# gattia/pyfocusr

Hardware: AMD Instinct MI355X
Metric: lowest-k eigenpairs/sec + KNN-correspondence wall-clock, 250k-vertex mesh pair k=5 (higher is better)
Workload: dtype f64

## Files before the change

include/pyfocusr_hip.h:

```cpp
#ifndef PYFOCUSR_HIP_H
#define PYFOCUSR_HIP_H

#include <stddef.h>
#include <stdint.h>

#ifdef __cplusplus
extern "C" {
#endif

#define PF_VERSION 1

#define PF_OK 0
#define PF_E_ARG (-1)
#define PF_E_HIP (-2)
#define PF_E_DEGENERATE (-3)
#define PF_E_STATE (-4)
#define PF_E_PERSIST_TIMEOUT (-5)
#define PF_E_INTERNAL (-6)

#define PF_OP_RW 0
#define PF_OP_SYM 1

typedef struct pf_ctx pf_ctx;
typedef struct pf_graph pf_graph;
typedef struct pf_mesh pf_mesh;

typedef struct pf_graph_info {
    int64_t n;
    int64_t n_faces;
    int64_t nnz_w;
    int64_t nnz_l;
    int32_t is_symmetric;
    int32_t n_isolated;
    int32_t n_components;
    int32_t max_degree;
    int64_t sell_entries;
    int64_t n_pad;
    int64_t n_oneway;
    double spectral_bound;
} pf_graph_info;

typedef struct pf_timing {
    double op_ms;
    int64_t op_launches;
    double op_bytes;
    double knn_ms;
    double build_ms;
    double persist_ms;
    int64_t persist_launches;
    int64_t persist_steps;
    double persist_bytes;
    double persist_lds_bytes;
} pf_timing;

int pf_version(void);
int pf_pool_poison(int on);
const char* pf_last_error(void);
int pf_device_count(void);
int pf_create(int device, pf_ctx** out);
void pf_destroy(pf_ctx* ctx);
int pf_sync(pf_ctx* ctx);
void* pf_stream(pf_ctx* ctx);
int pf_timing_enable(pf_ctx* ctx, int on);
int pf_timing_get(pf_ctx* ctx, pf_timing* out, int reset);

int pf_graph_build(pf_ctx* ctx, const double* pts, int64_t n, const int32_t* faces, int64_t n_faces,
                   int32_t verts_per_face, pf_graph** out);
int pf_mesh_upload(pf_ctx* ctx, const double* pts, int64_t n, const int32_t* faces, int64_t n_faces,
                   int32_t verts_per_face, pf_mesh** out);
void pf_mesh_free(pf_mesh* mesh);
int pf_graph_build_device(pf_mesh* mesh, pf_graph** out);
int pf_graph_build_device2(pf_mesh* mesh_a, pf_mesh* mesh_b, pf_graph** out_a, pf_graph** out_b);
int pf_graph_from_matrix(pf_ctx* ctx, int64_t n, const int32_t* rowptr, const int32_t* colidx, const double* values,
                         pf_graph** out);
int pf_graph_build_cotan(pf_mesh* mesh, int32_t mass_kind , pf_graph** out);
int pf_graph_cotan_info(pf_graph* g, double* hi, double* total_area);
int pf_graph_cotan_download(pf_graph* g, double* w, double* diag, double* mass);
int pf_cotan_apply(pf_graph* g, const double* x, int32_t ncols, double* out);
void pf_graph_free(pf_graph* g);
int pf_graph_get_info(pf_graph* g, pf_graph_info* out);
int pf_graph_rows_compacted(pf_graph* g);
int pf_graph_download(pf_graph* g, int32_t* rowptr, int32_t* colidx, double* w, double* l_offdiag,
                      double* deg, double* l_diag, int32_t* component_label);

int pf_ws_ensure(pf_graph* g, int32_t n_slots);
int pf_ws_upload(pf_graph* g, int32_t slot, const double* x);
int pf_ws_download(pf_graph* g, int32_t first, int32_t count, double* out);
int pf_ws_copy(pf_graph* g, int32_t src, int32_t dst, int32_t count);
int pf_start_vector(pf_graph* g, int32_t slot, uint64_t seed);
int pf_mask_isolated(pf_graph* g, int32_t slot);
int pf_lock_null_vectors(pf_graph* g, int32_t op, int32_t* n_locked);

int pf_spmv(pf_graph* g, int32_t op, int32_t src, int32_t dst);
int pf_spmv_multi(pf_graph* g, int32_t op, int32_t src_first, int32_t dst_first, int32_t count);
int pf_persist_enable(int on);
int pf_persist_two_step(int level);
int pf_persist_pair_halves(int on);
int pf_persist_clock(pf_ctx* ctx, double* kernel_ms, int64_t* launches, int reset);
typedef struct pf_persist_info {
    int32_t enabled;
    int32_t two_step;
    int32_t owner;
    int32_t timeouts;
    int64_t launches;
    int64_t launches_two_step;
    int32_t suspended_for;
    int32_t rearms;
    int32_t owner_switches;
    int32_t hold_ticks;
} pf_persist_info;
int pf_persist_state(pf_ctx* ctx , pf_persist_info* out);
int pf_graph_window_info(pf_graph* g, int32_t want_rings, int32_t* win_rows, int32_t* n_windows, int32_t* state,
                         int32_t* state2, int32_t* ghosts , int32_t* ghosts2 ,
                         int32_t* need );
int pf_persist_test_hook(int n_launches);
int pf_cheb(pf_graph* g, int32_t op, int32_t src, int32_t dst, int32_t degree, double c, double e, double rho);
int pf_cheb2(pf_graph* ga, int32_t op_a, int32_t src_a, int32_t dst_a, int32_t degree_a, double c_a, double e_a, double rho_a,
             pf_graph* gb, int32_t op_b, int32_t src_b, int32_t dst_b, int32_t degree_b, double c_b, double e_b, double rho_b);
int pf_dots(pf_graph* g, int32_t w, int32_t first, int32_t count, double* out);
int pf_orth(pf_graph* g, int32_t w, int32_t first, int32_t count, double* h, double* nrm);
int pf_orth_begin(pf_graph* g, int32_t w, int32_t first, int32_t count, int32_t normalize);
int pf_orth_end(pf_graph* g, double* h, double* nrm);
int pf_orth_begin2(pf_graph* ga, int32_t w_a, int32_t first_a, int32_t count_a, int32_t normalize_a, pf_graph* gb, int32_t w_b,
                   int32_t first_b, int32_t count_b, int32_t normalize_b);
int pf_orth_cheb2(pf_graph* ga, pf_graph* gb, const int32_t* orth, const int32_t* cheb_i, const double* cheb_d);
int pf_orth_redone(pf_graph* g);
int pf_orth_strict(pf_graph* g, int32_t on);
int pf_orth_device_passes(pf_graph* g, int32_t on);
int pf_orth_split(pf_graph* g, int32_t first2, int32_t split);
int pf_orth_one_launch(int32_t on);
int pf_scale(pf_graph* g, int32_t slot, double alpha);
int pf_combine(pf_graph* g, int32_t src_first, int32_t m, const double* Y, int32_t k, int32_t dst_first);
int pf_resnorm(pf_graph* g, int32_t ax, int32_t x, double lam, double* out);
int pf_gram(pf_graph* g, int32_t first_a, int32_t count_a, int32_t first_b, int32_t count_b, double* out);
int pf_resnorms(pf_graph* g, int32_t ax_first, int32_t x_first, const double* lam, int32_t count, double* out);
int pf_finalize_vectors(pf_graph* g, int32_t first, int32_t count, int32_t from_sym, int32_t minmax,
                        double* out);
int pf_finalize_vectors_begin(pf_graph* g, int32_t first, int32_t count, int32_t from_sym, int32_t minmax, double* out);
int pf_finalize_vectors_end(pf_graph* g);
int pf_final_remap_begin(pf_graph* g, const int32_t* col, const double* sign, int32_t count, double* out);
int pf_host_alloc(size_t bytes, void** out);
int pf_host_free(void* p);
int pf_host_detach(void* p);
int pf_final_rows(pf_graph* g, const int64_t* rows, int64_t n_rows, double* out);
int pf_point_rows(pf_graph* g, const int64_t* rows, int64_t n_rows, double* out);
int pf_spmv_host(pf_graph* g, int32_t op, const double* x, double* y);
int pf_mean_filter(pf_graph* g, const double* values, int32_t ncols, int32_t iterations, double* out);

int pf_knn1(pf_ctx* ctx, const double* ref, int64_t n_ref, const double* qry, int64_t n_qry, int32_t d,
            int64_t* idx_out, double* d2_out);
int pf_knn_mode(pf_ctx* ctx, int32_t mode);
int pf_knn_tree_stats(pf_ctx* ctx, int32_t enable_counting, int64_t* leaves_scanned, int64_t* supers_opened);
int pf_knn_count(pf_ctx* ctx, int32_t enable_counting, int64_t* pairs);
int pf_knn_wave_stats(pf_ctx* ctx, double* sum_us, double* max_us, int64_t* waves, int64_t* max_candidates, double* detail);
int pf_knn(pf_ctx* ctx, const double* ref, int64_t n_ref, const double* qry, int64_t n_qry, int32_t d, int32_t k,
           int64_t* idx_out, double* d2_out);
int pf_knn_topk(pf_ctx* ctx, const double* ref, int64_t n_ref, const double* qry, int64_t n_qry, int32_t d, int32_t k,
                int64_t* idx_out, double* d2_out);
int pf_knn1_graphs(pf_graph* ref_g, pf_graph* qry_g, int32_t d, const int32_t* col_ref, const double* scale_ref,
                   const int32_t* col_qry, const double* scale_qry, int64_t* idx_out, double* d2_out);
int pf_knn1_blocks(pf_ctx* ctx, const double* ref_block, int64_t n_ref, int32_t ref_stride, const double* qry_block,
                   int64_t n_qry, int32_t qry_stride, int32_t d, const int32_t* col_ref, const double* scale_ref,
                   const int32_t* col_qry, const double* scale_qry, int64_t* idx_out, double* d2_out);
int pf_eigsort_costs(pf_graph* g_target, pf_graph* g_source, const int64_t* rows_t, int64_t m_t, const int64_t* rows_s, int64_t m_s,
                     int32_t k, const int32_t* col_t, const double* sign_t, const int32_t* col_s, const double* sign_s, double* out,
                     int64_t* idx_out);
int pf_final_device(pf_graph* g, double** block, int64_t* n_rows, int32_t* n_cols);
int pf_knn_upload(pf_ctx* ctx, const double* ref, int64_t n_ref, const double* qry, int64_t n_qry, int32_t d);
int pf_knn_run(pf_ctx* ctx);
int pf_knn_download(pf_ctx* ctx, int64_t* idx_out, double* d2_out);

int pf_knn1_wide(pf_ctx* ctx, const double* ref, int64_t n_ref, const double* qry, int64_t n_qry, int32_t d,
                 int64_t* idx_out, double* d2_out );
int pf_knn1_wide_count(pf_ctx* ctx, int32_t enable_counting, int64_t* coordinate_pairs);
typedef struct pf_fmap pf_fmap;
int pf_fmap_create(pf_ctx* ctx, const double* phi_t, int64_t n_t, const double* phi_s, int64_t n_s, const double* mass_s,
                   int32_t K, pf_fmap** out);
void pf_fmap_free(pf_fmap* h);
int pf_fmap_set_p2p(pf_fmap* h, const int64_t* T);
int pf_fmap_get_p2p(pf_fmap* h, int64_t* T_out, double* d2_out);
int pf_fmap_project(pf_fmap* h, int32_t k_s, int32_t k_t, double* C_out);
int pf_fmap_convert(pf_fmap* h, const double* C, int32_t k_s, int32_t k_t);
int pf_fmap_zoomout(pf_fmap* h, int32_t k_start, int32_t k_end, int32_t step, int32_t n_iter_at_end, double* C_out);
int pf_fmap_set_samples(pf_fmap* h, const int64_t* S_t, int64_t q_t, const int64_t* S_s, int64_t q_s);
int pf_fmap_zoomout_sampled(pf_fmap* h, int32_t k_start, int32_t k_end, int32_t step, int32_t n_iter_at_end, double* C_out);

int pf_fps(pf_ctx* ctx, const double* points, int64_t n, int32_t d, int64_t m, int64_t start, int64_t* sel_out,
           int32_t* owner_out, double* dmin_out);

int pf_spectral_descriptors(pf_ctx* ctx, const double* phi, int64_t n, int32_t K, const double* G, int32_t T, double* out);
int pf_descriptor_coefficients(pf_ctx* ctx, const double* phi, const double* mass, int64_t n, int32_t K, const double* G,
                               int32_t T, int32_t k_out, double* A_out);

typedef struct pf_eigs_stats {
    int64_t matvecs;
    int32_t outer_steps;
    int32_t restarts;
    int32_t filter_resets;
    int32_t degree;
    int32_t n_null;
    double cut;
    double max_residual;
    int32_t second_passes;
    int32_t mode;
    int32_t local_steps;
    int32_t reserved;
} pf_eigs_stats;
int pf_eigs_smallest(pf_graph* g, int32_t n_wanted, int32_t minmax, double* vals, double* vecs, int32_t* n_out,
                     pf_eigs_stats* stats);
int pf_eigs_smallest_ex(pf_graph* g, int32_t n_wanted, int32_t minmax, int32_t async_download, double* vals, double* vecs,
                        double* residuals, int32_t* n_out, pf_eigs_stats* stats);
int pf_eigs_smallest2(pf_graph* ga, pf_graph* gb, int32_t n_wanted_a, int32_t n_wanted_b, int32_t minmax, int32_t async_download,
                      double* vals_a, double* vecs_a, double* res_a, int32_t* n_out_a, pf_eigs_stats* stats_a,
                      double* vals_b, double* vecs_b, double* res_b, int32_t* n_out_b, pf_eigs_stats* stats_b);

typedef struct pf_rows pf_rows;
int pf_op_step(pf_graph* g, int32_t op, int32_t x, int32_t prev, int32_t out, double alpha, double shift, double beta);
int pf_cheb_steps(pf_graph* g, int32_t op, int32_t prev, int32_t cur, int32_t k_first, int32_t n_steps, double c, double e,
                  double rho, int32_t* out_prev, int32_t* out_cur);
int pf_axpy(pf_graph* g, int32_t w, int32_t first, int32_t count, const double* coef);
int pf_rows_create(pf_graph* g, const int64_t* rows, int64_t n, pf_rows** out);
void pf_rows_free(pf_rows* r);
int pf_rows_gather(pf_rows* r, int32_t slot, double* out);
int pf_rows_scatter(pf_rows* r, int32_t slot, const double* in);
int pf_rows_gather_dev(pf_rows* r, int32_t slot, double* dst_device);
int pf_rows_scatter_dev(pf_rows* r, int32_t slot, const double* src_device);
int pf_rows_set_sources(pf_rows* r, const int64_t* offsets);
int pf_rows_gather2_dev(pf_rows* r, int32_t slot_a, int32_t slot_b, double* dst_device, int64_t stride);
int pf_rows_scatter2_dev(pf_rows* r, int32_t slot_a, int32_t slot_b, const double* src_device, int64_t stride);
int pf_rows_fill(pf_rows* r, int32_t slot, double value);

typedef struct pf_surface pf_surface;
int pf_surface_create(pf_ctx* ctx, const double* points, int64_t n, const int32_t* faces, int64_t n_faces,
                      int32_t verts_per_face, pf_surface** out);
void pf_surface_free(pf_surface* s);
int pf_surface_closest(pf_surface* s, const double* qry, int64_t n_qry, double* out_pts, int32_t* out_face,
                       double* out_d2);
int pf_surface_distance(pf_surface* s, const double* qry, int64_t n_qry, double* out_d2, int32_t* out_face,
                        double* stats);
int pf_surface_prepare_signed(pf_surface* s, const double* points, const int32_t* faces, int64_t* topology);
int pf_surface_signed_distance(pf_surface* s, const double* qry, int64_t n_qry, double* out_sd, int32_t* out_face,
                               int32_t* out_feature, int64_t* n_ambiguous);
int pf_surface_prepare_winding(pf_surface* s);
int pf_surface_winding(pf_surface* s, const double* qry, int64_t n_qry, double beta, double* out_w, double* out_bound);
int pf_surface_raycast(pf_surface* s, const double* origins, const double* dirs, int64_t n_rays, double t_min, double t_max,
                       int32_t facing, double* out_t, int32_t* out_face, double* out_uv, int32_t* out_count);
int pf_surface_vertex_normals(pf_surface* s, double* out);

typedef struct pf_surface_nd pf_surface_nd;
int pf_surface_nd_create(pf_ctx* ctx, const double* coords, int64_t n, int32_t d, const int32_t* faces, int64_t n_faces,
                         int32_t verts_per_face, pf_surface_nd** out);
void pf_surface_nd_free(pf_surface_nd* s);
int pf_surface_nd_closest(pf_surface_nd* s, const double* qry, int64_t n_qry, int32_t* out_face, int32_t* out_verts,
                          double* out_bary, double* out_d2, int32_t exhaustive);
int pf_surface_nd_last_search(pf_surface_nd* s, int64_t* chunks_opened, int64_t* packets, int64_t* n_chunks);

typedef struct pf_cpd pf_cpd;
int pf_cpd_create(pf_ctx* ctx, const double* X, int64_t N, const double* Y, int64_t M, int32_t d, pf_cpd** out);
void pf_cpd_free(pf_cpd* h);
int pf_cpd_estep(pf_cpd* h, const double* TY, double sigma2, double w, double* P1, double* Pt1, double* PX);
int pf_cpd_set_basis(pf_cpd* h, const double* Q, int32_t K);
int pf_cpd_weighted_gram(pf_cpd* h, double* H);
int pf_cpd_affine_sums(pf_cpd* h, double* shifts, double* sums);
int pf_cpd_apply_affine(pf_cpd* h, const double* B, const double* t);
int pf_cpd_deform_sums(pf_cpd* h, double* H, double* R);
int pf_cpd_apply_deform(pf_cpd* h, const double* C, double* sums);
int pf_cpd_download(pf_cpd* h, double* TY, double* P1, double* Pt1, double* PX);
int pf_cpd_gram(pf_ctx* ctx, const double* A, int64_t n_a, const double* B, int64_t n_b, int32_t d, double beta,
                const double* V, int32_t n_cols, double* out);

typedef struct pf_assign_stats {
    int32_t phases;
    int32_t dense_passes;
    int64_t rounds;
    int64_t bids;
    int64_t dense_bids;
    int64_t candidate_edges;
    int64_t launches;
    int64_t device_bytes;
    int32_t k;
    int32_t eps_floor_hit;
    double eps_initial, eps_final, eps_floor;
    double total_cost;
    double gap_bound;
    double lower_bound;
    double ms_candidates, ms_auction, ms_certificate;
} pf_assign_stats;
int pf_assign(pf_ctx* ctx, const double* rows, int64_t n_rows, const double* cols, int64_t n_cols, int32_t d,
              int64_t* col_of_row, double* u_out, double* v_out, pf_assign_stats* stats);

int pf_curvatures(pf_ctx* ctx, const double* pts, int64_t n, const int32_t* faces, int64_t n_faces, double* out_area,
                  double* out_gauss, double* out_mean, double* out_tensor6, double* out_kminmax, double* out_dirs,
                  double* out_normals, uint8_t* out_boundary, int64_t* topology, double* device_ms);

#define PF_TOPOLOGY_OUTWARD 1u
int pf_mesh_topology(pf_ctx* ctx, const double* pts, int64_t n, const int32_t* faces, int64_t n_faces, uint32_t flags,
                     int32_t* face_neighbours, int32_t* patch, uint8_t* flip, int32_t* boundary_loop, uint8_t* patch_orientable,
                     double* patch_volume, int64_t* report, double* device_ms);

#define PF_CLUSTER_UPDATE_ONLY 1u
int pf_mesh_cluster(pf_ctx* ctx, const double* pts, int64_t n, const int32_t* faces, int64_t n_faces, const double* mass,
                    const int64_t* seeds, int64_t m, int32_t n_iter, uint32_t flags, const double* centroids_in,
                    const int32_t* labels_in, int32_t* labels, double* centroids, int32_t* rep, int32_t* count, int32_t* changed,
                    int32_t* out_faces, int32_t* face_src, int32_t* votes, int64_t* report, double* device_ms);

int pf_map_distortion(pf_ctx* ctx, const double* src_pts, int64_t n_src, const int32_t* src_faces, int64_t n_faces,
                      const double* tgt_pts, int64_t n_tgt, const double* tgt_normals, const int32_t* map_vertices,
                      const double* map_weights, int32_t c, double* face_sigma, double* face_area_ratio, uint8_t* face_flags,
                      double* vertex_area, double* vertex_sigma, uint8_t* vertex_flags, int32_t* target_count,
                      double* target_premass, double* totals, int64_t* report, double* device_ms);

#ifdef __cplusplus
}
#endif
#endif
```

pyfocusr_amd/_hip.py:

```python
import atexit
import ctypes as C
import os
import threading
import weakref

import numpy as np

_HERE = os.path.dirname(os.path.abspath(__file__))
LIB_PATH = os.environ.get("PYFOCUSR_HIP_LIB", os.path.join(_HERE, "csrc", "libpyfocusr_hip.so"))

PF_OP_RW = 0
PF_OP_SYM = 1

_f64p = C.POINTER(C.c_double)
_i32p = C.POINTER(C.c_int32)
_i64p = C.POINTER(C.c_int64)


class HipUnavailable(RuntimeError):
    pass


class PfError(RuntimeError):
    def __init__(self, code, msg):
        RuntimeError.__init__(self, "libpyfocusr_hip error %d: %s" % (code, msg))
        self.code = code


class _Struct(C.Structure):

    def as_dict(self):
        return {name: getattr(self, name) for name, _ in self._fields_}


class GraphInfo(_Struct):
    _fields_ = [("n", C.c_int64), ("n_faces", C.c_int64), ("nnz_w", C.c_int64), ("nnz_l", C.c_int64),
                ("is_symmetric", C.c_int32), ("n_isolated", C.c_int32), ("n_components", C.c_int32),
                ("max_degree", C.c_int32), ("sell_entries", C.c_int64), ("n_pad", C.c_int64), ("n_oneway", C.c_int64),
                ("spectral_bound", C.c_double)]


class EigsStats(_Struct):
    _fields_ = [("matvecs", C.c_int64), ("outer_steps", C.c_int32), ("restarts", C.c_int32), ("filter_resets", C.c_int32),
                ("degree", C.c_int32), ("n_null", C.c_int32), ("cut", C.c_double), ("max_residual", C.c_double),
                ("second_passes", C.c_int32), ("mode", C.c_int32), ("local_steps", C.c_int32), ("reserved", C.c_int32)]


class Timing(_Struct):
    _fields_ = [("op_ms", C.c_double), ("op_launches", C.c_int64), ("op_bytes", C.c_double), ("knn_ms", C.c_double),
                ("build_ms", C.c_double), ("persist_ms", C.c_double), ("persist_launches", C.c_int64),
                ("persist_steps", C.c_int64), ("persist_bytes", C.c_double), ("persist_lds_bytes", C.c_double)]


class AssignStats(_Struct):
    _fields_ = [("phases", C.c_int32), ("dense_passes", C.c_int32), ("rounds", C.c_int64), ("bids", C.c_int64),
                ("dense_bids", C.c_int64), ("candidate_edges", C.c_int64), ("launches", C.c_int64),
                ("device_bytes", C.c_int64), ("k", C.c_int32), ("eps_floor_hit", C.c_int32), ("eps_initial", C.c_double),
                ("eps_final", C.c_double), ("eps_floor", C.c_double), ("total_cost", C.c_double),
                ("gap_bound", C.c_double), ("lower_bound", C.c_double), ("ms_candidates", C.c_double),
                ("ms_auction", C.c_double), ("ms_certificate", C.c_double)]


SIGNATURES = {
    "pf_version": (C.c_int, []),
    "pf_pool_poison": (C.c_int, [C.c_int]),
    "pf_last_error": (C.c_char_p, []),
    "pf_device_count": (C.c_int, []),
    "pf_create": (C.c_int, [C.c_int, C.POINTER(C.c_void_p)]),
    "pf_destroy": (None, [C.c_void_p]),
    "pf_sync": (C.c_int, [C.c_void_p]),
    "pf_stream": (C.c_void_p, [C.c_void_p]),
    "pf_timing_enable": (C.c_int, [C.c_void_p, C.c_int]),
    "pf_timing_get": (C.c_int, [C.c_void_p, C.POINTER(Timing), C.c_int]),
    "pf_graph_build": (C.c_int, [C.c_void_p, _f64p, C.c_int64, _i32p, C.c_int64, C.c_int32, C.POINTER(C.c_void_p)]),
    "pf_mesh_upload": (C.c_int, [C.c_void_p, _f64p, C.c_int64, _i32p, C.c_int64, C.c_int32, C.POINTER(C.c_void_p)]),
    "pf_mesh_free": (None, [C.c_void_p]),
    "pf_graph_build_device": (C.c_int, [C.c_void_p, C.POINTER(C.c_void_p)]),
    "pf_graph_build_device2": (C.c_int, [C.c_void_p, C.c_void_p, C.POINTER(C.c_void_p), C.POINTER(C.c_void_p)]),
    "pf_graph_from_matrix": (C.c_int, [C.c_void_p, C.c_int64, _i32p, _i32p, _f64p, C.POINTER(C.c_void_p)]),
    "pf_graph_build_cotan": (C.c_int, [C.c_void_p, C.c_int32, C.POINTER(C.c_void_p)]),
    "pf_graph_cotan_info": (C.c_int, [C.c_void_p, C.POINTER(C.c_double), C.POINTER(C.c_double)]),
    "pf_graph_cotan_download": (C.c_int, [C.c_void_p, _f64p, _f64p, _f64p]),
    "pf_cotan_apply": (C.c_int, [C.c_void_p, _f64p, C.c_int32, _f64p]),
    "pf_graph_free": (None, [C.c_void_p]),
    "pf_graph_get_info": (C.c_int, [C.c_void_p, C.POINTER(GraphInfo)]),
    "pf_graph_rows_compacted": (C.c_int, [C.c_void_p]),
    "pf_graph_download": (C.c_int, [C.c_void_p, _i32p, _i32p, _f64p, _f64p, _f64p, _f64p, _i32p]),
    "pf_ws_ensure": (C.c_int, [C.c_void_p, C.c_int32]),
    "pf_ws_upload": (C.c_int, [C.c_void_p, C.c_int32, _f64p]),
    "pf_ws_download": (C.c_int, [C.c_void_p, C.c_int32, C.c_int32, _f64p]),
    "pf_ws_copy": (C.c_int, [C.c_void_p, C.c_int32, C.c_int32, C.c_int32]),
    "pf_start_vector": (C.c_int, [C.c_void_p, C.c_int32, C.c_uint64]),
    "pf_mask_isolated": (C.c_int, [C.c_void_p, C.c_int32]),
    "pf_lock_null_vectors": (C.c_int, [C.c_void_p, C.c_int32, _i32p]),
    "pf_spmv": (C.c_int, [C.c_void_p, C.c_int32, C.c_int32, C.c_int32]),
    "pf_spmv_multi": (C.c_int, [C.c_void_p, C.c_int32, C.c_int32, C.c_int32, C.c_int32]),
    "pf_knn_mode": (C.c_int, [C.c_void_p, C.c_int32]),
    "pf_knn_tree_stats": (C.c_int, [C.c_void_p, C.c_int32, C.POINTER(C.c_int64), C.POINTER(C.c_int64)]),
    "pf_persist_enable": (C.c_int, [C.c_int]),
    "pf_persist_two_step": (C.c_int, [C.c_int]),
    "pf_persist_pair_halves": (C.c_int, [C.c_int]),
    "pf_persist_clock": (C.c_int, [C.c_void_p, C.POINTER(C.c_double), C.POINTER(C.c_int64), C.c_int]),
    "pf_persist_state": (C.c_int, [C.c_void_p, C.c_void_p]),
    "pf_graph_window_info": (C.c_int, [C.c_void_p, C.c_int32] + [C.POINTER(C.c_int32)] * 4 + [_i32p, _i32p, _i32p]),
    "pf_persist_test_hook": (C.c_int, [C.c_int]),
    "pf_cheb": (C.c_int, [C.c_void_p, C.c_int32, C.c_int32, C.c_int32, C.c_int32, C.c_double, C.c_double, C.c_double]),
    "pf_cheb2": (C.c_int, [C.c_void_p, C.c_int32, C.c_int32, C.c_int32, C.c_int32, C.c_double, C.c_double, C.c_double,
                           C.c_void_p, C.c_int32, C.c_int32, C.c_int32, C.c_int32, C.c_double, C.c_double, C.c_double]),
    "pf_dots": (C.c_int, [C.c_void_p, C.c_int32, C.c_int32, C.c_int32, _f64p]),
    "pf_orth": (C.c_int, [C.c_void_p, C.c_int32, C.c_int32, C.c_int32, _f64p, _f64p]),
    "pf_orth_begin": (C.c_int, [C.c_void_p, C.c_int32, C.c_int32, C.c_int32, C.c_int32]),
    "pf_orth_end": (C.c_int, [C.c_void_p, _f64p, _f64p]),
    "pf_orth_split": (C.c_int, [C.c_void_p, C.c_int32, C.c_int32]),
    "pf_orth_one_launch": (C.c_int, [C.c_int32]),
    "pf_orth_begin2": (C.c_int, [C.c_void_p, C.c_int32, C.c_int32, C.c_int32, C.c_int32, C.c_void_p, C.c_int32, C.c_int32, C.c_int32,
                                 C.c_int32]),
    "pf_orth_cheb2": (C.c_int, [C.c_void_p, C.c_void_p, _i32p, _i32p, _f64p]),
    "pf_eigsort_costs": (C.c_int, [C.c_void_p, C.c_void_p, _i64p, C.c_int64, _i64p, C.c_int64, C.c_int32, _i32p, _f64p, _i32p, _f64p, _f64p,
                                   _i64p]),
    "pf_orth_redone": (C.c_int, [C.c_void_p]),
    "pf_orth_strict": (C.c_int, [C.c_void_p, C.c_int32]),
    "pf_scale": (C.c_int, [C.c_void_p, C.c_int32, C.c_double]),
    "pf_combine": (C.c_int, [C.c_void_p, C.c_int32, C.c_int32, _f64p, C.c_int32, C.c_int32]),
    "pf_resnorm": (C.c_int, [C.c_void_p, C.c_int32, C.c_int32, C.c_double, _f64p]),
    "pf_gram": (C.c_int, [C.c_void_p, C.c_int32, C.c_int32, C.c_int32, C.c_int32, _f64p]),
    "pf_resnorms": (C.c_int, [C.c_void_p, C.c_int32, C.c_int32, _f64p, C.c_int32, _f64p]),
    "pf_finalize_vectors": (C.c_int, [C.c_void_p, C.c_int32, C.c_int32, C.c_int32, C.c_int32, _f64p]),
    "pf_finalize_vectors_begin": (C.c_int, [C.c_void_p, C.c_int32, C.c_int32, C.c_int32, C.c_int32, _f64p]),
    "pf_finalize_vectors_end": (C.c_int, [C.c_void_p]),
    "pf_final_remap_begin": (C.c_int, [C.c_void_p, _i32p, _f64p, C.c_int32, _f64p]),
    "pf_host_alloc": (C.c_int, [C.c_size_t, C.POINTER(C.c_void_p)]),
    "pf_host_free": (C.c_int, [C.c_void_p]),
    "pf_final_rows": (C.c_int, [C.c_void_p, _i64p, C.c_int64, _f64p]),
    "pf_point_rows": (C.c_int, [C.c_void_p, _i64p, C.c_int64, _f64p]),
    "pf_spmv_host": (C.c_int, [C.c_void_p, C.c_int32, _f64p, _f64p]),
    "pf_mean_filter": (C.c_int, [C.c_void_p, _f64p, C.c_int32, C.c_int32, _f64p]),
    "pf_knn1": (C.c_int, [C.c_void_p, _f64p, C.c_int64, _f64p, C.c_int64, C.c_int32, _i64p, _f64p]),
    "pf_knn": (C.c_int, [C.c_void_p, _f64p, C.c_int64, _f64p, C.c_int64, C.c_int32, C.c_int32, _i64p, _f64p]),
    "pf_knn_topk": (C.c_int, [C.c_void_p, _f64p, C.c_int64, _f64p, C.c_int64, C.c_int32, C.c_int32, _i64p, _f64p]),
    "pf_knn1_graphs": (C.c_int, [C.c_void_p, C.c_void_p, C.c_int32, _i32p, _f64p, _i32p, _f64p, _i64p, _f64p]),
    "pf_knn1_blocks": (C.c_int, [C.c_void_p, C.c_void_p, C.c_int64, C.c_int32, C.c_void_p, C.c_int64, C.c_int32, C.c_int32,
                                 _i32p, _f64p, _i32p, _f64p, _i64p, _f64p]),
    "pf_final_device": (C.c_int, [C.c_void_p, C.POINTER(C.c_void_p), _i64p, _i32p]),
    "pf_knn_upload": (C.c_int, [C.c_void_p, _f64p, C.c_int64, _f64p, C.c_int64, C.c_int32]),
    "pf_knn_run": (C.c_int, [C.c_void_p]),
    "pf_knn_download": (C.c_int, [C.c_void_p, _i64p, _f64p]),
    "pf_eigs_smallest": (C.c_int, [C.c_void_p, C.c_int32, C.c_int32, _f64p, _f64p, C.POINTER(C.c_int32), C.POINTER(EigsStats)]),
    "pf_knn_count": (C.c_int, [C.c_void_p, C.c_int32, C.POINTER(C.c_int64)]),
    "pf_knn_wave_stats": (C.c_int, [C.c_void_p, C.POINTER(C.c_double), C.POINTER(C.c_double), C.POINTER(C.c_int64), C.POINTER(C.c_int64),
                                    _f64p]),
    "pf_host_detach": (C.c_int, [C.c_void_p]),
    "pf_orth_device_passes": (C.c_int, [C.c_void_p, C.c_int32]),
    "pf_eigs_smallest_ex": (C.c_int, [C.c_void_p, C.c_int32, C.c_int32, C.c_int32, _f64p, _f64p, _f64p, C.POINTER(C.c_int32),
                                      C.POINTER(EigsStats)]),
    "pf_eigs_smallest2": (C.c_int, [C.c_void_p, C.c_void_p, C.c_int32, C.c_int32, C.c_int32, C.c_int32,
                                    _f64p, _f64p, _f64p, C.POINTER(C.c_int32), C.POINTER(EigsStats),
                                    _f64p, _f64p, _f64p, C.POINTER(C.c_int32), C.POINTER(EigsStats)]),
    "pf_op_step": (C.c_int, [C.c_void_p, C.c_int32, C.c_int32, C.c_int32, C.c_int32, C.c_double, C.c_double, C.c_double]),
    "pf_cheb_steps": (C.c_int, [C.c_void_p, C.c_int32, C.c_int32, C.c_int32, C.c_int32, C.c_int32, C.c_double, C.c_double,
                                C.c_double, C.POINTER(C.c_int32), C.POINTER(C.c_int32)]),
    "pf_axpy": (C.c_int, [C.c_void_p, C.c_int32, C.c_int32, C.c_int32, _f64p]),
    "pf_rows_create": (C.c_int, [C.c_void_p, _i64p, C.c_int64, C.POINTER(C.c_void_p)]),
    "pf_rows_free": (None, [C.c_void_p]),
    "pf_rows_gather": (C.c_int, [C.c_void_p, C.c_int32, _f64p]),
    "pf_rows_scatter": (C.c_int, [C.c_void_p, C.c_int32, _f64p]),
    "pf_rows_gather_dev": (C.c_int, [C.c_void_p, C.c_int32, C.c_void_p]),
    "pf_rows_scatter_dev": (C.c_int, [C.c_void_p, C.c_int32, C.c_void_p]),
    "pf_rows_set_sources": (C.c_int, [C.c_void_p, _i64p]),
    "pf_rows_gather2_dev": (C.c_int, [C.c_void_p, C.c_int32, C.c_int32, C.c_void_p, C.c_int64]),
    "pf_rows_scatter2_dev": (C.c_int, [C.c_void_p, C.c_int32, C.c_int32, C.c_void_p, C.c_int64]),
    "pf_rows_fill": (C.c_int, [C.c_void_p, C.c_int32, C.c_double]),
    "pf_surface_create": (C.c_int, [C.c_void_p, _f64p, C.c_int64, _i32p, C.c_int64, C.c_int32, C.POINTER(C.c_void_p)]),
    "pf_surface_free": (None, [C.c_void_p]),
    "pf_surface_closest": (C.c_int, [C.c_void_p, _f64p, C.c_int64, _f64p, _i32p, _f64p]),
    "pf_surface_distance": (C.c_int, [C.c_void_p, _f64p, C.c_int64, _f64p, _i32p, _f64p]),
    "pf_surface_prepare_signed": (C.c_int, [C.c_void_p, _f64p, _i32p, _i64p]),
    "pf_surface_signed_distance": (C.c_int, [C.c_void_p, _f64p, C.c_int64, _f64p, _i32p, _i32p, _i64p]),
    "pf_surface_prepare_winding": (C.c_int, [C.c_void_p]),
    "pf_surface_winding": (C.c_int, [C.c_void_p, _f64p, C.c_int64, C.c_double, _f64p, _f64p]),
    "pf_surface_raycast": (C.c_int, [C.c_void_p, _f64p, _f64p, C.c_int64, C.c_double, C.c_double, C.c_int32, _f64p, _i32p, _f64p,
                                     _i32p]),
    "pf_surface_vertex_normals": (C.c_int, [C.c_void_p, _f64p]),
    "pf_knn1_wide": (C.c_int, [C.c_void_p, _f64p, C.c_int64, _f64p, C.c_int64, C.c_int32, _i64p, _f64p]),
    "pf_knn1_wide_count": (C.c_int, [C.c_void_p, C.c_int32, _i64p]),
    "pf_fmap_create": (C.c_int, [C.c_void_p, _f64p, C.c_int64, _f64p, C.c_int64, _f64p, C.c_int32, C.POINTER(C.c_void_p)]),
    "pf_fmap_free": (None, [C.c_void_p]),
    "pf_fmap_set_p2p": (C.c_int, [C.c_void_p, _i64p]),
    "pf_fmap_get_p2p": (C.c_int, [C.c_void_p, _i64p, _f64p]),
    "pf_fmap_project": (C.c_int, [C.c_void_p, C.c_int32, C.c_int32, _f64p]),
    "pf_fmap_convert": (C.c_int, [C.c_void_p, _f64p, C.c_int32, C.c_int32]),
    "pf_fmap_zoomout": (C.c_int, [C.c_void_p, C.c_int32, C.c_int32, C.c_int32, C.c_int32, _f64p]),
    "pf_fmap_set_samples": (C.c_int, [C.c_void_p, _i64p, C.c_int64, _i64p, C.c_int64]),
    "pf_fmap_zoomout_sampled": (C.c_int, [C.c_void_p, C.c_int32, C.c_int32, C.c_int32, C.c_int32, _f64p]),
    "pf_fps": (C.c_int, [C.c_void_p, _f64p, C.c_int64, C.c_int32, C.c_int64, C.c_int64, _i64p, _i32p, _f64p]),
    "pf_spectral_descriptors": (C.c_int, [C.c_void_p, _f64p, C.c_int64, C.c_int32, _f64p, C.c_int32, _f64p]),
    "pf_descriptor_coefficients": (C.c_int, [C.c_void_p, _f64p, _f64p, C.c_int64, C.c_int32, _f64p, C.c_int32, C.c_int32, _f64p]),
    "pf_surface_nd_create": (C.c_int, [C.c_void_p, _f64p, C.c_int64, C.c_int32, _i32p, C.c_int64, C.c_int32,
                                       C.POINTER(C.c_void_p)]),
    "pf_surface_nd_free": (None, [C.c_void_p]),
    "pf_surface_nd_closest": (C.c_int, [C.c_void_p, _f64p, C.c_int64, _i32p, _i32p, _f64p, _f64p, C.c_int32]),
    "pf_surface_nd_last_search": (C.c_int, [C.c_void_p, _i64p, _i64p, _i64p]),
    "pf_cpd_create": (C.c_int, [C.c_void_p, _f64p, C.c_int64, _f64p, C.c_int64, C.c_int32, C.POINTER(C.c_void_p)]),
    "pf_cpd_free": (None, [C.c_void_p]),
    "pf_cpd_estep": (C.c_int, [C.c_void_p, _f64p, C.c_double, C.c_double, _f64p, _f64p, _f64p]),
    "pf_cpd_set_basis": (C.c_int, [C.c_void_p, _f64p, C.c_int32]),
    "pf_cpd_weighted_gram": (C.c_int, [C.c_void_p, _f64p]),
    "pf_cpd_affine_sums": (C.c_int, [C.c_void_p, _f64p, _f64p]),
    "pf_cpd_apply_affine": (C.c_int, [C.c_void_p, _f64p, _f64p]),
    "pf_cpd_deform_sums": (C.c_int, [C.c_void_p, _f64p, _f64p]),
    "pf_cpd_apply_deform": (C.c_int, [C.c_void_p, _f64p, _f64p]),
    "pf_cpd_download": (C.c_int, [C.c_void_p, _f64p, _f64p, _f64p, _f64p]),
    "pf_cpd_gram": (C.c_int, [C.c_void_p, _f64p, C.c_int64, _f64p, C.c_int64, C.c_int32, C.c_double, _f64p, C.c_int32, _f64p]),
    "pf_assign": (C.c_int, [C.c_void_p, _f64p, C.c_int64, _f64p, C.c_int64, C.c_int32, _i64p, _f64p, _f64p,
                            C.POINTER(AssignStats)]),
    "pf_curvatures": (C.c_int, [C.c_void_p, _f64p, C.c_int64, _i32p, C.c_int64, _f64p, _f64p, _f64p, _f64p, _f64p, _f64p, _f64p,
                                C.POINTER(C.c_uint8), _i64p, _f64p]),
    "pf_mesh_topology": (C.c_int, [C.c_void_p, _f64p, C.c_int64, _i32p, C.c_int64, C.c_uint32, _i32p, _i32p, C.POINTER(C.c_uint8),
                                   _i32p, C.POINTER(C.c_uint8), _f64p, _i64p, _f64p]),
    "pf_mesh_cluster": (C.c_int, [C.c_void_p, _f64p, C.c_int64, _i32p, C.c_int64, _f64p, _i64p, C.c_int64, C.c_int32, C.c_uint32,
                                  _f64p, _i32p, _i32p, _f64p, _i32p, _i32p, _i32p, _i32p, _i32p, _i32p, _i64p, _f64p]),
    "pf_map_distortion": (C.c_int, [C.c_void_p, _f64p, C.c_int64, _i32p, C.c_int64, _f64p, C.c_int64, _f64p, _i32p, _f64p, C.c_int32,
                                    _f64p, _f64p, C.POINTER(C.c_uint8), _f64p, _f64p, C.POINTER(C.c_uint8), _i32p, _f64p, _f64p,
                                    _i64p, _f64p]),
}

_lib = None
_lib_lock = threading.Lock()
_live_graphs = weakref.WeakSet()
_live_contexts = weakref.WeakSet()


@atexit.register
def _shutdown():
    for g in list(_live_graphs):
        g.close()
    for c in list(_live_contexts):
        c.close()


def load_library():
    global _lib
    with _lib_lock:
        if _lib is not None:
            return _lib
        if not os.path.exists(LIB_PATH):
            raise HipUnavailable(
                "%s not found: build it with `python -c 'import __graft_entry__ as g; g.build()'` "
                "(hipcc --offload-arch=gfx950); there is no CPU fallback" % LIB_PATH)
        lib = C.CDLL(LIB_PATH)
        for name, (res, args) in SIGNATURES.items():
            fn = getattr(lib, name)
            fn.restype = res
            fn.argtypes = args
        _lib = lib
        return lib


PF_E_DEGENERATE = -3
PF_E_STATE = -4
PF_E_PERSIST_TIMEOUT = -5
PF_E_INTERNAL = -6
PF_TOPOLOGY_OUTWARD = 1
PF_CLUSTER_UPDATE_ONLY = 1


class _PinnedBlock(object):
    __slots__ = ("ptr", "nbytes")

    def __init__(self, ptr, nbytes):
        self.ptr, self.nbytes = ptr, nbytes

    def __del__(self):
        try:
            _pinned_release(self.ptr, self.nbytes)
        except Exception:
            pass


_pinned_free = {}
_pinned_cached = [0]
_pinned_lock = threading.RLock()
_PINNED_CACHE_BYTES = 1 << 30


def _pinned_release(ptr, nbytes):
    if _pinned_free is None or _lib is None:
        return
    _lib.pf_host_detach(C.c_void_p(ptr))
    evicted = []
    with _pinned_lock:
        if nbytes <= _PINNED_CACHE_BYTES:
            while _pinned_cached[0] + nbytes > _PINNED_CACHE_BYTES:
                others = [sz for sz, ptrs in _pinned_free.items() if ptrs and sz != nbytes]
                if not others:
                    break
                sz = max(others)
                evicted.append(_pinned_free[sz].pop())
                _pinned_cached[0] -= sz
        keep = _pinned_cached[0] + nbytes <= _PINNED_CACHE_BYTES
        if keep:
            _pinned_free.setdefault(nbytes, []).append(ptr)
            _pinned_cached[0] += nbytes
    for other in evicted:
        _lib.pf_host_free(C.c_void_p(other))
    if not keep:
        _lib.pf_host_free(C.c_void_p(ptr))


def pinned_trim():
    with _pinned_lock:
        blocks = [p for ptrs in _pinned_free.values() for p in ptrs]
        _pinned_free.clear()
        _pinned_cached[0] = 0
    for ptr in blocks:
        _lib.pf_host_free(C.c_void_p(ptr))


def pinned_empty(shape, dtype=np.float64):
    lib = load_library()
    dtype = np.dtype(dtype)
    count = int(np.prod(shape)) if len(shape) else 1
    nbytes = max(count * dtype.itemsize, 1)
    nbytes = (nbytes + 4095) & ~4095
    ptr = None
    with _pinned_lock:
        free = _pinned_free.get(nbytes)
        if free:
            ptr = free.pop()
            _pinned_cached[0] -= nbytes
    if ptr is None:
        p = C.c_void_p()
        _check(lib.pf_host_alloc(C.c_size_t(nbytes), C.byref(p)))
        ptr = int(p.value)
    buf = (C.c_char * nbytes).from_address(ptr)
    buf._pf_block = _PinnedBlock(ptr, nbytes)
    return np.frombuffer(buf, dtype=dtype, count=count).reshape(shape)


def persist_enable(on=True):
    _check(load_library().pf_persist_enable(int(bool(on))))


def pool_poison(on=True):
    on = int(on)
    if on not in (0, 1, 2):
        raise ValueError("pool_poison: 0 (off), 1 (0xFF bytes) or 2 (zero bytes), got %r" % (on,))
    _check(load_library().pf_pool_poison(on))


def orth_one_launch(on=True):
    _check(load_library().pf_orth_one_launch(int(bool(on))))


def persist_two_step(level=1):
    _check(load_library().pf_persist_two_step(int(level)))


def persist_pair_halves(on=True):
    _check(load_library().pf_persist_pair_halves(int(bool(on))))


def persist_clock(ctx, reset=False):
    ms, n = C.c_double(0.0), C.c_int64(0)
    _check(load_library().pf_persist_clock(ctx._h, C.byref(ms), C.byref(n), int(bool(reset))))
    return ms.value, n.value


class _PersistInfo(_Struct):
    _fields_ = [("enabled", C.c_int32), ("two_step", C.c_int32), ("owner", C.c_int32), ("timeouts", C.c_int32),
                ("launches", C.c_int64), ("launches_two_step", C.c_int64), ("suspended_for", C.c_int32), ("rearms", C.c_int32),
                ("owner_switches", C.c_int32), ("hold_ticks", C.c_int32)]


def persist_state(ctx=None):
    info = _PersistInfo()
    _check(load_library().pf_persist_state(None if ctx is None else ctx._h, C.byref(info)))
    return info.as_dict()


def persist_test_hook(n_launches=1):
    _check(load_library().pf_persist_test_hook(int(n_launches)))


def _check(code):
    if code != 0:
        raise PfError(code, load_library().pf_last_error().decode("utf-8", "replace"))


_POINTER_OF = {np.dtype(t): C.POINTER(c) for t, c in ((np.float64, C.c_double), (np.int32, C.c_int32), (np.int64, C.c_int64),
                                                        (np.uint8, C.c_uint8), (np.uint64, C.c_uint64))}


def _ptr(a):
    if a is None:
        return None
    try:
        ptype = _POINTER_OF[a.dtype]
    except KeyError:
        raise TypeError("no pointer type for dtype %s: the library takes float64, int32, int64, uint8 and uint64" % a.dtype)
    if not a.flags.c_contiguous:
        raise ValueError("the library needs a C-contiguous array, not a strided view")
    return a.ctypes.data_as(ptype)


def _f64(a):
    if a is not None and a.dtype != np.float64:
        raise TypeError("a float64 array is needed, not %s" % a.dtype)
    return _ptr(a)


def _c_f64(a, shape=None):
    a = np.ascontiguousarray(a, dtype=np.float64)
    if shape is not None and a.shape != shape:
        raise ValueError("expected shape %r, got %r" % (shape, a.shape))
    return a


def _c_i32(a):
    return np.ascontiguousarray(a, dtype=np.int32)


def _c_i64(a):
    return np.ascontiguousarray(a, dtype=np.int64)


_EQUAL_D = "%s must be (n, d) arrays with equal d"


def _same_d(a, b, message=_EQUAL_D % "ref and qry"):
    a, b = _c_f64(a), _c_f64(b)
    if a.ndim != 2 or b.ndim != 2 or a.shape[1] != b.shape[1]:
        raise ValueError(message)
    return a, b


def _queries(a, noun="queries", message=None):
    a = _c_f64(a)
    if a.ndim != 2 or a.shape[1] != 3 or a.shape[0] == 0:
        raise ValueError(message or "%s must be a non-empty (n, 3) array" % noun)
    return a


def _rays(origins, directions):
    message = "origins and directions must be non-empty (n, 3) arrays of the same length"
    o, d = _queries(origins, message=message), _c_f64(directions)
    if d.shape != o.shape:
        raise ValueError(message)
    return o, d


def _upload_arrays(points, faces, empty_ok=True):
    pts, f = _c_f64(points).reshape(-1, 3), _c_i32(faces)
    if f.ndim != 2 or not (empty_ok or f.shape[0]):
        raise ValueError("faces must be %s" % ("(F, verts_per_face)" if empty_ok else "a non-empty (F, verts_per_face) array"))
    return pts, f, f.shape[1] if f.shape[0] else 3


def degenerate_extent_message(target_points, source_points):
    found = []
    for name, pts in (("target", target_points), ("source", source_points)):
        pts = np.asarray(pts, dtype=np.float64).reshape(-1, 3)
        with np.errstate(invalid="ignore"):
            flat = np.isnan(pts).any(axis=0) | ~(np.max(pts, axis=0) > np.min(pts, axis=0))
        if flat.any():
            found.append("the %s sample (%d points) has no extent along %s" % (name, len(pts), ", ".join("xyz"[a] for a in np.where(flat)[0])))
    return ("eigsort: degenerate extent - %s: the min-max normalisation of the sampled points divides by zero (a planar "
            "mesh, or a sample of one point), so no point has a nearest neighbour"
            % ("; ".join(found) if found else "the sampled points do not compare"))


KNN_TOPK_MAX_K = 64
KNN_TOPK_MAX_D = 128


def check_knn_topk(ref, qry, k):
    ref_shape, qry_shape = np.shape(ref), np.shape(qry)
    if len(ref_shape) != 2 or len(qry_shape) != 2 or ref_shape[1] != qry_shape[1]:
        raise ValueError(_EQUAL_D % "ref and qry")
    if not 1 <= ref_shape[1] <= KNN_TOPK_MAX_D:
        raise ValueError("d = %d out of range (1 .. %d)" % (ref_shape[1], KNN_TOPK_MAX_D))
    k = int(k)
    if not 1 <= k <= min(KNN_TOPK_MAX_K, ref_shape[0]):
        raise ValueError("k = %d out of range (1 .. min(%d, n_ref = %d))" % (k, KNN_TOPK_MAX_K, ref_shape[0]))
    return k


class Context(object):

    def __init__(self, device=0):
        lib = load_library()
        if lib.pf_device_count() <= 0:
            raise HipUnavailable("no HIP device visible: the pyfocusr_amd hot path needs an MI355X (no CPU fallback)")
        h = C.c_void_p()
        _check(lib.pf_create(int(device), C.byref(h)))
        self._lib = lib
        self._h = h
        self.device = int(device)
        self._children = weakref.WeakSet()
        _live_contexts.add(self)

    def close(self):
        if getattr(self, "_h", None):
            for child in list(self._children):
                child.close()
            self._lib.pf_destroy(self._h)
            self._h = None

    def __del__(self):
        try:
            self.close()
        except Exception:
            pass

    def sync(self):
        _check(self._lib.pf_sync(self._h))

    @property
    def stream_ptr(self):
        return int(self._lib.pf_stream(self._h) or 0)

    def timing_enable(self, on=True):
        _check(self._lib.pf_timing_enable(self._h, int(on)))

    def timing(self, reset=False):
        t = Timing()
        _check(self._lib.pf_timing_get(self._h, C.byref(t), int(bool(reset))))
        return t.as_dict()

    def knn_mode(self, mode):
        _check(self._lib.pf_knn_mode(self._h, int(mode)))

    def knn_count(self, enable_counting=False):
        pairs = C.c_int64()
        _check(self._lib.pf_knn_count(self._h, int(bool(enable_counting)), C.byref(pairs)))
        return int(pairs.value)

    def knn_tree_stats(self, enable_counting=False):
        a, b = C.c_int64(), C.c_int64()
        _check(self._lib.pf_knn_tree_stats(self._h, int(bool(enable_counting)), C.byref(a), C.byref(b)))
        return int(a.value), int(b.value)

    def knn1(self, ref, qry, return_d2=False):
        ref, qry = _same_d(ref, qry)
        idx = np.empty(qry.shape[0], dtype=np.int64)
        d2 = np.empty(qry.shape[0], dtype=np.float64) if return_d2 else None
        _check(self._lib.pf_knn1(self._h, _f64(ref), ref.shape[0], _f64(qry), qry.shape[0], ref.shape[1],
                                 _ptr(idx), _f64(d2)))
        return (idx, d2) if return_d2 else idx

    def knn1_wide(self, ref, qry, return_d2=False):
        ref, qry = _same_d(ref, qry)
        idx = np.empty(qry.shape[0], dtype=np.int64)
        d2 = np.empty(qry.shape[0], dtype=np.float64) if return_d2 else None
        _check(self._lib.pf_knn1_wide(self._h, _f64(ref), ref.shape[0], _f64(qry), qry.shape[0], ref.shape[1],
                                      _ptr(idx), _f64(d2)))
        return (idx, d2) if return_d2 else idx

    def knn1_wide_count(self, enable_counting=False):
        pairs = C.c_int64()
        _check(self._lib.pf_knn1_wide_count(self._h, int(bool(enable_counting)), C.byref(pairs)))
        return int(pairs.value)

    def farthest_point_sampling(self, points, m, start=-1, return_owner=False, return_d2=False):
        pts = _c_f64(points)
        if pts.ndim != 2:
            raise ValueError("points must be an (n, d) array")
        n, m = pts.shape[0], int(m)
        sel = np.empty(max(m, 0), dtype=np.int64)
        owner = np.empty(n, dtype=np.int32) if return_owner else None
        d2 = np.empty(n, dtype=np.float64) if return_d2 else None
        _check(self._lib.pf_fps(self._h, _f64(pts), n, pts.shape[1], m, int(start), _ptr(sel), _ptr(owner), _f64(d2)))
        out = (sel,) + ((owner,) if return_owner else ()) + ((d2,) if return_d2 else ())
        return out if len(out) > 1 else sel

    def spectral_descriptors(self, phi, G):
        phi, G = _c_f64(phi), _c_f64(G)
        if phi.ndim != 2 or G.ndim != 2 or G.shape[0] != phi.shape[1]:
            raise ValueError("phi must be (n, K) and G (K, T)")
        out = np.empty((phi.shape[0], G.shape[1]), dtype=np.float64)
        _check(self._lib.pf_spectral_descriptors(self._h, _f64(phi), phi.shape[0], phi.shape[1], _f64(G), G.shape[1], _f64(out)))
        return out

    def descriptor_coefficients(self, phi, mass, G, k_out):
        phi, G = _c_f64(phi), _c_f64(G)
        if phi.ndim != 2 or G.ndim != 2 or G.shape[0] != phi.shape[1]:
            raise ValueError("phi must be (n, K) and G (K, T)")
        mass = _c_f64(mass, (phi.shape[0],))
        out = np.empty((max(int(k_out), 0), G.shape[1]), dtype=np.float64)
        _check(self._lib.pf_descriptor_coefficients(self._h, _f64(phi), _f64(mass), phi.shape[0], phi.shape[1], _f64(G), G.shape[1],
                                                    int(k_out), _f64(out)))
        return out

    def curvatures(self, points, faces):
        pts = _c_f64(points)
        f = _c_i32(faces)
        if pts.ndim != 2 or pts.shape[1] != 3 or f.ndim != 2 or f.shape[1] != 3:
            raise ValueError("points must be (n, 3) and faces (m, 3)")
        n = pts.shape[0]
        out = {"area": np.empty(n), "gaussian": np.empty(n), "mean": np.empty(n), "tensor": np.empty((n, 6)), "k": np.empty((n, 4)),
               "dirs": np.empty((n, 6)), "normals": np.empty((n, 3))}
        boundary = np.empty(n, dtype=np.uint8)
        topology = np.zeros(5, dtype=np.int64)
        ms = C.c_double(0.0)
        _check(self._lib.pf_curvatures(self._h, _f64(pts), n, _ptr(f), f.shape[0], _f64(out["area"]),
                                       _f64(out["gaussian"]), _f64(out["mean"]), _f64(out["tensor"]), _f64(out["k"]),
                                       _f64(out["dirs"]), _f64(out["normals"]), _ptr(boundary), _ptr(topology), C.byref(ms)))
        out.update(boundary=boundary.astype(bool), topology=topology, device_ms=ms.value)
        return out

    def mesh_topology(self, n_points, faces, points=None, outward=True):
        f = _c_i32(faces)
        if f.ndim != 2 or f.shape[1] != 3:
            raise ValueError("faces must be (m, 3)")
        n, m = int(n_points), f.shape[0]
        pts = None
        if points is not None:
            pts = _c_f64(points)
            if pts.shape != (n, 3):
                raise ValueError("points must be (n_points, 3)")
        nbr, loop = np.empty((m, 3), dtype=np.int32), np.empty((m, 3), dtype=np.int32)
        patch, flip = np.empty(m, dtype=np.int32), np.empty(m, dtype=np.uint8)
        orientable, volume = np.empty(m, dtype=np.uint8), np.empty(m)
        report = np.zeros(8, dtype=np.int64)
        ms = C.c_double(0.0)
        _check(self._lib.pf_mesh_topology(self._h, _f64(pts), n, _ptr(f), m, PF_TOPOLOGY_OUTWARD if outward else 0, _ptr(nbr),
                                          _ptr(patch), _ptr(flip), _ptr(loop), _ptr(orientable), _f64(volume), _ptr(report),
                                          C.byref(ms)))
        P = int(report[4])
        return {"face_neighbours": nbr, "patch": patch, "flip": flip.astype(bool), "boundary_loop": loop,
                "patch_orientable": orientable[:P].astype(bool), "patch_volume": volume[:P].copy(), "report": report,
                "device_ms": ms.value}

    def cluster_mesh(self, points, faces, mass, seeds=None, n_iter=20, centroids=None, labels=None, update_only=False):
        pts = _c_f64(points)
        if pts.ndim != 2 or pts.shape[1] != 3:
            raise ValueError("points must be (n, 3)")
        n = pts.shape[0]
        f = np.zeros((0, 3), dtype=np.int32) if faces is None else _c_i32(faces)
        if f.ndim != 2 or f.shape[1] != 3:
            raise ValueError("faces must be (f, 3)")
        mass = _c_f64(mass, (n,))
        if (seeds is None) == (centroids is None):
            raise ValueError("give either seeds or centroids")
        sel = cen = lab = None
        if seeds is not None:
            sel = _c_i64(seeds)
            if sel.ndim != 1:
                raise ValueError("seeds must be a vector of vertex indices")
            m = sel.shape[0]
        else:
            cen = _c_f64(centroids)
            if cen.ndim != 2 or cen.shape[1] != 3:
                raise ValueError("centroids must be (m, 3)")
            m = cen.shape[0]
        if labels is not None:
            lab = _c_i32(labels)
            if lab.shape != (n,):
                raise ValueError("labels must be (n,)")
        n_iter, k = int(n_iter), f.shape[0]
        out_labels, out_c = np.empty(n, dtype=np.int32), np.empty((m, 3))
        rep, count = np.empty(m, dtype=np.int32), np.empty(m, dtype=np.int32)
        changed = np.zeros(max(n_iter, 0), dtype=np.int32)
        out_f, src, votes = np.empty((k, 3), dtype=np.int32), np.empty(k, dtype=np.int32), np.empty((k, 2), dtype=np.int32)
        report = np.zeros(8, dtype=np.int64)
        ms = C.c_double(0.0)
        _check(self._lib.pf_mesh_cluster(
            self._h, _f64(pts), n, _ptr(f if k else None), k, _f64(mass), _ptr(sel), m, n_iter,
            PF_CLUSTER_UPDATE_ONLY if update_only else 0, _f64(cen), _ptr(lab), _ptr(out_labels), _f64(out_c), _ptr(rep),
            _ptr(count), _ptr(changed), _ptr(out_f), _ptr(src), _ptr(votes), _ptr(report), C.byref(ms)))
        run, kept = (0 if update_only else int(report[0])), int(report[1])
        return {"labels": out_labels, "centroids": out_c, "rep": rep, "count": count, "changed": changed[:run].copy(),
                "n_iter_run": int(report[0]), "faces": out_f[:kept].copy(), "face_src": src[:kept].copy(),
                "votes": votes[:kept].copy(), "n_candidate_faces": int(report[2]), "report": report, "device_ms": ms.value}

    def map_distortion(self, src_points, src_faces, tgt_points, map_vertices, map_weights=None, tgt_normals=None):
        pts, tgt = _c_f64(src_points), _c_f64(tgt_points)
        f = _c_i32(src_faces)
        if pts.ndim != 2 or pts.shape[1] != 3 or tgt.ndim != 2 or tgt.shape[1] != 3 or f.ndim != 2 or f.shape[1] != 3:
            raise ValueError("points must be (n, 3) and faces (m, 3)")
        n, m, k = pts.shape[0], f.shape[0], tgt.shape[0]
        mv = _c_i32(map_vertices)
        if mv.ndim == 1:
            mv = mv.reshape(-1, 1)
        if mv.ndim != 2 or mv.shape[0] != n or mv.shape[1] not in (1, 3):
            raise ValueError("map_vertices must be (n,), (n, 1) or (n, 3)")
        c = mv.shape[1]
        mw = None
        if c == 3:
            if map_weights is None:
                raise ValueError("a map of 3 corners needs map_weights (n, 3)")
            mw = _c_f64(map_weights, (n, 3))
        nrm = None if tgt_normals is None else _c_f64(tgt_normals, (k, 3))
        out = {"face_sigma": np.empty((m, 2)), "face_area_ratio": np.empty(m), "face_flags": np.empty(m, dtype=np.uint8),
               "vertex_area": np.empty(n), "vertex_sigma": np.empty((n, 2)), "vertex_flags": np.empty(n, dtype=np.uint8),
               "target_count": np.empty(k, dtype=np.int32), "target_premass": np.empty(k), "totals": np.zeros(8),
               "report": np.zeros(8, dtype=np.int64)}
        ms = C.c_double(0.0)
        _check(self._lib.pf_map_distortion(
            self._h, _f64(pts), n, _ptr(f), m, _f64(tgt), k, _f64(nrm), _ptr(mv), _f64(mw), c, _f64(out["face_sigma"]),
            _f64(out["face_area_ratio"]), _ptr(out["face_flags"]), _f64(out["vertex_area"]), _f64(out["vertex_sigma"]),
            _ptr(out["vertex_flags"]), _ptr(out["target_count"]), _f64(out["target_premass"]), _f64(out["totals"]),
            _ptr(out["report"]), C.byref(ms)))
        out["device_ms"] = ms.value
        return out

    def assign(self, rows, cols, return_duals=False):
        rows, cols = _same_d(rows, cols, _EQUAL_D % "rows and cols")
        if not (np.isfinite(rows).all() and np.isfinite(cols).all()):
            raise ValueError("coordinates must be finite")
        n_r, n_c = rows.shape[0], cols.shape[0]
        col = np.empty(n_r, dtype=np.int64)
        u = np.empty(n_r) if return_duals else None
        v = np.empty(n_c) if return_duals else None
        stats = AssignStats()
        _check(self._lib.pf_assign(self._h, _f64(rows), n_r, _f64(cols), n_c, rows.shape[1], _ptr(col), _f64(u), _f64(v),
                                   C.byref(stats)))
        return (col, stats, u, v) if return_duals else (col, stats)

    def knn(self, ref, qry, k):
        ref, qry = _same_d(ref, qry)
        idx = np.empty((qry.shape[0], int(k)), dtype=np.int64)
        d2 = np.empty((qry.shape[0], int(k)), dtype=np.float64)
        _check(self._lib.pf_knn(self._h, _f64(ref), ref.shape[0], _f64(qry), qry.shape[0], ref.shape[1], int(k),
                                _ptr(idx), _f64(d2)))
        return idx, d2

    def knn_topk(self, ref, qry, k, return_d2=True):
        k = check_knn_topk(ref, qry, k)
        ref, qry = _c_f64(ref), _c_f64(qry)
        idx = np.empty((qry.shape[0], k), dtype=np.int64)
        d2 = np.empty((qry.shape[0], k), dtype=np.float64) if return_d2 else None
        _check(self._lib.pf_knn_topk(self._h, _f64(ref), ref.shape[0], _f64(qry), qry.shape[0], ref.shape[1], k,
                                     _ptr(idx), _f64(d2)))
        return (idx, d2) if return_d2 else idx

    def knn1_graphs(self, dev_ref, dev_qry, col_ref, scale_ref, col_qry, scale_qry, return_d2=False):
        col_ref, col_qry = _c_i32(col_ref), _c_i32(col_qry)
        scale_ref, scale_qry = _c_f64(scale_ref), _c_f64(scale_qry)
        d = len(col_ref)
        if not (len(col_qry) == len(scale_ref) == len(scale_qry) == d):
            raise ValueError("col / scale arrays must share one length d")
        idx = np.empty(dev_qry.n, dtype=np.int64)
        d2 = np.empty(dev_qry.n, dtype=np.float64) if return_d2 else None
        _check(self._lib.pf_knn1_graphs(dev_ref._h, dev_qry._h, d, _ptr(col_ref), _f64(scale_ref), _ptr(col_qry), _f64(scale_qry),
                                        _ptr(idx), _f64(d2)))
        return (idx, d2) if return_d2 else idx

    def eigsort_costs(self, dev_t, dev_s, rows_t, rows_s, k, col_t, sign_t, col_s, sign_s):
        rows_t, rows_s, col_t, col_s = _c_i64(rows_t), _c_i64(rows_s), _c_i32(col_t), _c_i32(col_s)
        sign_t, sign_s = _c_f64(sign_t), _c_f64(sign_s)
        if min(len(col_t), len(col_s), len(sign_t), len(sign_s)) < k:
            raise ValueError("eigsort_costs: k columns / signs per graph are needed")
        out = np.empty((4, int(k), int(k)), dtype=np.float64)
        idx = np.empty(len(rows_t), dtype=np.int64)
        _check(self._lib.pf_eigsort_costs(dev_t._h, dev_s._h, _ptr(rows_t), len(rows_t), _ptr(rows_s), len(rows_s), int(k),
                                          _ptr(col_t), _f64(sign_t), _ptr(col_s), _f64(sign_s), _f64(out), _ptr(idx)))
        if len(idx) and (idx.min() < 0 or idx.max() >= len(rows_s)):
            raise ValueError(degenerate_extent_message(dev_t.point_rows(rows_t), dev_s.point_rows(rows_s)))
        return out, idx

    def knn1_blocks(self, ref_ptr, n_ref, ref_stride, qry_ptr, n_qry, qry_stride, col_ref, scale_ref, col_qry, scale_qry,
                    return_d2=False):
        col_ref, col_qry = _c_i32(col_ref), _c_i32(col_qry)
        scale_ref, scale_qry = _c_f64(scale_ref), _c_f64(scale_qry)
        d = len(col_ref)
        if not (len(col_qry) == len(scale_ref) == len(scale_qry) == d):
            raise ValueError("col / scale arrays must share one length d")
        idx = np.empty(int(n_qry), dtype=np.int64)
        d2 = np.empty(int(n_qry), dtype=np.float64) if return_d2 else None
        _check(self._lib.pf_knn1_blocks(self._h, C.c_void_p(int(ref_ptr)), int(n_ref), int(ref_stride), C.c_void_p(int(qry_ptr)),
                                        int(n_qry), int(qry_stride), d, _ptr(col_ref), _f64(scale_ref), _ptr(col_qry),
                                        _f64(scale_qry), _ptr(idx), _f64(d2)))
        return (idx, d2) if return_d2 else idx

    def knn_upload(self, ref, qry):
        ref, qry = _c_f64(ref), _c_f64(qry)
        _check(self._lib.pf_knn_upload(self._h, _f64(ref), ref.shape[0], _f64(qry), qry.shape[0], ref.shape[1]))
        self._knn_nq = qry.shape[0]

    def knn_run(self):
        _check(self._lib.pf_knn_run(self._h))

    def knn_download(self):
        idx = np.empty(self._knn_nq, dtype=np.int64)
        d2 = np.empty(self._knn_nq, dtype=np.float64)
        _check(self._lib.pf_knn_download(self._h, _ptr(idx), _f64(d2)))
        return idx, d2


_default_ctx = {}


def default_context(device=None):
    if device is None:
        device = int(os.environ.get("PYFOCUSR_DEVICE", os.environ.get("LOCAL_RANK", "0")))
        n = load_library().pf_device_count()
        if n > 0:
            device %= n
    if device not in _default_ctx:
        _default_ctx[device] = Context(device)
    return _default_ctx[device]


class _Handle(object):

    _free = None
    _h = None

    def __init__(self, ctx=None):
        self.ctx = ctx if ctx is not None else default_context()
        self._lib = self.ctx._lib

    def _adopt(self, h):
        self._h = h
        _live_graphs.add(self)
        self.ctx._children.add(self)

    def _create(self, name, *args):
        h = C.c_void_p()
        _check(getattr(self._lib, name)(*(args + (C.byref(h),))))
        self._adopt(h)

    def close(self):
        h, self._h = self._h, None
        if h:
            getattr(self._lib, self._free)(h)

    def __enter__(self):
        return self

    def __exit__(self, *exc):
        self.close()
        return False

    def __del__(self):
        try:
            self.close()
        except Exception:
            pass


class DeviceMesh(_Handle):

    _free = "pf_mesh_free"

    def __init__(self, points, faces, ctx=None):
        _Handle.__init__(self, ctx)
        pts, f, v = _upload_arrays(points, faces)
        self._create("pf_mesh_upload", self.ctx._h, _f64(pts), pts.shape[0], _ptr(f), f.shape[0], v)
        self.n, self.n_faces = pts.shape[0], f.shape[0]


def _fan_triangles(faces):
    v = faces.shape[1]
    return np.stack([faces[:, [0, j + 1, j + 2]] for j in range(v - 2)], axis=1).reshape(-1, 3)


class DeviceSurface(_Handle):

    _free = "pf_surface_free"

    def __init__(self, points, faces, ctx=None):
        _Handle.__init__(self, ctx)
        pts, f, v = _upload_arrays(points, faces, empty_ok=False)
        self._create("pf_surface_create", self.ctx._h, _f64(pts), pts.shape[0], _ptr(f), f.shape[0], v)
        self.n, self.n_faces = pts.shape[0], f.shape[0]
        self.points, self.faces = pts, f
        self._topology = None
        self._winding_ready = False

    def _prepare_signed(self):
        if self._topology is None:
            t = np.zeros(4, dtype=np.int64)
            _check(self._lib.pf_surface_prepare_signed(self._h, _f64(self.points), _ptr(self.faces), _ptr(t)))
            self._topology = t
        return self._topology

    def topology(self):
        t = self._prepare_signed()
        tri = _fan_triangles(self.faces)
        a, b, c = self.points[tri[:, 0]], self.points[tri[:, 1]], self.points[tri[:, 2]]
        volume = float(np.sum(np.einsum("ij,ij->i", a, np.cross(b, c)))) / 6.0
        return {"n_edges": int(t[0]), "n_boundary_edges": int(t[1]), "n_nonmanifold_edges": int(t[2]),
                "n_inconsistent_edges": int(t[3]), "closed": bool(t[1] == 0), "volume": volume}

    def signed_distance(self, queries):
        q = _queries(queries)
        self._prepare_signed()
        sd = np.empty(len(q), dtype=np.float64)
        face = np.empty(len(q), dtype=np.int32)
        feature = np.empty(len(q), dtype=np.int32)
        amb = C.c_int64(0)
        _check(self._lib.pf_surface_signed_distance(self._h, _f64(q), len(q), _f64(sd), _ptr(face), _ptr(feature), C.byref(amb)))
        return sd, face, feature, int(amb.value)

    def winding_number(self, queries, beta=0.0):
        q = _queries(queries)
        if not self._winding_ready:
            _check(self._lib.pf_surface_prepare_winding(self._h))
            self._winding_ready = True
        w = np.empty(len(q), dtype=np.float64)
        bound = np.empty(len(q), dtype=np.float64)
        _check(self._lib.pf_surface_winding(self._h, _f64(q), len(q), float(beta), _f64(w), _f64(bound)))
        return w, bound

    def raycast(self, origins, directions, t_min=0.0, t_max=np.inf, facing=0, count=False):
        o, d = _rays(origins, directions)
        t = np.empty(len(o), dtype=np.float64)
        face = np.empty(len(o), dtype=np.int32)
        uv = np.empty((len(o), 2), dtype=np.float64)
        n_hit = np.empty(len(o), dtype=np.int32) if count else None
        _check(self._lib.pf_surface_raycast(self._h, _f64(o), _f64(d), len(o), float(t_min), float(t_max), int(facing), _f64(t),
                                            _ptr(face), _f64(uv), _ptr(n_hit)))
        return (t, face, uv, n_hit) if count else (t, face, uv)

    def vertex_normals(self):
        self._prepare_signed()
        out = np.empty((self.n, 3), dtype=np.float64)
        _check(self._lib.pf_surface_vertex_normals(self._h, _f64(out)))
        return out

    def closest(self, queries):
        q = _c_f64(queries).reshape(-1, 3)
        pts = np.empty_like(q)
        face = np.empty(len(q), dtype=np.int32)
        d2 = np.empty(len(q), dtype=np.float64)
        _check(self._lib.pf_surface_closest(self._h, _f64(q), len(q), _f64(pts), _ptr(face), _f64(d2)))
        return pts, face, d2

    def distance(self, queries, per_point=True):
        q = _queries(queries)
        d2 = np.empty(len(q), dtype=np.float64) if per_point else None
        face = np.empty(len(q), dtype=np.int32) if per_point else None
        st = np.empty(6, dtype=np.float64)
        _check(self._lib.pf_surface_distance(self._h, _f64(q), len(q), _f64(d2), _ptr(face), _f64(st)))
        stats = {"n_finite": int(st[0]), "n_nan": int(st[1]), "sum_d": float(st[2]), "sum_d2": float(st[3]),
                 "max_d": float(st[4]), "argmax": int(st[5])}
        return d2, face, stats


class DeviceSurfaceND(_Handle):

    MAX_DIM = 16
    _free = "pf_surface_nd_free"

    def __init__(self, coords, faces, ctx=None):
        x = _c_f64(coords)
        f = _c_i32(faces)
        if x.ndim != 2 or x.shape[0] == 0 or not 1 <= x.shape[1] <= self.MAX_DIM:
            raise ValueError("coords must be a non-empty (n, d) array with 1 <= d <= %d" % self.MAX_DIM)
        if f.ndim != 2 or f.shape[0] == 0 or f.shape[1] < 3:
            raise ValueError("faces must be a non-empty (F, verts_per_face >= 3) array")
        _Handle.__init__(self, ctx)
        self._create("pf_surface_nd_create", self.ctx._h, _f64(x), x.shape[0], x.shape[1], _ptr(f), f.shape[0], f.shape[1])
        self.n, self.d, self.n_faces = x.shape[0], x.shape[1], f.shape[0]

    def closest(self, queries, exhaustive=False):
        q = _c_f64(queries)
        if q.ndim != 2 or q.shape[0] == 0 or q.shape[1] != self.d:
            raise ValueError("queries must be a non-empty (n, %d) array" % self.d)
        face = np.empty(len(q), dtype=np.int32)
        verts = np.empty((len(q), 3), dtype=np.int32)
        bary = np.empty((len(q), 3), dtype=np.float64)
        d2 = np.empty(len(q), dtype=np.float64)
        _check(self._lib.pf_surface_nd_closest(self._h, _f64(q), len(q), _ptr(face), _ptr(verts),
                                               _f64(bary), _f64(d2), 1 if exhaustive else 0))
        return face, verts, bary, d2

    def last_search(self):
        v = [C.c_int64(0) for _ in range(3)]
        _check(self._lib.pf_surface_nd_last_search(self._h, *[C.byref(x) for x in v]))
        return {"chunks_opened": int(v[0].value), "packets": int(v[1].value), "n_chunks": int(v[2].value)}


class DeviceFunctionalMap(_Handle):

    MAX_K = 128
    _free = "pf_fmap_free"

    def __init__(self, phi_t, phi_s, mass_s, ctx=None):
        pt, ps, m = _c_f64(phi_t), _c_f64(phi_s), _c_f64(mass_s)
        if pt.ndim != 2 or ps.ndim != 2 or pt.shape[1] != ps.shape[1] or pt.shape[0] == 0 or ps.shape[0] == 0:
            raise ValueError("phi_t and phi_s must be non-empty (n, K) arrays with equal K")
        if not 1 <= pt.shape[1] <= self.MAX_K:
            raise ValueError("1 <= K <= %d basis functions, got %d" % (self.MAX_K, pt.shape[1]))
        if m.shape != (ps.shape[0],):
            raise ValueError("mass_s must have one entry per source vertex")
        _Handle.__init__(self, ctx)
        self._create("pf_fmap_create", self.ctx._h, _f64(pt), pt.shape[0], _f64(ps), ps.shape[0], _f64(m), pt.shape[1])
        self.n_t, self.n_s, self.K = pt.shape[0], ps.shape[0], pt.shape[1]

    def set_p2p(self, T):
        T = _c_i64(T)
        if T.shape != (self.n_s,):
            raise ValueError("T must have one target index per source vertex")
        _check(self._lib.pf_fmap_set_p2p(self._h, _ptr(T)))

    def get_p2p(self, return_d2=False):
        T = np.empty(self.n_s, dtype=np.int64)
        d2 = np.empty(self.n_s) if return_d2 else None
        _check(self._lib.pf_fmap_get_p2p(self._h, _ptr(T), _f64(d2)))
        return (T, d2) if return_d2 else T

    def project(self, k_s, k_t):
        Cm = np.empty((int(k_s), int(k_t)))
        _check(self._lib.pf_fmap_project(self._h, int(k_s), int(k_t), _f64(Cm)))
        return Cm

    def convert(self, k_s, k_t, Cm=None):
        if Cm is not None:
            Cm = _c_f64(Cm, (int(k_s), int(k_t)))
        _check(self._lib.pf_fmap_convert(self._h, _f64(Cm), int(k_s), int(k_t)))

    def zoomout(self, k_start, k_end, step=1, n_iter_at_end=0):
        Cm = np.empty((int(k_end), int(k_end)))
        _check(self._lib.pf_fmap_zoomout(self._h, int(k_start), int(k_end), int(step), int(n_iter_at_end), _f64(Cm)))
        return Cm

    def set_samples(self, S_t, S_s):
        S_t, S_s = _c_i64(S_t), _c_i64(S_s)
        if S_t.ndim != 1 or S_s.ndim != 1:
            raise ValueError("S_t and S_s must be vectors of indices")
        _check(self._lib.pf_fmap_set_samples(self._h, _ptr(S_t), S_t.shape[0], _ptr(S_s), S_s.shape[0]))

    def zoomout_sampled(self, k_start, k_end, step=1, n_iter_at_end=0):
        if not 1 <= int(k_end) <= self.K:
            raise ValueError("k_end must lie in 1 .. K = %d" % self.K)
        Cm = np.empty((int(k_end), int(k_end)))
        _check(self._lib.pf_fmap_zoomout_sampled(self._h, int(k_start), int(k_end), int(step), int(n_iter_at_end), _f64(Cm)))
        return Cm


class DeviceCpd(_Handle):

    _free = "pf_cpd_free"

    def __init__(self, X, Y, ctx=None):
        _Handle.__init__(self, ctx)
        X, Y = _same_d(X, Y, "X (N,d) and Y (M,d) must share d")
        self.N, self.M, self.D = X.shape[0], Y.shape[0], X.shape[1]
        self._create("pf_cpd_create", self.ctx._h, _f64(X), self.N, _f64(Y), self.M, self.D)
        self._P1, self._Pt1, self._PX = np.empty(self.M), np.empty(self.N), np.empty((self.M, self.D))
        self._H = np.empty((0, 0))

    def estep(self, TY, sigma2, w=0.0):
        TY = _c_f64(TY)
        if TY.shape != (self.M, self.D):
            raise ValueError("TY must be (%d, %d)" % (self.M, self.D))
        _check(self._lib.pf_cpd_estep(self._h, _f64(TY), float(sigma2), float(w), _f64(self._P1), _f64(self._Pt1),
                                      _f64(self._PX)))
        return self._P1, self._Pt1, self._PX

    def estep_resident(self, sigma2, w=0.0):
        _check(self._lib.pf_cpd_estep(self._h, None, float(sigma2), float(w), None, None, None))

    def affine_sums(self):
        D = self.D
        shifts, sums = np.empty(32), np.empty(2 * D * D + 3 * D + 3)
        _check(self._lib.pf_cpd_affine_sums(self._h, _f64(shifts), _f64(sums)))
        o = 1 + 2 * D + 2 * D * D
        return dict(cx=shifts[:D], cy=shifts[16:16 + D], Np=sums[0], sPX=sums[1:1 + D], sP1Y=sums[1 + D:1 + 2 * D],
                    PXY=sums[1 + 2 * D:1 + 2 * D + D * D].reshape(D, D), YPY=sums[1 + 2 * D + D * D:o].reshape(D, D),
                    sPt1=sums[o], sPt1XX=sums[o + 1], sPt1X=sums[o + 2:o + 2 + D])

    def apply_affine(self, B, t):
        B, t = _c_f64(B), _c_f64(t)
        _check(self._lib.pf_cpd_apply_affine(self._h, _f64(B), _f64(t)))

    def deform_sums(self):
        K = self._H.shape[0]
        R = np.empty((K, self.D))
        _check(self._lib.pf_cpd_deform_sums(self._h, _f64(self._H), _f64(R)))
        return self._H, R

    def apply_deform(self, Cmat):
        Cmat = _c_f64(Cmat)
        sums = np.empty(5)
        _check(self._lib.pf_cpd_apply_deform(self._h, _f64(Cmat), _f64(sums)))
        return sums

    def download(self):
        TY = np.empty((self.M, self.D))
        _check(self._lib.pf_cpd_download(self._h, _f64(TY), _f64(self._P1), _f64(self._Pt1), _f64(self._PX)))
        return TY, self._P1, self._Pt1, self._PX

    def set_basis(self, Q):
        Q = _c_f64(Q)
        if Q.ndim != 2 or Q.shape[0] != self.M:
            raise ValueError("Q must be (%d, K)" % self.M)
        _check(self._lib.pf_cpd_set_basis(self._h, _f64(Q), Q.shape[1]))
        self._H = np.empty((Q.shape[1], Q.shape[1]))

    def weighted_gram(self):
        _check(self._lib.pf_cpd_weighted_gram(self._h, _f64(self._H)))
        return self._H


def gaussian_gram_product(A, B, beta, V, ctx=None):
    ctx = ctx if ctx is not None else default_context()
    A, B, V = _c_f64(A), _c_f64(B), _c_f64(V)
    if A.ndim != 2 or B.ndim != 2 or A.shape[1] != B.shape[1] or V.ndim != 2 or V.shape[0] != B.shape[0]:
        raise ValueError("shapes: A (a,d), B (b,d), V (b,c)")
    out = np.empty((A.shape[0], V.shape[1]))
    _check(ctx._lib.pf_cpd_gram(ctx._h, _f64(A), A.shape[0], _f64(B), B.shape[0], A.shape[1], float(beta), _f64(V),
                                V.shape[1], _f64(out)))
    return out


class _Rows(_Handle):

    _free = "pf_rows_free"

    def __init__(self, graph, idx):
        _Handle.__init__(self, graph.ctx)
        idx = _c_i64(idx)
        self._create("pf_rows_create", graph._h, _ptr(idx), len(idx))
        self.n = len(idx)


class DeviceLaplacian(_Handle):

    _free = "pf_graph_free"
    _rows = ()
    cotangent = False

    def __init__(self, points=None, faces=None, ctx=None, device_mesh=None, matrix=None, _handle=None, cotangent=False):
        if cotangent:
            if matrix is not None or _handle is not None:
                raise ValueError("cotangent=True needs a mesh (points and faces, or device_mesh)")
            mesh = device_mesh if device_mesh is not None else DeviceMesh(points, faces, ctx=ctx)
            _Handle.__init__(self, mesh.ctx)
            try:
                self._create("pf_graph_build_cotan", mesh._h, 0)
            finally:
                if device_mesh is None:
                    mesh.close()
        elif _handle is not None:
            _Handle.__init__(self, _handle[0])
            self._adopt(_handle[1])
        elif matrix is not None:
            _Handle.__init__(self, ctx)
            rp, ci, va = _c_i32(matrix[0]), _c_i32(matrix[1]), _c_f64(matrix[2])
            self._create("pf_graph_from_matrix", self.ctx._h, len(rp) - 1, _ptr(rp), _ptr(ci), _f64(va))
        elif device_mesh is not None:
            _Handle.__init__(self, device_mesh.ctx)
            self._create("pf_graph_build_device", device_mesh._h)
        else:
            _Handle.__init__(self, ctx)
            pts, f, v = _upload_arrays(points, faces)
            self._create("pf_graph_build", self.ctx._h, _f64(pts), pts.shape[0], _ptr(f), f.shape[0], v)
        h = self._h
        info = GraphInfo()
        _check(self._lib.pf_graph_get_info(h, C.byref(info)))
        self.info = info
        fields = info.as_dict()
        for name in ("n", "nnz_w", "nnz_l", "n_isolated", "n_components", "max_degree", "n_oneway"):
            setattr(self, name, fields[name])
        self.symmetric = bool(info.is_symmetric)
        self.rows_compacted = bool(self._lib.pf_graph_rows_compacted(h))
        self.spectral_bound = info.spectral_bound if 0.0 < info.spectral_bound <= 2.0 else 2.0
        self.op = PF_OP_SYM if self.symmetric else PF_OP_RW
        self.has_points = matrix is None
        self._rows = []
        if cotangent:
            self.cotangent = True
            hi, area = C.c_double(), C.c_double()
            _check(self._lib.pf_graph_cotan_info(h, C.byref(hi), C.byref(area)))
            self.hi, self.total_area = float(hi.value), float(area.value)
            self.spectral_bound = self.hi
            self.mass = self.cotan_download(w=False, diag=False)["mass"]

    @classmethod
    def build_pair(cls, mesh_a, mesh_b):
        if mesh_a.ctx is not mesh_b.ctx:
            raise ValueError("build_pair: the two meshes must belong to one context")
        ha, hb = C.c_void_p(), C.c_void_p()
        _check(mesh_a.ctx._lib.pf_graph_build_device2(mesh_a._h, mesh_b._h, C.byref(ha), C.byref(hb)))
        return cls(_handle=(mesh_a.ctx, ha)), cls(_handle=(mesh_b.ctx, hb))

    def close(self):
        for rows in self._rows:
            rows.close()
        _Handle.close(self)
        self._final_out = None

    def download(self, labels=False):
        n, nnz = self.n, self.nnz_w
        out = dict(rowptr=np.empty(n + 1, np.int32), colidx=np.empty(nnz, np.int32), w=np.empty(nnz),
                   l_offdiag=np.empty(nnz), deg=np.empty(n), l_diag=np.empty(n))
        lab = np.empty(n, np.int32) if labels else None
        _check(self._lib.pf_graph_download(self._h, _ptr(out["rowptr"]), _ptr(out["colidx"]), _f64(out["w"]), _f64(out["l_offdiag"]),
                                           _f64(out["deg"]), _f64(out["l_diag"]), _ptr(lab)))
        if labels:
            out["labels"] = lab
        return out

    def cotan_download(self, w=True, diag=True, mass=True):
        out = {}
        if w:
            out["w"] = np.empty(self.nnz_w)
        if diag:
            out["diag"] = np.empty(self.n)
        if mass:
            out["mass"] = np.empty(self.n)
        _check(self._lib.pf_graph_cotan_download(self._h, *[_f64(out.get(k)) for k in ("w", "diag", "mass")]))
        return out

    def cotan_apply(self, x):
        v = _c_f64(x)
        v2 = v.reshape(self.n, -1)
        out = np.empty_like(v2)
        _check(self._lib.pf_cotan_apply(self._h, _f64(v2), v2.shape[1], _f64(out)))
        return out[:, 0] if v.ndim == 1 else out

    def ws_ensure(self, n_slots):
        _check(self._lib.pf_ws_ensure(self._h, int(n_slots)))

    def upload(self, slot, x):
        x = _c_f64(x, (self.n,))
        _check(self._lib.pf_ws_upload(self._h, int(slot), _f64(x)))

    def download_slots(self, first, count):
        out = np.empty((int(count), self.n), dtype=np.float64)
        _check(self._lib.pf_ws_download(self._h, int(first), int(count), _f64(out)))
        return out.T

    def copy(self, src, dst, count):
        _check(self._lib.pf_ws_copy(self._h, int(src), int(dst), int(count)))

    def mask_isolated(self, slot):
        _check(self._lib.pf_mask_isolated(self._h, int(slot)))

    def start_vector(self, slot, seed):
        _check(self._lib.pf_start_vector(self._h, int(slot), int(seed)))

    def lock_null_vectors(self):
        k = C.c_int32()
        _check(self._lib.pf_lock_null_vectors(self._h, self.op, C.byref(k)))
        return int(k.value)

    def spmv(self, src, dst):
        _check(self._lib.pf_spmv(self._h, self.op, int(src), int(dst)))

    def spmv_multi(self, src_first, dst_first, count):
        _check(self._lib.pf_spmv_multi(self._h, self.op, int(src_first), int(dst_first), int(count)))

    def cheb(self, src, dst, degree, c, e, rho=1.0):
        _check(self._lib.pf_cheb(self._h, self.op, int(src), int(dst), int(degree), float(c), float(e), float(rho)))

    def window_info(self, rings=False):
        n_max = int(self.info.n_pad) // 1024 + 1
        scalars = [C.c_int32() for _ in range(4)]
        ghosts, ghosts2, need = (np.full(n_max, -1, np.int32) for _ in range(3))
        _check(self._lib.pf_graph_window_info(self._h, int(bool(rings)), *[C.byref(s) for s in scalars],
                                              _ptr(ghosts), _ptr(ghosts2), _ptr(need)))
        win_rows, nw, state, state2 = (int(s.value) for s in scalars)
        return dict(win_rows=win_rows, n_windows=nw, state=state, state2=state2,
                    ghosts=ghosts[:nw].copy() if state == 1 else None, need=need[:nw].copy() if state == 1 else None,
                    ghosts2=ghosts2[:nw].copy() if state2 == 1 else None)

    def cheb2(self, req_self, other, req_other):
        a, b = req_self, req_other
        _check(self._lib.pf_cheb2(self._h, self.op, int(a[0]), int(a[1]), int(a[2]), float(a[3]), float(a[4]), float(a[5]),
                                  other._h, other.op, int(b[0]), int(b[1]), int(b[2]), float(b[3]), float(b[4]), float(b[5])))

    def dots(self, w, first, count):
        out = np.empty(int(count), dtype=np.float64)
        _check(self._lib.pf_dots(self._h, int(w), int(first), int(count), _f64(out)))
        return out

    def orth(self, w, first, count):
        h = np.empty(max(int(count), 1), dtype=np.float64)
        nrm = C.c_double()
        _check(self._lib.pf_orth(self._h, int(w), int(first), int(count), _f64(h), C.byref(nrm)))
        return h[: int(count)], float(nrm.value)

    def orth_begin(self, w, first, count, normalize=True):
        _check(self._lib.pf_orth_begin(self._h, int(w), int(first), int(count), int(bool(normalize))))
        self._orth_count = int(count)

    def orth_begin2(self, req, other, req_other):
        _check(self._lib.pf_orth_begin2(self._h, int(req[0]), int(req[1]), int(req[2]), int(bool(req[3])), other._h, int(req_other[0]),
                                        int(req_other[1]), int(req_other[2]), int(bool(req_other[3]))))
        self._orth_count, other._orth_count = int(req[2]), int(req_other[2])

    def orth_cheb2(self, orth, req, other, orth_other, req_other):
        o = (C.c_int32 * 8)(int(orth[0]), int(orth[1]), int(orth[2]), int(bool(orth[3])), int(orth_other[0]), int(orth_other[1]),
                            int(orth_other[2]), int(bool(orth_other[3])))
        ci = (C.c_int32 * 8)(self.op, int(req[0]), int(req[1]), int(req[2]), other.op, int(req_other[0]), int(req_other[1]),
                             int(req_other[2]))
        cd = (C.c_double * 6)(float(req[3]), float(req[4]), float(req[5]), float(req_other[3]), float(req_other[4]), float(req_other[5]))
        _check(self._lib.pf_orth_cheb2(self._h, other._h, o, ci, cd))
        self._orth_count, other._orth_count = int(orth[2]), int(orth_other[2])

    def orth_split(self, first2, split):
        _check(self._lib.pf_orth_split(self._h, int(first2), int(split)))

    def orth_strict(self, on):
        _check(self._lib.pf_orth_strict(self._h, 2 if on == 2 and on is not True else int(bool(on))))

    def orth_device_passes(self, on):
        _check(self._lib.pf_orth_device_passes(self._h, int(bool(on))))

    def orth_end(self):
        h = np.empty(max(self._orth_count, 1), dtype=np.float64)
        nrm = C.c_double()
        _check(self._lib.pf_orth_end(self._h, _f64(h), C.byref(nrm)))
        r = self._lib.pf_orth_redone(self._h)
        self.orth_redone = r == 1
        self.orth_twice = r == 2
        return h[: self._orth_count], float(nrm.value)

    def orth_abandon(self):
        try:
            self.orth_end()
        except PfError:
            pass

    def scale(self, slot, alpha):
        _check(self._lib.pf_scale(self._h, int(slot), float(alpha)))

    def combine(self, src_first, m, Y, dst_first):
        Y = _c_f64(Y)
        if Y.ndim != 2 or Y.shape[0] != m:
            raise ValueError("Y must be (m, k)")
        _check(self._lib.pf_combine(self._h, int(src_first), int(m), _f64(Y), Y.shape[1], int(dst_first)))

    def resnorm(self, ax, x, lam):
        out = C.c_double()
        _check(self._lib.pf_resnorm(self._h, int(ax), int(x), float(lam), C.byref(out)))
        return float(out.value)

    def gram(self, first_a, count_a, first_b, count_b):
        out = np.empty((int(count_a), int(count_b)), dtype=np.float64)
        _check(self._lib.pf_gram(self._h, int(first_a), int(count_a), int(first_b), int(count_b), _f64(out)))
        return out

    def resnorms(self, ax_first, x_first, lams):
        lams = _c_f64(lams)
        out = np.empty(len(lams), dtype=np.float64)
        _check(self._lib.pf_resnorms(self._h, int(ax_first), int(x_first), _f64(lams), len(lams), _f64(out)))
        return out

    def finalize_vectors(self, first, count, minmax, wait=True):
        out = pinned_empty((self.n, int(count)))
        _check(self._lib.pf_finalize_vectors_begin(self._h, int(first), int(count), int(self.op == PF_OP_SYM), int(bool(minmax)),
                                                   _f64(out)))
        self._final_count = int(count)
        self._final_pending = True
        self._final_out = out
        if wait:
            self.finalize_wait()
        return out

    def final_remap(self, cols, signs, out):
        cols = _c_i32(cols)
        signs = np.ascontiguousarray(signs, dtype=np.float64)
        assert out.flags.c_contiguous and out.shape == (self.n, len(cols))
        _check(self._lib.pf_final_remap_begin(self._h, _ptr(cols), _f64(signs), len(cols), _f64(out)))
        self._final_pending = True
        self._final_out = out

    def finalize_wait(self):
        if getattr(self, "_final_pending", False) and self._h:
            self._final_pending = False
            try:
                _check(self._lib.pf_finalize_vectors_end(self._h))
            finally:
                self._final_out = None

    def final_rows(self, rows):
        rows = _c_i64(rows)
        out = np.empty((len(rows), self._final_count), dtype=np.float64)
        _check(self._lib.pf_final_rows(self._h, _ptr(rows), len(rows), _f64(out)))
        return out

    def final_device(self):
        ptr, n_rows, n_cols = C.c_void_p(), C.c_int64(), C.c_int32()
        _check(self._lib.pf_final_device(self._h, C.byref(ptr), C.byref(n_rows), C.byref(n_cols)))
        return int(ptr.value), int(n_rows.value), int(n_cols.value)

    def point_rows(self, rows):
        rows = _c_i64(rows)
        out = np.empty((len(rows), 3), dtype=np.float64)
        _check(self._lib.pf_point_rows(self._h, _ptr(rows), len(rows), _f64(out)))
        return out

    def spmv_host(self, x, op=None):
        x = _c_f64(x, (self.n,))
        y = np.empty(self.n, dtype=np.float64)
        _check(self._lib.pf_spmv_host(self._h, self.op if op is None else int(op), _f64(x), _f64(y)))
        return y

    def eigs_smallest(self, n_wanted, minmax=False, wait=True):
        m = int(n_wanted)
        vals, vecs, resid, n_out, st = np.empty(m), pinned_empty((self.n, m)), np.zeros(m), C.c_int32(), EigsStats()
        _check(self._lib.pf_eigs_smallest_ex(self._h, m, int(bool(minmax)), 0 if wait else 1, _f64(vals), _f64(vecs), _f64(resid),
                                             C.byref(n_out), C.byref(st)))
        return self._eigs_result(vals, vecs, resid, n_out.value, st, wait)

    def _eigs_result(self, vals, vecs, resid, m, st, wait):
        self._final_count = m
        self._final_pending = (not wait) and m > 0
        self._final_out = vecs if self._final_pending else None
        if m != vecs.shape[1]:
            if self._final_pending:
                self.finalize_wait()
            vecs = np.ascontiguousarray(vecs.reshape(-1)[: self.n * m].reshape(self.n, m))
        stats = st.as_dict()
        stats["residuals"] = resid[:m].copy()
        return vals[:m].copy(), vecs, stats

    def eigs_smallest2(self, other, n_wanted, n_wanted_other, minmax=False, wait=True):
        outs = []
        for dev, m in ((self, int(n_wanted)), (other, int(n_wanted_other))):
            outs.append((np.empty(m), pinned_empty((dev.n, m)), np.zeros(m), C.c_int32(), EigsStats()))
        (va, xa, ra, na, sa), (vb, xb, rb, nb, sb) = outs
        _check(self._lib.pf_eigs_smallest2(self._h, other._h, int(n_wanted), int(n_wanted_other), int(bool(minmax)), 0 if wait else 1,
                                           _f64(va), _f64(xa), _f64(ra), C.byref(na), C.byref(sa),
                                           _f64(vb), _f64(xb), _f64(rb), C.byref(nb), C.byref(sb)))
        return tuple(dev._eigs_result(vals, vecs, resid, n_out.value, st, wait) for dev, (vals, vecs, resid, n_out, st) in zip((self, other), outs))

    def op_step(self, x, prev, out, alpha, c, beta, op=None):
        _check(self._lib.pf_op_step(self._h, self.op if op is None else int(op), int(x), -1 if prev is None else int(prev),
                                    int(out), float(alpha), float(c), float(beta)))

    def cheb_steps(self, prev, cur, k_first, n_steps, c, e, rho=1.0, op=None):
        op_, oc = C.c_int32(), C.c_int32()
        _check(self._lib.pf_cheb_steps(self._h, self.op if op is None else int(op), int(prev), int(cur), int(k_first),
                                       int(n_steps), float(c), float(e), float(rho), C.byref(op_), C.byref(oc)))
        return op_.value, oc.value

    def axpy(self, w, first, count, coef):
        coef = _c_f64(coef)
        _check(self._lib.pf_axpy(self._h, int(w), int(first), int(count), _f64(coef)))

    def rows_create(self, idx):
        rows = _Rows(self, idx)
        self._rows.append(rows)
        return rows

    def rows_gather(self, slot, rows):
        out = np.empty(rows.n)
        _check(self._lib.pf_rows_gather(rows._h, int(slot), _f64(out)))
        return out

    def rows_scatter(self, slot, rows, values):
        values = _c_f64(values, (rows.n,))
        _check(self._lib.pf_rows_scatter(rows._h, int(slot), _f64(values)))

    def rows_gather_dev(self, slot, rows, device_ptr):
        _check(self._lib.pf_rows_gather_dev(rows._h, int(slot), C.c_void_p(int(device_ptr))))

    def rows_scatter_dev(self, slot, rows, device_ptr):
        _check(self._lib.pf_rows_scatter_dev(rows._h, int(slot), C.c_void_p(int(device_ptr))))

    def rows_set_sources(self, rows, offsets):
        offsets = _c_i64(offsets)
        if len(offsets) != rows.n:
            raise ValueError("one offset per row")
        _check(self._lib.pf_rows_set_sources(rows._h, _ptr(offsets)))

    def rows_gather2_dev(self, slot_a, slot_b, rows, device_ptr, stride):
        _check(self._lib.pf_rows_gather2_dev(rows._h, int(slot_a), -1 if slot_b is None else int(slot_b),
                                             C.c_void_p(int(device_ptr)), int(stride)))

    def rows_scatter2_dev(self, slot_a, slot_b, rows, device_ptr, stride):
        _check(self._lib.pf_rows_scatter2_dev(rows._h, int(slot_a), -1 if slot_b is None else int(slot_b),
                                              C.c_void_p(int(device_ptr)), int(stride)))

    def sync(self):
        self.ctx.sync()

    def rows_fill(self, slot, rows, value):
        _check(self._lib.pf_rows_fill(rows._h, int(slot), float(value)))

    def mean_filter(self, values, iterations):
        v = _c_f64(values)
        one_d = v.ndim == 1
        v2 = v.reshape(self.n, -1)
        out = np.empty_like(v2)
        _check(self._lib.pf_mean_filter(self._h, _f64(v2), v2.shape[1], int(iterations), _f64(out)))
        return out[:, 0] if one_d else out
```

pyfocusr_amd/csrc/pf_eigsort.hip:

```cpp
#include <float.h>
#include <string.h>

#include <vector>

#include "pf_internal.h"

extern "C" int pf_knn1_blocks(pf_ctx* c, const double* ref_block, int64_t n_ref, int32_t ref_stride, const double* qry_block, int64_t n_qry,
                              int32_t qry_stride, int32_t d, const int32_t* col_ref, const double* scale_ref, const int32_t* col_qry,
                              const double* scale_qry, int64_t* idx_out, double* d2_out);

namespace {

constexpr int ES_SORT_THREADS = 1024;
constexpr int ES_MAX_SAMPLES = 16384;
constexpr int ES_RED_THREADS = 256;

__global__ __launch_bounds__(PF_BLOCK) void k_es_gather(const double* __restrict__ fin, int32_t fc, const double* __restrict__ pts,
                                                        const int64_t* __restrict__ rows, int64_t m, int32_t k,
                                                        const int32_t* __restrict__ col, const double* __restrict__ sign,
                                                        double* __restrict__ vals, double* __restrict__ raw) {
    const int64_t e = (int64_t)blockIdx.x * PF_BLOCK + threadIdx.x;
    if (e >= m * (k + 3)) return;
    const int64_t c = e / m, r = e - c * m;
    if (c < k) vals[c * m + r] = fin[rows[r] * fc + col[c]] * sign[c];
    else raw[r * 3 + (c - k)] = pts[rows[r] * 3 + (c - k)];
}

__global__ __launch_bounds__(ES_RED_THREADS) void k_es_minmax(const double* __restrict__ raw, int64_t m, double* __restrict__ lohi) {
    __shared__ double slo[ES_RED_THREADS], shi[ES_RED_THREADS];
    const int c = blockIdx.x;
    double lo = INFINITY, hi = -INFINITY;
    for (int64_t r = threadIdx.x; r < m; r += ES_RED_THREADS) {
        const double v = raw[r * 3 + c];
        lo = v < lo ? v : lo;
        hi = v > hi ? v : hi;
    }
    slo[threadIdx.x] = lo;
    shi[threadIdx.x] = hi;
    __syncthreads();
    for (int s = ES_RED_THREADS / 2; s > 0; s >>= 1) {
        if (threadIdx.x < s) {
            slo[threadIdx.x] = slo[threadIdx.x + s] < slo[threadIdx.x] ? slo[threadIdx.x + s] : slo[threadIdx.x];
            shi[threadIdx.x] = shi[threadIdx.x + s] > shi[threadIdx.x] ? shi[threadIdx.x + s] : shi[threadIdx.x];
        }
        __syncthreads();
    }
    if (threadIdx.x == 0) {
        lohi[c] = slo[0];
        lohi[3 + c] = shi[0];
    }
}

__global__ __launch_bounds__(PF_BLOCK) void k_es_normalize(const double* __restrict__ raw, const double* __restrict__ lohi, int64_t m,
                                                           double* __restrict__ out) {
    const int64_t e = (int64_t)blockIdx.x * PF_BLOCK + threadIdx.x;
    if (e >= m * 3) return;
    const int c = (int)(e % 3);
    out[e] = (raw[e] - lohi[c]) / (lohi[3 + c] - lohi[c]);
}

__global__ __launch_bounds__(ES_SORT_THREADS) void k_es_sort_log(const double* __restrict__ vals_t, const double* __restrict__ vals_s,
                                                                 int64_t mt, int64_t ms, int32_t k, double* __restrict__ lt,
                                                                 double* __restrict__ ls, double* __restrict__ lsf) {
    extern __shared__ double buf[];
    const int b = blockIdx.x;
    const int64_t m = b < k ? mt : ms;
    int n_pow2 = 2;
    while (n_pow2 < m) n_pow2 <<= 1;
    const double* src = b < k ? vals_t + (int64_t)b * m : vals_s + (int64_t)(b - k) * m;
    for (int i = threadIdx.x; i < n_pow2; i += ES_SORT_THREADS) buf[i] = i < m ? src[i] : INFINITY;
    __syncthreads();
    for (int size = 2; size <= n_pow2; size <<= 1) {
        for (int stride = size >> 1; stride > 0; stride >>= 1) {
            for (int t = threadIdx.x; t < n_pow2 / 2; t += ES_SORT_THREADS) {
                const int pos = 2 * t - (t & (stride - 1));
                const double a = buf[pos], c = buf[pos + stride];
                const bool up = (pos & size) == 0;
                if ((a > c) == up) {
                    buf[pos] = c;
                    buf[pos + stride] = a;
                }
            }
            __syncthreads();
        }
    }
    const double eps = DBL_EPSILON;
    if (b < k) {
        for (int64_t i = threadIdx.x; i < m; i += ES_SORT_THREADS) lt[(int64_t)b * m + i] = log(buf[i] + 0.5 + eps);
    } else {
        const int64_t o = (int64_t)(b - k) * m;
        for (int64_t i = threadIdx.x; i < m; i += ES_SORT_THREADS) {
            ls[o + i] = log(buf[i] + 0.5 + eps);
            lsf[o + i] = log(-buf[m - 1 - i] + 0.5 + eps);
        }
    }
}

__device__ __forceinline__ double es_block_sum(double v, double* sh) {
    sh[threadIdx.x] = v;
    __syncthreads();
    for (int s = ES_RED_THREADS / 2; s > 0; s >>= 1) {
        if (threadIdx.x < s) sh[threadIdx.x] += sh[threadIdx.x + s];
        __syncthreads();
    }
    const double r = sh[0];
    __syncthreads();
    return r;
}

__global__ __launch_bounds__(ES_RED_THREADS) void k_es_w1(const double* __restrict__ lt, const double* __restrict__ ls,
                                                          const double* __restrict__ lsf, int64_t mt, int64_t ms, int32_t k,
                                                          double* __restrict__ out) {
    __shared__ double sh[ES_RED_THREADS];
    const int i = blockIdx.x / k, j = blockIdx.x - i * k;
    const double unit = 1.0 / ((double)mt * (double)ms);
    double acc = 0.0, accf = 0.0;
    for (int64_t a = threadIdx.x; a < mt; a += ES_RED_THREADS) {
        const double t = lt[(int64_t)i * mt + a];
        const int64_t lo = a * ms, hi = lo + ms;
        for (int64_t b = lo / mt; b < ms && b * mt < hi; ++b) {
            const int64_t from = b * mt > lo ? b * mt : lo, to = (b + 1) * mt < hi ? (b + 1) * mt : hi;
            const double len = (double)(to - from) * unit;
            acc += len * fabs(t - ls[(int64_t)j * ms + b]);
            accf += len * fabs(t - lsf[(int64_t)j * ms + b]);
        }
    }
    acc = es_block_sum(acc, sh);
    accf = es_block_sum(accf, sh);
    if (threadIdx.x == 0) {
        out[i * k + j] = acc;
        out[k * k + i * k + j] = accf;
    }
}

__global__ __launch_bounds__(ES_RED_THREADS) void k_es_spatial(const double* __restrict__ vals_t, const double* __restrict__ vals_s,
                                                               const int64_t* __restrict__ idx, int64_t m, int64_t ms, int32_t k,
                                                               double* __restrict__ out) {
    __shared__ double sh[ES_RED_THREADS];
    const int i = blockIdx.x / k, j = blockIdx.x - i * k;
    double a = 0.0, f = 0.0;
    for (int64_t r = threadIdx.x; r < m; r += ES_RED_THREADS) {
        const int64_t nn = idx[r];
        const double t = vals_t[(int64_t)i * m + r], s = (nn >= 0 && nn < ms) ? vals_s[(int64_t)j * ms + nn] : NAN;
        const double d0 = s - t, d1 = -s - t;
        a += d0 * d0;
        f += d1 * d1;
    }
    a = es_block_sum(a, sh);
    f = es_block_sum(f, sh);
    if (threadIdx.x == 0) {
        out[2 * k * k + i * k + j] = sqrt(a) / (double)m;
        out[3 * k * k + i * k + j] = sqrt(f) / (double)m;
    }
}

}

extern "C" int pf_eigsort_costs(pf_graph* gt, pf_graph* gs, const int64_t* rows_t, int64_t mt, const int64_t* rows_s, int64_t ms, int32_t k,
                                const int32_t* col_t, const double* sign_t, const int32_t* col_s, const double* sign_s, double* out,
                                int64_t* idx_out) {
    PF_CHECK(gt && gs && rows_t && rows_s && col_t && sign_t && col_s && sign_s && out && idx_out, PF_E_ARG,
             "pf_eigsort_costs: NULL argument");
    PF_CHECK(gt->ctx == gs->ctx, PF_E_ARG, "pf_eigsort_costs: the two graphs must share one ctx");
    PF_CHECK(mt >= 1 && mt <= ES_MAX_SAMPLES && ms >= 1 && ms <= ES_MAX_SAMPLES && k >= 1 && k <= 16, PF_E_ARG,
             "pf_eigsort_costs: %lld / %lld samples (1..%d), k = %d (1..16)", (long long)mt, (long long)ms, ES_MAX_SAMPLES, k);
    PF_CHECK(gt->final_vecs && gs->final_vecs, PF_E_STATE, "pf_eigsort_costs: no pf_finalize_vectors result is resident");
    PF_CHECK(gt->pts && gs->pts, PF_E_STATE, "pf_eigsort_costs: the graphs were not built from meshes");
    for (int32_t c = 0; c < k; ++c)
        PF_CHECK(col_t[c] >= 0 && col_t[c] < gt->final_count && col_s[c] >= 0 && col_s[c] < gs->final_count, PF_E_ARG,
                 "pf_eigsort_costs: column out of range");
    for (int64_t r = 0; r < mt; ++r) PF_CHECK(rows_t[r] >= 0 && rows_t[r] < gt->n, PF_E_ARG, "pf_eigsort_costs: sample row out of range");
    for (int64_t r = 0; r < ms; ++r) PF_CHECK(rows_s[r] >= 0 && rows_s[r] < gs->n, PF_E_ARG, "pf_eigsort_costs: sample row out of range");
    pf_ctx* c = gt->ctx;
    PF_HIP(hipSetDevice(c->device));
    hipStream_t st = c->stream;
    int32_t n_pow2 = 2;
    while (n_pow2 < (mt > ms ? mt : ms)) n_pow2 <<= 1;
    const size_t sort_lds = sizeof(double) * (size_t)n_pow2;
    if (sort_lds > 64 * 1024)
        PF_HIP(hipFuncSetAttribute(reinterpret_cast<const void*>(k_es_sort_log), hipFuncAttributeMaxDynamicSharedMemorySize,
                                   (int)(sizeof(double) * ES_MAX_SAMPLES)));

    const size_t head = sizeof(int64_t) * (size_t)(mt + ms);
    const size_t small = ((sizeof(int32_t) * 2 * k + 7) & ~(size_t)7) + sizeof(double) * 2 * k;
    std::vector<unsigned char> host(head + small);
    memcpy(host.data(), rows_t, sizeof(int64_t) * (size_t)mt);
    memcpy(host.data() + sizeof(int64_t) * (size_t)mt, rows_s, sizeof(int64_t) * (size_t)ms);
    int32_t* hcol = reinterpret_cast<int32_t*>(host.data() + head);
    double* hsign = reinterpret_cast<double*>(host.data() + head + ((sizeof(int32_t) * 2 * k + 7) & ~(size_t)7));
    for (int32_t i = 0; i < k; ++i) {
        hcol[i] = col_t[i];
        hcol[k + i] = col_s[i];
        hsign[i] = sign_t[i];
        hsign[k + i] = sign_s[i];
    }
    const size_t kt = (size_t)k * (size_t)mt, ks = (size_t)k * (size_t)ms;
    const size_t doubles = 2 * kt + 3 * ks + 6 * (size_t)(mt + ms) + 12 + 4 * (size_t)k * k;
    unsigned char* d = nullptr;
    const size_t up_bytes = (host.size() + 7) & ~(size_t)7, out_bytes = sizeof(double) * 4 * (size_t)k * k;
    unsigned char* pin = nullptr;
    PF_TRY(pf_pinned_scratch(c, up_bytes + out_bytes, reinterpret_cast<void**>(&pin)));
    memcpy(pin, host.data(), host.size());
    PF_HIP(pf_malloc(st, (void**)&d, up_bytes + sizeof(double) * doubles));
    int rc = PF_OK;
    do {
        auto fail = [&](hipError_t e) {
            if (e == hipSuccess) return false;
            pf_set_error("pf_eigsort_costs: %s", hipGetErrorString(e));
            rc = PF_E_HIP;
            return true;
        };
        if ((rc = pf_copy_by_kernel(st, pin, d, up_bytes)) != PF_OK) break;
        const int64_t* d_rows_t = reinterpret_cast<const int64_t*>(d);
        const int64_t* d_rows_s = d_rows_t + mt;
        const int32_t* d_col = reinterpret_cast<const int32_t*>(d + head);
        const double* d_sign = reinterpret_cast<const double*>(d + head + ((sizeof(int32_t) * 2 * k + 7) & ~(size_t)7));
        double* base = reinterpret_cast<double*>(d + up_bytes);
        double* vals_t = base;
        double* vals_s = vals_t + kt;
        double* raw_t = vals_s + ks;
        double* raw_s = raw_t + 3 * mt;
        double* norm_t = raw_s + 3 * ms;
        double* norm_s = norm_t + 3 * mt;
        double* lohi = norm_s + 3 * ms;
        double* lt = lohi + 12;
        double* ls = lt + kt;
        double* lsf = ls + ks;
        double* d_out = lsf + ks;
        k_es_gather<<<pf_blocks(mt * (k + 3)), PF_BLOCK, 0, st>>>(gt->final_vecs, gt->final_count, gt->pts, d_rows_t, mt, k, d_col, d_sign,
                                                                  vals_t, raw_t);
        k_es_gather<<<pf_blocks(ms * (k + 3)), PF_BLOCK, 0, st>>>(gs->final_vecs, gs->final_count, gs->pts, d_rows_s, ms, k, d_col + k,
                                                                  d_sign + k, vals_s, raw_s);
        k_es_minmax<<<3, ES_RED_THREADS, 0, st>>>(raw_t, mt, lohi);
        k_es_minmax<<<3, ES_RED_THREADS, 0, st>>>(raw_s, ms, lohi + 6);
        k_es_normalize<<<pf_blocks(3 * mt), PF_BLOCK, 0, st>>>(raw_t, lohi, mt, norm_t);
        k_es_normalize<<<pf_blocks(3 * ms), PF_BLOCK, 0, st>>>(raw_s, lohi + 6, ms, norm_s);
        k_es_sort_log<<<(unsigned)(2 * k), ES_SORT_THREADS, sort_lds, st>>>(vals_t, vals_s, mt, ms, k, lt, ls, lsf);
        k_es_w1<<<(unsigned)(k * k), ES_RED_THREADS, 0, st>>>(lt, ls, lsf, mt, ms, k, d_out);
        if (fail(hipGetLastError())) break;
        const int32_t cols3[3] = {0, 1, 2};
        const double ones3[3] = {1.0, 1.0, 1.0};
        rc = pf_knn1_blocks(c, norm_s, ms, 3, norm_t, mt, 3, 3, cols3, ones3, cols3, ones3, idx_out, nullptr);
        if (rc != PF_OK) break;
        k_es_spatial<<<(unsigned)(k * k), ES_RED_THREADS, 0, st>>>(vals_t, vals_s, c->knn_idx.p, mt, ms, k, d_out);
        if (fail(hipGetLastError())) break;
        if ((rc = pf_copy_by_kernel(st, d_out, pin + up_bytes, out_bytes)) != PF_OK) break;
        if (fail(hipStreamSynchronize(st))) break;
        memcpy(out, pin + up_bytes, out_bytes);
    } while (0);
    if (rc != PF_OK) (void)hipStreamSynchronize(st);
    pf_free(st, d);
    return rc;
}
```

pyfocusr_amd/csrc/pf_internal.h:

```cpp
#pragma once
#include <hip/hip_runtime.h>
#include <stdint.h>
#include <atomic>
#include <map>
#include <mutex>
#include <type_traits>
#include <unordered_map>
#include <vector>

#include "../../include/pyfocusr_hip.h"
#include "pf_scratch.h"

void pf_set_error(const char* fmt, ...);

#define PF_HIP(call)                                                                          \
    do {                                                                                      \
        hipError_t e_ = (call);                                                               \
        if (e_ != hipSuccess) {                                                               \
            pf_set_error("%s:%d %s: %s", __FILE__, __LINE__, #call, hipGetErrorString(e_));   \
            (void)hipGetLastError();  \
            return PF_E_HIP;                                                                  \
        }                                                                                     \
    } while (0)

#define PF_CHECK(cond, code, ...)        \
    do {                                 \
        if (!(cond)) {                   \
            pf_set_error(__VA_ARGS__);   \
            return (code);               \
        }                                \
    } while (0)

#define PF_TRY(call)            \
    do {                        \
        int r_ = (call);        \
        if (r_ != PF_OK) return r_; \
    } while (0)

template <int LO, int HI, class F>
int pf_dispatch_d(int d, F&& f, const char* msg) {
    if constexpr (LO > HI) {
        pf_set_error(msg, d);
        return PF_E_ARG;
    } else {
        if (d == LO) return f(std::integral_constant<int, LO>{});
        return pf_dispatch_d<LO + 1, HI>(d, f, msg);
    }
}

constexpr int PF_WAVE = 64;
constexpr int PF_BLOCK = 256;
constexpr int PF_DOT_CHUNK = 4096;
constexpr int PF_MAX_ROOTS = 4096;
constexpr int PF_WIN_THREADS = 1024;
constexpr int PF_WIN_GHOSTS = 1024;
constexpr int PF_WIN_MAX = 1024;
constexpr int PF_WIN_G1 = 512;
constexpr int PF_WIN_GW = 16;
constexpr int PF_STAGE_SLOTS = 8;
constexpr size_t PF_STAGE_BYTES = 32768;
constexpr int PF_WS_TMPS = 4;

inline unsigned pf_blocks(int64_t n) { return (unsigned)((n + PF_BLOCK - 1) / PF_BLOCK); }

inline int pf_index_bits(int64_t count) {
    int b = 1;
    while (b < 62 && ((int64_t)1 << b) < count) ++b;
    return b;
}

inline int pf_check_faces(const char* fn, const int32_t* faces, int64_t n_faces, int32_t vpf, int64_t n, bool distinct) {
    for (int64_t i = 0; !distinct && i < n_faces * vpf; ++i)
        PF_CHECK(faces[i] >= 0 && faces[i] < n, PF_E_ARG, "%s: face %lld references vertex %d of %lld", fn, (long long)(i / vpf),
                 faces[i], (long long)n);
    for (int64_t t = 0; distinct && t < n_faces; ++t) {
        const int32_t* f = faces + 3 * t;
        for (int j = 0; j < 3; ++j)
            PF_CHECK(f[j] >= 0 && f[j] < n, PF_E_ARG, "%s: face %lld references vertex %d of %lld", fn, (long long)t, f[j], (long long)n);
        PF_CHECK(f[0] != f[1] && f[1] != f[2] && f[0] != f[2], PF_E_DEGENERATE, "%s: face %lld repeats a vertex", fn, (long long)t);
    }
    return PF_OK;
}

inline int pf_hip_failed(const char* fn, hipError_t e) {
    (void)hipGetLastError();
    pf_set_error("%s: %s", fn, hipGetErrorString(e));
    return PF_E_HIP;
}

struct pf_knn_tree {
    DevBuf<double> pts;
    DevBuf<int32_t> orig;
    DevBuf<double> leaf_lo;
    DevBuf<double> sup_lo;
    DevBuf<int32_t> qry_order;
    void* grid = nullptr;
    unsigned long long* counters = nullptr;
    bool count_visits = false;
};

struct pf_ctx {
    int device = 0;
    hipStream_t stream = nullptr;
    void* stage_ring = nullptr;
    hipEvent_t stage_ev[8] = {nullptr, nullptr, nullptr, nullptr, nullptr, nullptr, nullptr, nullptr};
    int stage_next = 0;
    hipStream_t copy_stream = nullptr;
    hipEvent_t ev0 = nullptr, ev1 = nullptr;
    bool timing = false;
    int timing_stride = 1;
    int64_t timing_count = 0;
    uint32_t* persist_sync = nullptr;
    int32_t* persist_abort = nullptr;
    void* persist_cal = nullptr;
    double op_ms = 0.0;
    int64_t op_launches = 0;
    double op_bytes = 0.0;
    double persist_ms = 0.0, persist_bytes = 0.0, persist_lds_bytes = 0.0;
    int64_t persist_launches = 0, persist_steps = 0;
    double knn_ms = 0.0;
    double build_ms = 0.0;
    bool build_pending = false;
    DevBuf<double> knn_ref;
    DevBuf<double> knn_qry;
    DevBuf<double> knn_ref_s;
    DevBuf<double> knn_ref_soa;
    int64_t knn_ref_ld = 0;
    DevBuf<double> knn_qry_s;
    DevBuf<unsigned> knn_ref_key;
    DevBuf<unsigned> knn_qry_key;
    DevBuf<int32_t> knn_cell_start;
    int knn_res = 0;
    void* knn_grid = nullptr;
    DevBuf<int32_t> knn_ref_orig;
    DevBuf<int32_t> knn_qry_orig;
    unsigned long long* knn_ext = nullptr;
    int64_t knn_nref = 0, knn_nqry = 0;
    int32_t knn_d = 0;
    int32_t knn_k = 1;
    DevBuf<int64_t> knn_idx;
    DevBuf<double> knn_d2;
    bool knn_ready = false, knn_done = false;
    pf_knn_tree knn_tree;
    bool knn_count_on = false;
    DevBuf<unsigned long long> knn_visited;
    int64_t knn_visited_waves = 0;
    unsigned long long* wide_count = nullptr;
    bool wide_count_on = false;
    int32_t knn_mode = 0;
    struct TimedSpan {
        hipEvent_t e0, e1;
        int64_t launches;
        double bytes;
        int64_t persist_steps;
        double lds_bytes;
    };
    std::vector<TimedSpan> spans_pending;
    std::vector<std::pair<hipEvent_t, hipEvent_t>> spans_free;
    HostPools pools;
    void* pinned_scratch = nullptr;
    size_t pinned_scratch_bytes = 0;
    std::multimap<size_t, void*> free_blocks;
    std::unordered_map<void*, size_t> live_blocks;
    std::mutex alloc_mutex;
    hipStream_t stream_b = nullptr;
    hipEvent_t poison_ev = nullptr;
    hipEvent_t join_ev = nullptr, fork_ev = nullptr;
    std::vector<pf_graph*> deferred;
    std::mutex deferred_mutex;
    int64_t alloc_misses = 0;
    void* pinned_scratch_b = nullptr;
    size_t pinned_scratch_b_bytes = 0;
    void* pinned_scratch_knn = nullptr;
    size_t pinned_scratch_knn_bytes = 0;
};

inline uint64_t pf_next_uid() {
    static std::atomic<uint64_t> next{1};
    return next.fetch_add(1);
}

struct pf_graph {
    hipStream_t side_stream = nullptr;
    uint64_t uid = pf_next_uid();
    pf_ctx* ctx = nullptr;
    int64_t n = 0, n_pad = 0, n_faces = 0;
    int32_t vpf = 0;
    int32_t* rowptr = nullptr;
    int32_t* col = nullptr;
    double* w = nullptr;
    int64_t nnz_w = 0;
    double* deg = nullptr;
    double* g = nullptr;
    double* sg = nullptr;
    int32_t* label = nullptr;
    int32_t* morder = nullptr;
    int32_t* mrank = nullptr;
    int32_t* perm_m = nullptr;
    int32_t* iperm_m = nullptr;
    int32_t* perm = nullptr;
    int32_t* iperm = nullptr;
    unsigned long long* order_bbox = nullptr;
    double* smooth = nullptr;
    DevBuf<double> stage;
    int64_t n_slices = 0, sell_entries = 0;
    int64_t* slice_ptr = nullptr;
    int32_t* scol = nullptr;
    double* sval_rw = nullptr;
    double* sval_sym = nullptr;
    double* diag = nullptr;
    int32_t* mf_col = nullptr;
    double* mf_val = nullptr;
    int32_t win_rows = 1024;
    std::vector<int64_t> h_slice_ptr;
    int32_t px_state = -1;
    HostLanding px_land;
    int32_t* px_slot = nullptr;
    int32_t* px_gh_cnt = nullptr;
    int32_t* px_gh_row = nullptr;
    int32_t* px_need = nullptr;
    std::vector<int32_t> h_px_gh_cnt;
    int64_t px_gh_total = 0;
    double* persist_ring = nullptr;
    int32_t persist_phase = 0;
    uint64_t persist_epoch = 0;
    int32_t px2_state = -1;
    int32_t* px_gh_cnt2 = nullptr;
    int32_t* px_need2 = nullptr;
    uint8_t* px_g1_w = nullptr;
    int32_t* px_g1_pos = nullptr;
    uint16_t* px_g1_slot = nullptr;
    int32_t* px_g1_gw = nullptr;
    std::vector<int32_t> h_px_gh_cnt2, h_px_g1_gw;
    int64_t px_gh2_total = 0, px_g1_entries = 0;
    int32_t single_applications = 0;
    uint64_t lds_need_partner = 0;
    int64_t lds_need_value = -2, lds_need2_value = -2;
    double* persist_ring2 = nullptr;
    int32_t persist_phase2 = 0;
    uint64_t persist_epoch2 = 0;
    int32_t is_symmetric = 0, n_isolated = 0, n_components = 0, max_degree = 0, n_oneway = 0;
    bool rows_compacted = false;
    int32_t unit_g = 0;
    std::vector<int32_t> roots;
    double* ws = nullptr;
    int32_t n_slots = 0;
    double* partials = nullptr;
    int32_t partial_cap = 0;
    double* coef = nullptr;
    int32_t coef_cap = 0;
    int64_t n_chunks = 0;
    HostLanding orth_land;
    int32_t orth_pending = -1;
    HostLanding small_land;
    int32_t small_pending = 0;
    bool small_root = false;
    hipEvent_t orth_wait = nullptr;
    int32_t orth_w = 0, orth_first = 0, orth_normalize = 0;
    int32_t orth_redone = 0;
    double orth_serial = 0.0;
    unsigned long long* orth_counter = nullptr;
    unsigned long long orth_arrivals = 0;
    uint64_t orth_epoch = 0;
    int32_t orth_split = -1, orth_first2 = 0;
    int32_t orth_split_now = -1, orth_first2_now = 0;
    double orth_ticket = 0.0;
    double orth_thresh = 0.09;
    int32_t orth_device_passes = 0;
    int32_t orth_twice = 0;
    double* final_vecs = nullptr;
    int32_t final_count = 0;
    int32_t final_pending = 0;
    double* final_params = nullptr;
    HostLanding final_land;
    hipEvent_t final_done = nullptr;
    const double* dl_src = nullptr;
    double* dl_dst = nullptr;
    size_t dl_bytes = 0;
    int32_t final_check = 0;
    double* final_tmp = nullptr;
    double* pts = nullptr;
    bool deg_block = false;
    double spectral_bound = 2.0;
    int32_t is_cotan = 0;
    double* cot_w = nullptr;
    double* cot_diag = nullptr;
    double* cot_mass = nullptr;
    double* cot_sqrtm = nullptr;
    double cot_hi = 0.0;
    double cot_area = 0.0;
};

struct pf_mesh {
    pf_ctx* ctx = nullptr;
    double* pts = nullptr;
    int32_t* faces = nullptr;
    int64_t n = 0, n_faces = 0;
    int32_t vpf = 0;
};

int pf_timing_collect(pf_ctx* c);
int pf_pinned_scratch(pf_ctx* c, size_t bytes, void** out, int which = 0);
int pf_copy_by_kernel(hipStream_t st, const void* src, void* dst, size_t bytes);
int pf_downloads_release(pf_ctx* c);
int pf_download_cancel(pf_graph* g);
hipStream_t pf_stream_b(pf_ctx* c);
hipError_t pf_create_side_stream(hipStream_t* s, bool low = false);

constexpr int PF_ND_MAX = 16;
struct TriHierarchy {
    double* tri = nullptr;
    int32_t* tri_orig = nullptr;
    double* box = nullptr;
    double* sbox = nullptr;
    int64_t n_tri = 0, n_chunks = 0, n_super = 0;
    int32_t d = 0;
};
struct KeyBox {
    double lo[3], ext[3];
    int32_t nk;
};
KeyBox pf_key_box(const double* pts, int64_t n, int32_t d, bool finite_only);
const int32_t* pf_surface_morton_order(Scratch& sc, const double* d_pts, int32_t d, const int32_t* d_faces, int32_t vpf, int64_t n,
                                       const KeyBox& bb);
void pf_tri_hierarchy_build(Scratch& sc, TriHierarchy& h, const double* d_pts, int32_t d, const int32_t* d_faces, int64_t n_faces,
                            int32_t vpf, const KeyBox& bb);
void pf_tri_hierarchy_free(hipStream_t st, TriHierarchy& h);

__host__ __device__ static inline int64_t pf_sell_index(int64_t base, int32_t width, int32_t j, int lane) {
    const int32_t pairs = width >> 1;
    return j < 2 * pairs ? base + (int64_t)(j >> 1) * (2 * PF_WAVE) + 2 * lane + (j & 1)
                         : base + (int64_t)pairs * (2 * PF_WAVE) + lane;
}

static inline double* pf_slot(pf_graph* g, int32_t s) { return g->ws + (int64_t)s * g->n_pad; }
static inline double* pf_tmp(pf_graph* g, int which) { return g->ws + (int64_t)(g->n_slots + which) * g->n_pad; }

int pf_graph_finish_general(pf_graph* g, const double* d_pts);

void pf_sort_pairs(Scratch& sc, const unsigned* k_in, unsigned* k_out, const int32_t* v_in, int32_t* v_out, int64_t n, int end_bit);
void pf_sort_pairs(Scratch& sc, const unsigned long long* k_in, unsigned long long* k_out, const int32_t* v_in, int32_t* v_out,
                   int64_t n, int end_bit);
inline void pf_sort_pairs(Scratch& sc, const unsigned long long* k_in, unsigned long long* k_out, const unsigned* v_in, unsigned* v_out,
                          int64_t n, int end_bit) {
    pf_sort_pairs(sc, k_in, k_out, (const int32_t*)v_in, (int32_t*)v_out, n, end_bit);
}

int pf_exclusive_scan_i32(hipStream_t st, const int32_t* in, int32_t* out, int64_t n);
int pf_exclusive_scan_i64(hipStream_t st, const int64_t* in, int64_t* out, int64_t n);

int pf_check_slots(pf_graph* g, int32_t first, int32_t count, const char* who);
const double* pf_op_values(pf_graph* g, int32_t op);
int64_t pf_op_bytes(const pf_graph* g);
int pf_launch_op(pf_graph* g, const double* vals, const double* x, const double* prev, double* out, double alpha, double shift,
                 double beta);
struct OpTimer {
    pf_ctx* c;
    int64_t launches;
    double bytes;
    bool on;
    int64_t persist_steps = 0;
    double lds_bytes = 0.0;
    hipEvent_t e0 = nullptr, e1 = nullptr;
    OpTimer(pf_ctx* ctx, int64_t n, double b);
    int finish();
};

constexpr size_t PF_PARTIAL_BYTES = 48;
int pf_reduce_ensure(pf_graph* g, int32_t count);
int pf_dots_device(pf_graph* g, int32_t w, int32_t first, int32_t count, double* d_out, double* d_acc, int accumulate);
int pf_dot_partials(pf_graph* g, int32_t w, int32_t first, int32_t count, double* partial);
int pf_scale_rsqrt(pf_graph* g, double* x, const double* nrm2);

int pf_multi_axpy(pf_graph* g, int32_t w, int32_t first, int32_t count, const double* d_h);

int pf_compute_order(pf_graph* g, const double* d_pts, int32_t* d_overflow = nullptr);
int pf_morton_order(pf_graph* g, const double* d_pts, int32_t* d_overflow);

static inline int32_t pf_window_rows(int64_t n_pad) { return n_pad <= 262144 ? 1024 : (n_pad <= 524288 ? 2048 : 4096); }

int pf_knn1_device(pf_ctx* c, const double* ref_block, int64_t n_ref, int32_t ref_stride, const double* qry_block, int64_t n_qry,
                   int32_t qry_stride, int32_t d);

int pf_knn_extent(hipStream_t st, const double* pts, int64_t n, int32_t d, unsigned long long* ext);

constexpr int PF_KNN_TREE_MIN_D = 7;
int pf_knn_tree_run(pf_ctx* c);

int pf_gram_begin(pf_graph* g, int32_t first_a, int32_t count_a, int32_t first_b, int32_t count_b, int32_t append);
int pf_resnorms_begin(pf_graph* g, int32_t ax_first, int32_t x_first, const double* lam, int32_t count);
int pf_small_end(pf_graph* g, double* out);
int pf_combine2(pf_graph* g, int32_t src_first, int32_t m, const double* Y, int32_t k, int32_t dst_first, int32_t src_first2,
                int32_t dst_first2);

struct pf_persist_args {
    pf_graph* g;
    const double* vals;
    const double* src;
    double* dst;
    int32_t degree;
    double c, e, rho;
};
int pf_persist_cheb(const pf_persist_args* a, const pf_persist_args* b , int* done, double* lds_bytes ,
                    bool first_try = true );
int pf_persist_ring_prefill(pf_graph* g, hipStream_t st);
int pf_persist_check(pf_ctx* ctx);
int pf_persist_set(int on);
void pf_persist_release(pf_ctx* ctx);
int pf_window_slots_prepare(pf_graph* g);
int pf_window_slots_begin(pf_graph* g);
bool pf_persist_enabled();
bool pf_persist_trusted();
uint64_t pf_persist_abort_epoch();
int pf_persist_sync_ensure(pf_ctx* ctx);
int pf_window_rings_prepare(pf_graph* g);
void pf_window_slots_free(pf_graph* g);
```

pyfocusr_amd/csrc/pf_knn.hip:

```cpp
#include <hipcub/hipcub.hpp>

#include <string.h>

#include <algorithm>

#include "pf_internal.h"
#include "pf_wave.h"

namespace {

constexpr int KNN_LDS_DOUBLES = 4096;

struct KnnGrid {
    int a0, a1;
    int r0, r1;
    double lo0, lo1;
    double s0, s1;
};

__device__ __forceinline__ int cell_of(double x, double lo, double scale, int r) {
    const double t = (x - lo) * scale;
    return t > 0.0 ? (t >= (double)r ? r - 1 : (int)t) : 0;
}

__global__ __launch_bounds__(PF_BLOCK) void k_extent(const double* __restrict__ pts, int64_t n, int d, unsigned long long* ext ) {
    __shared__ unsigned long long part[PF_BLOCK / PF_WAVE][32];
    const int wave = threadIdx.x / PF_WAVE;
    for (int a = 0; a < d; ++a) {
        unsigned long long lo = ~0ull, hi = 0ull;
        for (int64_t i = (int64_t)blockIdx.x * PF_BLOCK + threadIdx.x; i < n; i += (int64_t)gridDim.x * PF_BLOCK) {
            const unsigned long long e = enc_f64(pts[i * d + a]);
            lo = e < lo ? e : lo;
            hi = e > hi ? e : hi;
        }
        for (int off = PF_WAVE / 2; off > 0; off >>= 1) {
            const unsigned long long l2 = __shfl_xor(lo, off, PF_WAVE), h2 = __shfl_xor(hi, off, PF_WAVE);
            lo = l2 < lo ? l2 : lo;
            hi = h2 > hi ? h2 : hi;
        }
        if ((threadIdx.x & (PF_WAVE - 1)) == 0) {
            part[wave][a] = lo;
            part[wave][16 + a] = hi;
        }
    }
    __syncthreads();
    if ((int)threadIdx.x < 2 * d) {
        const bool is_hi = (int)threadIdx.x >= d;
        const int a = is_hi ? (int)threadIdx.x - d + 16 : (int)threadIdx.x;
        unsigned long long v = part[0][a];
        for (int w = 1; w < PF_BLOCK / PF_WAVE; ++w) {
            const unsigned long long o = part[w][a];
            v = is_hi ? (o > v ? o : v) : (o < v ? o : v);
        }
        if (is_hi)
            atomicMax(&ext[a], v);
        else
            atomicMin(&ext[a], v);
    }
}

__global__ void k_make_grid(const unsigned long long* __restrict__ ext, int d, int res, KnnGrid* g) {
    if (threadIdx.x | blockIdx.x) return;
    int b0 = 0, b1 = 0;
    double w0 = -1.0, w1 = -1.0;
    for (int a = 0; a < d; ++a) {
        const double e = dec_f64(ext[16 + a]) - dec_f64(ext[a]);
        if (e > w0) {
            w1 = w0;
            b1 = b0;
            w0 = e;
            b0 = a;
        } else if (e > w1) {
            w1 = e;
            b1 = a;
        }
    }
    if (d == 1) {
        b1 = b0;
        w1 = 0.0;
    }
    g->a0 = b0;
    g->a1 = b1;
    g->r0 = res;
    g->r1 = d == 1 ? 1 : res;
    g->lo0 = dec_f64(ext[b0]);
    g->lo1 = dec_f64(ext[b1]);
    g->s0 = (w0 > 0.0 && isfinite(w0)) ? (double)res / w0 : 0.0;
    g->s1 = (d > 1 && w1 > 0.0 && isfinite(w1)) ? (double)res / w1 : 0.0;
}

__device__ __forceinline__ unsigned spread16(unsigned v) {
    v &= 0xffffu;
    v = (v | (v << 8)) & 0x00ff00ffu;
    v = (v | (v << 4)) & 0x0f0f0f0fu;
    v = (v | (v << 2)) & 0x33333333u;
    v = (v | (v << 1)) & 0x55555555u;
    return v;
}

__global__ __launch_bounds__(PF_BLOCK) void k_cell_keys(const double* __restrict__ pts, int64_t n, int d,
                                                        const KnnGrid* __restrict__ gp, int morton, unsigned* __restrict__ keys,
                                                        int32_t* __restrict__ vals, int32_t* __restrict__ hist) {
    const int64_t i = (int64_t)blockIdx.x * PF_BLOCK + threadIdx.x;
    if (i >= n) return;
    const KnnGrid g = *gp;
    const int cx = cell_of(pts[i * d + g.a0], g.lo0, g.s0, g.r0);
    const int cy = cell_of(pts[i * d + g.a1], g.lo1, g.s1, g.r1);
    const unsigned key = morton ? (spread16((unsigned)cx) | (spread16((unsigned)cy) << 1)) : (unsigned)(cy * g.r0 + cx);
    keys[i] = key;
    if (hist) atomicAdd(&hist[key], 1);
    else vals[i] = (int32_t)i;
}

__global__ __launch_bounds__(PF_BLOCK) void k_gather_rows(const double* __restrict__ pts, const int32_t* __restrict__ order,
                                                          int64_t n, int d, double* __restrict__ out) {
    const int64_t i = (int64_t)blockIdx.x * PF_BLOCK + threadIdx.x;
    if (i >= n) return;
    const int64_t src = order[i];
    for (int c = 0; c < d; ++c) out[i * d + c] = pts[src * d + c];
}

__global__ __launch_bounds__(PF_BLOCK) void k_cell_start(const unsigned* __restrict__ keys, int64_t n, int64_t n_cells,
                                                         int32_t* __restrict__ cell_start) {
    const int64_t c = (int64_t)blockIdx.x * PF_BLOCK + threadIdx.x;
    if (c > n_cells) return;
    int64_t lo = 0, hi = n;
    while (lo < hi) {
        const int64_t mid = (lo + hi) >> 1;
        if ((int64_t)keys[mid] < c) lo = mid + 1; else hi = mid;
    }
    cell_start[c] = (int32_t)lo;
}

template <int D>
__device__ __forceinline__ double dist2(const double (&q)[D], const double* __restrict__ r) {
    double s = 0.0;
#pragma unroll
    for (int c = 0; c < D; ++c) {
        const double df = q[c] - r[c];
        const double sq = df * df;
        s = (c == 0) ? sq : s + sq;
    }
    return s;
}

template <int D, int P>
__device__ __forceinline__ double dist2_head(const double (&q)[D], const double* __restrict__ r) {
    double s = 0.0;
#pragma unroll
    for (int c = 0; c < P; ++c) {
        const double df = q[c] - r[c];
        const double sq = df * df;
        s = (c == 0) ? sq : s + sq;
    }
    return s;
}
template <int D, int P>
__device__ __forceinline__ double dist2_tail(const double (&q)[D], const double* __restrict__ r, double s) {
#pragma unroll
    for (int c = P; c < D; ++c) {
        const double df = q[c] - r[c];
        s = s + df * df;
    }
    return s;
}

template <int K>
__device__ __forceinline__ void topk_insert(double (&best)[K], int32_t (&bidx)[K], double s, int32_t o) {
    if (!(s < best[K - 1] || (s == best[K - 1] && o < bidx[K - 1]))) return;
    best[K - 1] = s;
    bidx[K - 1] = o;
#pragma unroll
    for (int j = K - 1; j > 0; --j) {
        const bool sw = best[j] < best[j - 1] || (best[j] == best[j - 1] && bidx[j] < bidx[j - 1]);
        const double ts = best[j - 1];
        const int32_t to = bidx[j - 1];
        best[j - 1] = sw ? best[j] : ts;
        bidx[j - 1] = sw ? bidx[j] : to;
        best[j] = sw ? ts : best[j];
        bidx[j] = sw ? to : bidx[j];
    }
}

template <int D, int K, int BS, int LANE_CELLS>
__global__ __launch_bounds__(BS) void k_knn_grid(const double* __restrict__ ref_s ,
                                                       const int32_t* __restrict__ ref_orig,
                                                       const int32_t* __restrict__ cell_start, int64_t n_ref,
                                                       const double* __restrict__ qry_s, const int32_t* __restrict__ qry_orig,
                                                       int64_t n_qry, const KnnGrid* __restrict__ gp,
                                                       int64_t* __restrict__ idx_out, double* __restrict__ d2_out) {
    constexpr int KNN_TILE = (BS >= 256 ? KNN_LDS_DOUBLES : KNN_LDS_DOUBLES / 4) / (D <= 8 ? 8 : 16);
    __shared__ double tile[KNN_TILE * D];
    __shared__ int32_t tile_idx[KNN_TILE];
    __shared__ int box[BS / PF_WAVE][4];
    const KnnGrid g = *gp;
    const int64_t qi = (int64_t)blockIdx.x * BS + threadIdx.x;
    const bool mine = qi < n_qry;
    const int64_t qq = mine ? qi : n_qry - 1;
    double q[D];
#pragma unroll
    for (int c = 0; c < D; ++c) q[c] = qry_s[qq * D + c];
    const double qx = qry_s[qq * D + g.a0], qy = qry_s[qq * D + g.a1];
    const int cx = cell_of(qx, g.lo0, g.s0, g.r0), cy = cell_of(qy, g.lo1, g.s1, g.r1);

    double bestk[K];
    int32_t bidx[K];
#pragma unroll
    for (int j = 0; j < K; ++j) {
        bestk[j] = INFINITY;
        bidx[j] = 0x7fffffff;
    }
    int rx0 = 0, rx1 = -1, ry0 = 0, ry1 = -1;
    for (int ring = 1; ring <= 4 && bestk[K - 1] == INFINITY; ++ring) {
#pragma unroll
        for (int j = 0; j < K; ++j) {
            bestk[j] = INFINITY;
            bidx[j] = 0x7fffffff;
        }
        const int y0 = cy - ring > 0 ? cy - ring : 0, y1 = cy + ring < g.r1 - 1 ? cy + ring : g.r1 - 1;
        const int x0 = cx - ring > 0 ? cx - ring : 0, x1 = cx + ring < g.r0 - 1 ? cx + ring : g.r0 - 1;
        rx0 = x0, rx1 = x1, ry0 = y0, ry1 = y1;
        for (int y = y0; y <= y1; ++y) {
            const int32_t b = cell_start[y * g.r0 + x0], e = cell_start[y * g.r0 + x1 + 1];
            for (int32_t r = b; r < e; ++r) {
                topk_insert<K>(bestk, bidx, dist2<D>(q, ref_s + (int64_t)r * D), ref_orig[r]);
            }
        }
    }
    auto block_rectangle = [&](int& bx0, int& bx1, int& by0, int& by1) {
        const double best = bestk[K - 1];
        const double rad = sqrt(best) * (1.0 + 1e-9) + 1e-300;
        double xl = qx - rad, xh = qx + rad, yl = qy - rad, yh = qy + rad;
        xl -= fabs(xl) * 1e-15;
        xh += fabs(xh) * 1e-15;
        yl -= fabs(yl) * 1e-15;
        yh += fabs(yh) * 1e-15;
        bx0 = cell_of(xl, g.lo0, g.s0, g.r0), bx1 = cell_of(xh, g.lo0, g.s0, g.r0);
        by0 = cell_of(yl, g.lo1, g.s1, g.r1), by1 = cell_of(yh, g.lo1, g.s1, g.r1);
        if (!(best < INFINITY)) {
            bx0 = 0;
            by0 = 0;
            bx1 = g.r0 - 1;
            by1 = g.r1 - 1;
        }
#pragma unroll
        for (int off = PF_WAVE / 2; off > 0; off >>= 1) {
            bx0 = min(bx0, __shfl_xor(bx0, off, PF_WAVE));
            by0 = min(by0, __shfl_xor(by0, off, PF_WAVE));
            bx1 = max(bx1, __shfl_xor(bx1, off, PF_WAVE));
            by1 = max(by1, __shfl_xor(by1, off, PF_WAVE));
        }
        __syncthreads();
        if ((threadIdx.x & (PF_WAVE - 1)) == 0) {
            int* b = box[threadIdx.x / PF_WAVE];
            b[0] = bx0;
            b[1] = bx1;
            b[2] = by0;
            b[3] = by1;
        }
        __syncthreads();
#pragma unroll
        for (int w = 0; w < BS / PF_WAVE; ++w) {
            bx0 = min(bx0, box[w][0]);
            bx1 = max(bx1, box[w][1]);
            by0 = min(by0, box[w][2]);
            by1 = max(by1, box[w][3]);
        }
    };
    {
        const double best = bestk[K - 1];
        const double rad = sqrt(best) * (1.0 + 1e-9) + 1e-300;
        double xl = qx - rad, xh = qx + rad, yl = qy - rad, yh = qy + rad;
        xl -= fabs(xl) * 1e-15;
        xh += fabs(xh) * 1e-15;
        yl -= fabs(yl) * 1e-15;
        yh += fabs(yh) * 1e-15;
        int lx0 = cell_of(xl, g.lo0, g.s0, g.r0), lx1 = cell_of(xh, g.lo0, g.s0, g.r0);
        int ly0 = cell_of(yl, g.lo1, g.s1, g.r1), ly1 = cell_of(yh, g.lo1, g.s1, g.r1);
        const bool bounded = best < INFINITY;
        const int cells = bounded ? (lx1 - lx0 + 1) * (ly1 - ly0 + 1) : 0x7fffffff;
        if (!__syncthreads_or(cells > LANE_CELLS)) {
            if (!(lx0 >= rx0 && lx1 <= rx1 && ly0 >= ry0 && ly1 <= ry1)) {
                for (int y = ly0; y <= ly1; ++y) {
                    const int32_t b = cell_start[y * g.r0 + lx0], e = cell_start[y * g.r0 + lx1 + 1];
                    for (int32_t r = b; r < e; ++r) {
                        const double s = dist2<D>(q, ref_s + (int64_t)r * D);
                        if (s <= bestk[K - 1]) {
                            const int32_t o = ref_orig[r];
                            bool seen = false;
#pragma unroll
                            for (int j = 0; j < K; ++j) seen |= (bidx[j] == o);
                            if (!seen) topk_insert<K>(bestk, bidx, s, o);
                        }
                    }
                }
            }
            if (mine) {
                const int64_t dst = qry_orig[qi];
#pragma unroll
                for (int j = 0; j < K; ++j) {
                    idx_out[dst * K + j] = bidx[j];
                    d2_out[dst * K + j] = bestk[j];
                }
            }
            return;
        }
    }
    int bx0, bx1, by0, by1;
    block_rectangle(bx0, bx1, by0, by1);

    const int mid = (by0 + by1) / 2;
    const int half = max(mid - by0, by1 - mid);
    int since_refresh = 0;
    for (int t = 0; t <= 2 * half; ++t) {
        const int y = (t & 1) ? mid + (t + 1) / 2 : mid - t / 2;
        if (y < by0 || y > by1) continue;
        const int32_t run_b = cell_start[y * g.r0 + bx0], run_e = cell_start[y * g.r0 + bx1 + 1];
        for (int32_t t0 = run_b; t0 < run_e; t0 += KNN_TILE) {
            const int cnt = (run_e - t0) < KNN_TILE ? (run_e - t0) : KNN_TILE;
            __syncthreads();
            for (int k = threadIdx.x; k < cnt * D; k += BS) tile[k] = ref_s[(int64_t)t0 * D + k];
            for (int k = threadIdx.x; k < cnt; k += BS) tile_idx[k] = ref_orig[t0 + k];
            __syncthreads();
            for (int r = 0; r < cnt; ++r) {
                double s;
                if constexpr (D >= 6) {
                    constexpr int P = D / 2;
                    s = dist2_head<D, P>(q, tile + r * D);
                    if (!__any(s <= bestk[K - 1])) continue;
                    s = dist2_tail<D, P>(q, tile + r * D, s);
                } else {
                    s = dist2<D>(q, tile + r * D);
                }
                if (s <= bestk[K - 1]) {
                    const int32_t o = tile_idx[r];
                    bool seen = false;
#pragma unroll
                    for (int j = 0; j < K; ++j) seen |= (bidx[j] == o);
                    if (!seen) topk_insert<K>(bestk, bidx, s, o);
                }
            }
        }
        since_refresh += run_e - run_b;
        if (since_refresh >= 4 * KNN_TILE && by1 - by0 >= 8) {
            since_refresh = 0;
            int nx0, nx1, ny0, ny1;
            block_rectangle(nx0, nx1, ny0, ny1);
            bx0 = max(bx0, nx0);
            bx1 = min(bx1, nx1);
            by0 = max(by0, ny0);
            by1 = min(by1, ny1);
        }
    }
    if (mine) {
        const int64_t dst = qry_orig[qi];
#pragma unroll
        for (int j = 0; j < K; ++j) {
            idx_out[dst * K + j] = bidx[j];
            d2_out[dst * K + j] = bestk[j];
        }
    }
}

constexpr int knn_group(int d) { return d <= 4 ? 8 : (d <= 8 ? 4 : 2); }

template <int D, bool COUNT = false>
__global__ __launch_bounds__(PF_BLOCK) void k_knn_coop(const double* __restrict__ soa, int64_t ld, const int32_t* __restrict__ ref_orig,
                                                       const int32_t* __restrict__ cell_start, const double* __restrict__ qry_s,
                                                       const int32_t* __restrict__ qry_orig, int64_t n_qry,
                                                       const KnnGrid* __restrict__ gp, int64_t* __restrict__ idx_out,
                                                       double* __restrict__ d2_out, unsigned long long* __restrict__ visited = nullptr) {
    constexpr int G = knn_group(D);
    unsigned long long seen = 0;
    const unsigned long long t_begin = COUNT ? __builtin_amdgcn_s_memrealtime() : 0ull;
    unsigned long long n_chunks = 0, n_scans = 0, t_scan = 0, t_bounds = 0, n_pass = 0;
    const KnnGrid g = *gp;
    const int lane = threadIdx.x & (PF_WAVE - 1);
    const int64_t group = (int64_t)blockIdx.x * (PF_BLOCK / PF_WAVE) + __builtin_amdgcn_readfirstlane((int)(threadIdx.x / PF_WAVE));
    const int64_t q0 = group * G;
    if (q0 >= n_qry) return;
    const int nq = n_qry - q0 < G ? (int)(n_qry - q0) : G;
    double q[G][D];
    double qx[G], qy[G];
    double best[G];
    int32_t bidx[G];
    int ux0 = 0x7fffffff, ux1 = -1, uy0 = 0x7fffffff, uy1 = -1;
#pragma unroll
    for (int i = 0; i < G; ++i) {
        const int64_t qi = q0 + (i < nq ? i : nq - 1);
#pragma unroll
        for (int c = 0; c < D; ++c) q[i][c] = qry_s[qi * D + c];
        qx[i] = qry_s[qi * D + g.a0];
        qy[i] = qry_s[qi * D + g.a1];
        const int cx = cell_of(qx[i], g.lo0, g.s0, g.r0), cy = cell_of(qy[i], g.lo1, g.s1, g.r1);
        ux0 = min(ux0, cx), ux1 = max(ux1, cx);
        uy0 = min(uy0, cy), uy1 = max(uy1, cy);
        best[i] = INFINITY;
        bidx[i] = 0x7fffffff;
    }
    auto scan_rows = [&](int row_of, int x0, int x1) {
        int32_t b_l = 0, e_l = 0;
        if (row_of >= 0) {
            b_l = cell_start[row_of * g.r0 + x0];
            e_l = cell_start[row_of * g.r0 + x1 + 1];
        }
        int32_t inc = (e_l - b_l + PF_WAVE - 1) >> 6;
#pragma unroll
        for (int off = 1; off < PF_WAVE; off <<= 1) {
            const int32_t up = __shfl_up(inc, off, PF_WAVE);
            if (lane >= off) inc += up;
        }
        const int32_t total = __builtin_amdgcn_readlane(inc, PF_WAVE - 1);
        if constexpr (COUNT) n_chunks += (unsigned long long)total, n_scans += 1ull;
        for (int32_t j = 0; j < total; ++j) {
            const int row = (int)__popcll(__ballot(inc <= j));
            const int32_t first = row > 0 ? __builtin_amdgcn_readlane(inc, row - 1) : 0;
            const int32_t r = __builtin_amdgcn_readlane(b_l, row) + (j - first) * PF_WAVE + lane;
            if constexpr (COUNT) seen += (unsigned long long)__popcll(__ballot(r < __builtin_amdgcn_readlane(e_l, row)));
            if (r < __builtin_amdgcn_readlane(e_l, row)) {
                double x[D];
#pragma unroll
                for (int c = 0; c < D; ++c) x[c] = soa[(int64_t)c * ld + r];
                const int32_t o = ref_orig[r];
                if constexpr (COUNT) {
                    bool pass = false;
#pragma unroll
                    for (int i = 0; i < G; ++i) {
                        double s3 = 0.0;
#pragma unroll
                        for (int c = 0; c < D; ++c)
                            if (c != g.a0 && c != g.a1) s3 += (q[i][c] - x[c]) * (q[i][c] - x[c]);
                        pass = pass || s3 <= best[i];
                    }
                    n_pass += (unsigned long long)__popcll(__ballot(pass));
                }
#pragma unroll
                for (int i = 0; i < G; ++i) {
                    double s = 0.0;
                    constexpr int P = D >= 6 ? D / 2 : D;
#pragma unroll
                    for (int c = 0; c < P; ++c) {
                        const double df = q[i][c] - x[c];
                        const double sq = df * df;
                        s = (c == 0) ? sq : s + sq;
                    }
                    if constexpr (P < D) {
                        if (!__any(s <= best[i])) continue;
#pragma unroll
                        for (int c = P; c < D; ++c) {
                            const double df = q[i][c] - x[c];
                            s = s + df * df;
                        }
                    }
                    if (s < best[i] || (s == best[i] && o < bidx[i])) {
                        best[i] = s;
                        bidx[i] = o;
                    }
                }
            }
        }
    };
    auto bounds = [&](int& bx0, int& bx1, int& by0, int& by1) -> bool {
        bool all = true;
        bx0 = 0x7fffffff, bx1 = -1, by0 = 0x7fffffff, by1 = -1;
#pragma unroll
        for (int i = 0; i < G; ++i) {
            wave_argmin(best[i], bidx[i]);
            all = all && best[i] < INFINITY;
            const double rad = sqrt(best[i]) * (1.0 + 1e-9) + 1e-300;
            double xl = qx[i] - rad, xh = qx[i] + rad, yl = qy[i] - rad, yh = qy[i] + rad;
            xl -= fabs(xl) * 1e-15;
            xh += fabs(xh) * 1e-15;
            yl -= fabs(yl) * 1e-15;
            yh += fabs(yh) * 1e-15;
            bx0 = min(bx0, cell_of(xl, g.lo0, g.s0, g.r0)), bx1 = max(bx1, cell_of(xh, g.lo0, g.s0, g.r0));
            by0 = min(by0, cell_of(yl, g.lo1, g.s1, g.r1)), by1 = max(by1, cell_of(yh, g.lo1, g.s1, g.r1));
        }
        if (!all) bx0 = 0, by0 = 0, bx1 = g.r0 - 1, by1 = g.r1 - 1;
        return all;
    };
    int x0 = 0, x1 = -1, y0 = 0, y1 = -1;
    int rx0 = 0, rx1 = -1, ry0 = 0, ry1 = -1;
    for (int ring = 1; ring <= 4; ++ring) {
        rx0 = max(ux0 - ring, 0), rx1 = min(ux1 + ring, g.r0 - 1);
        ry0 = max(uy0 - ring, 0), ry1 = min(uy1 + ring, g.r1 - 1);
        unsigned long long ta = COUNT ? __builtin_amdgcn_s_memrealtime() : 0ull;
        for (int yb = ry0; yb <= ry1; yb += PF_WAVE) scan_rows(yb + lane <= ry1 ? yb + lane : -1, rx0, rx1);
        unsigned long long tb = COUNT ? __builtin_amdgcn_s_memrealtime() : 0ull;
        const bool all_bounded = bounds(x0, x1, y0, y1);
        if constexpr (COUNT) t_scan += tb - ta, t_bounds += __builtin_amdgcn_s_memrealtime() - tb;
        if (all_bounded) break;
    }
    if (!(x0 >= rx0 && x1 <= rx1 && y0 >= ry0 && y1 <= ry1)) {
        const int mid = min(max((uy0 + uy1) / 2, y0), y1);
        int lo = mid, hi = mid - 1;
        int w = 4;
        while (lo > y0 || hi < y1) {
            const int na = max(min(w, y1 - hi), 0), nb = max(min(w, lo - y0), 0);
            unsigned long long ta = COUNT ? __builtin_amdgcn_s_memrealtime() : 0ull;
            scan_rows(lane < na ? hi + 1 + lane : (lane < na + nb ? lo - 1 - (lane - na) : -1), x0, x1);
            unsigned long long tb = COUNT ? __builtin_amdgcn_s_memrealtime() : 0ull;
            hi += na;
            lo -= nb;
            w = min(2 * w, PF_WAVE / 2);
            int nx0, nx1, ny0, ny1;
            bounds(nx0, nx1, ny0, ny1);
            if constexpr (COUNT) t_scan += tb - ta, t_bounds += __builtin_amdgcn_s_memrealtime() - tb;
            x0 = max(x0, nx0), x1 = min(x1, nx1);
            y0 = max(y0, ny0), y1 = min(y1, ny1);
        }
    }
#pragma unroll
    for (int i = 0; i < G; ++i) {
        if (lane == i && i < nq) {
            const int64_t dst = qry_orig[q0 + i];
            idx_out[dst] = bidx[i];
            d2_out[dst] = best[i];
        }
    }
    if constexpr (COUNT) {
        if (lane == 0 && visited) {
            atomicAdd(visited, seen * (unsigned long long)nq);
            unsigned long long* rec = visited + 8 + 8 * group;
            rec[0] = __builtin_amdgcn_s_memrealtime() - t_begin;
            rec[1] = seen;
            rec[2] = n_chunks;
            rec[3] = n_scans;
            rec[4] = t_scan;
            rec[5] = t_bounds;
            rec[6] = n_pass;
        }
    }
}

constexpr int64_t PF_KNN_SMALL = 16384;
constexpr int knn_small_group(int d) { return d <= 4 ? 8 : 4; }

template <int D>
__global__ __launch_bounds__(PF_BLOCK) void k_knn_small(const double* __restrict__ ref, int64_t n_ref, const double* __restrict__ qry,
                                                        int64_t n_qry, int64_t* __restrict__ idx_out, double* __restrict__ d2_out) {
    constexpr int G = knn_small_group(D);
    const int lane = threadIdx.x & (PF_WAVE - 1);
    const int64_t group = (int64_t)blockIdx.x * (PF_BLOCK / PF_WAVE) + __builtin_amdgcn_readfirstlane((int)(threadIdx.x / PF_WAVE));
    const int64_t q0 = group * G;
    if (q0 >= n_qry) return;
    const int nq = n_qry - q0 < G ? (int)(n_qry - q0) : G;
    double q[G][D], best[G];
    int32_t bidx[G];
#pragma unroll
    for (int i = 0; i < G; ++i) {
        const int64_t qi = q0 + (i < nq ? i : nq - 1);
#pragma unroll
        for (int c = 0; c < D; ++c) q[i][c] = qry[qi * D + c];
        best[i] = INFINITY;
        bidx[i] = 0x7fffffff;
    }
    for (int64_t r = lane; r < n_ref; r += PF_WAVE) {
        double x[D];
#pragma unroll
        for (int c = 0; c < D; ++c) x[c] = ref[r * D + c];
#pragma unroll
        for (int i = 0; i < G; ++i) {
            double s = 0.0;
#pragma unroll
            for (int c = 0; c < D; ++c) {
                const double df = q[i][c] - x[c];
                const double sq = df * df;
                s = (c == 0) ? sq : s + sq;
            }
            if (s < best[i]) {
                best[i] = s;
                bidx[i] = (int32_t)r;
            }
        }
    }
#pragma unroll
    for (int i = 0; i < G; ++i) {
        wave_argmin(best[i], bidx[i]);
        if (lane == i && i < nq) {
            idx_out[q0 + i] = bidx[i];
            d2_out[q0 + i] = best[i];
        }
    }
}

template <int D>
static int launch_knn_small(pf_ctx* c) {
    const int64_t groups = (c->knn_nqry + knn_small_group(D) - 1) / knn_small_group(D);
    k_knn_small<D><<<(unsigned)((groups + PF_BLOCK / PF_WAVE - 1) / (PF_BLOCK / PF_WAVE)), PF_BLOCK, 0, c->stream>>>(
        c->knn_ref.p, c->knn_nref, c->knn_qry.p, c->knn_nqry, c->knn_idx.p, c->knn_d2.p);
    PF_HIP(hipGetLastError());
    return PF_OK;
}

__global__ __launch_bounds__(PF_BLOCK) void k_gather_rows_soa(const double* __restrict__ pts, const int32_t* __restrict__ order,
                                                              int64_t n, int d, int64_t ld, double* __restrict__ out) {
    const int64_t i = (int64_t)blockIdx.x * PF_BLOCK + threadIdx.x;
    if (i >= n) return;
    const int64_t src = order[i];
    for (int c = 0; c < d; ++c) out[(int64_t)c * ld + i] = pts[src * d + c];
}

template <int D, int K>
int launch_knn_k(pf_ctx* c) {
    constexpr int BS = D <= 6 ? PF_WAVE : PF_BLOCK;
    if constexpr (K == 1 && D <= 9) {
        const int64_t waves = (c->knn_nqry + knn_group(D) - 1) / knn_group(D);
        if (c->knn_count_on) {
            const int64_t words = 8 + 8 * waves;
            PF_HIP(c->knn_visited.grow(c->stream, words));
            c->knn_visited_waves = waves;
            PF_HIP(hipMemsetAsync(c->knn_visited.p, 0, words * sizeof(unsigned long long), c->stream));
            k_knn_coop<D, true><<<(unsigned)((waves + PF_BLOCK / PF_WAVE - 1) / (PF_BLOCK / PF_WAVE)), PF_BLOCK, 0, c->stream>>>(
                c->knn_ref_soa.p, c->knn_ref_ld, c->knn_ref_orig.p, c->knn_cell_start.p, c->knn_qry_s.p, c->knn_qry_orig.p, c->knn_nqry,
                (const KnnGrid*)c->knn_grid, c->knn_idx.p, c->knn_d2.p, c->knn_visited.p);
        } else {
            k_knn_coop<D><<<(unsigned)((waves + PF_BLOCK / PF_WAVE - 1) / (PF_BLOCK / PF_WAVE)), PF_BLOCK, 0, c->stream>>>(
                c->knn_ref_soa.p, c->knn_ref_ld, c->knn_ref_orig.p, c->knn_cell_start.p, c->knn_qry_s.p, c->knn_qry_orig.p, c->knn_nqry,
                (const KnnGrid*)c->knn_grid, c->knn_idx.p, c->knn_d2.p);
        }
    } else {
        k_knn_grid<D, K, BS, 512><<<(unsigned)((c->knn_nqry + BS - 1) / BS), BS, 0, c->stream>>>(
            c->knn_ref_s.p, c->knn_ref_orig.p, c->knn_cell_start.p, c->knn_nref, c->knn_qry_s.p, c->knn_qry_orig.p, c->knn_nqry,
            (const KnnGrid*)c->knn_grid, c->knn_idx.p, c->knn_d2.p);
    }
    PF_HIP(hipGetLastError());
    return PF_OK;
}

template <int D>
int launch_knn(pf_ctx* c) {
    if (c->knn_k == 1) return launch_knn_k<D, 1>(c);
    if constexpr (D <= 4) {
        if (c->knn_k == 2) return launch_knn_k<D, 2>(c);
        if (c->knn_k == 3) return launch_knn_k<D, 3>(c);
        if (c->knn_k == 4) return launch_knn_k<D, 4>(c);
    }
    pf_set_error("pf_knn: k = %d with d = %d is not supported (k <= 4 needs d <= 4)", c->knn_k, D);
    return PF_E_ARG;
}

__global__ __launch_bounds__(PF_BLOCK) void k_bucket_scatter(const unsigned* __restrict__ keys, int64_t n, const int32_t* __restrict__ start,
                                                             int32_t* __restrict__ cursor, unsigned* __restrict__ key_out,
                                                             int32_t* __restrict__ orig_out, const double* __restrict__ pts, int d,
                                                             double* __restrict__ rows_out) {
    const int64_t i = (int64_t)blockIdx.x * PF_BLOCK + threadIdx.x;
    if (i >= n) return;
    const unsigned k = keys[i];
    const int64_t pos = start[k] + atomicAdd(&cursor[k], 1);
    key_out[pos] = k;
    orig_out[pos] = (int32_t)i;
    for (int c = 0; c < d; ++c) rows_out[pos * d + c] = pts[i * d + c];
}

int sort_points(pf_ctx* c, const double* pts, int64_t n, int d, int morton, int key_bits, unsigned* key_out, int32_t* orig_out,
                double* rows_out) {
    Scratch s(c->stream);
    unsigned* k0 = s.get<unsigned>(n);
    int64_t n_buckets = 1;
    {
        const int res = c->knn_res;
        if (morton) {
            int bits = 0;
            while ((1 << bits) < res) ++bits;
            n_buckets = (int64_t)1 << (2 * bits);
        } else {
            n_buckets = d == 1 ? res : (int64_t)res * res;
        }
    }
    int64_t bucket_max = (int64_t)1 << 22;
    if (const char* ev = getenv("PF_KNN_BUCKET_MAX")) bucket_max = atoll(ev);
    if (n_buckets <= bucket_max) {
        int32_t* hist = s.get<int32_t>(3 * n_buckets + 2);
        s.zero(hist, sizeof(int32_t) * (size_t)(3 * n_buckets + 2));
        if (s.ok()) {
            int32_t* start = hist + n_buckets + 1;
            int32_t* cursor = start + n_buckets + 1;
            k_cell_keys<<<pf_blocks(n), PF_BLOCK, 0, s.st>>>(pts, n, d, (const KnnGrid*)c->knn_grid, morton, k0, nullptr, hist);
            s.launched();
            if (s.ok() && pf_exclusive_scan_i32(s.st, hist, start, n_buckets + 1) != PF_OK) s.note(hipErrorUnknown);
            if (s.ok()) {
                k_bucket_scatter<<<pf_blocks(n), PF_BLOCK, 0, s.st>>>(k0, n, start, cursor, key_out, orig_out, pts, d, rows_out);
                s.launched();
            }
        }
    } else {
        int32_t* v0 = s.get<int32_t>(n);
        if (s.ok()) {
            k_cell_keys<<<pf_blocks(n), PF_BLOCK, 0, s.st>>>(pts, n, d, (const KnnGrid*)c->knn_grid, morton, k0, v0, nullptr);
            s.launched();
        }
        pf_sort_pairs(s, k0, key_out, v0, orig_out, n, key_bits);
        if (s.ok()) {
            k_gather_rows<<<pf_blocks(n), PF_BLOCK, 0, s.st>>>(pts, orig_out, n, d, rows_out);
            s.launched();
        }
    }
    PF_CHECK(s.ok(), PF_E_HIP, "pf_knn: %s", hipGetErrorString(s.err));
    return PF_OK;
}

}

extern "C" {

static int knn_prepare(pf_ctx* c, int64_t n_ref, int64_t n_qry, int32_t d, int32_t k) {
    PF_CHECK(c != nullptr, PF_E_ARG, "pf_knn_upload: ctx is NULL");
    PF_CHECK(k >= 1 && k <= 4 && k <= n_ref, PF_E_ARG, "pf_knn: k = %d out of range (1..4, <= n_ref)", k);
    PF_CHECK(n_ref > 0 && n_ref < ((int64_t)1 << 31) && n_qry > 0 && n_qry < ((int64_t)1 << 31) && d >= 1 && d <= 16, PF_E_ARG,
             "pf_knn_upload: n_ref %lld, n_qry %lld, d %d out of range (1 <= d <= 16)", (long long)n_ref, (long long)n_qry, d);
    PF_HIP(hipSetDevice(c->device));
    hipStream_t st = c->stream;
    c->knn_ready = c->knn_done = false;
    PF_HIP(c->knn_ref.grow(st, n_ref * 16));
    PF_HIP(c->knn_ref_s.grow(st, n_ref * 16));
    PF_HIP(c->knn_ref_key.grow(st, n_ref));
    c->knn_ref_ld = (n_ref + PF_WAVE - 1) & ~(int64_t)(PF_WAVE - 1);
    PF_HIP(c->knn_ref_soa.grow(st, c->knn_ref_ld * d));
    static const double per_cell = [] { const char* e = getenv("PF_KNN_PER_CELL"); const double v = e ? atof(e) : 0.0; return v > 0.0 ? v : 4.0; }();
    int res = (int)sqrt((double)n_ref / per_cell);
    res = res < 4 ? 4 : (res > 2048 ? 2048 : res);
    c->knn_res = res;
    PF_HIP(c->knn_cell_start.grow(st, (int64_t)res * res + 2));
    PF_HIP(c->knn_ref_orig.grow(st, n_ref));
    PF_HIP(c->knn_qry.grow(st, n_qry * 16));
    PF_HIP(c->knn_qry_s.grow(st, n_qry * 16));
    PF_HIP(c->knn_qry_key.grow(st, n_qry));
    PF_HIP(c->knn_qry_orig.grow(st, n_qry));
    PF_HIP(c->knn_idx.grow(st, n_qry * k));
    PF_HIP(c->knn_d2.grow(st, n_qry * k));
    c->knn_k = k;
    Scratch once(st);
    if (!c->knn_ext) c->knn_ext = once.keep<unsigned long long>(32);
    if (!c->knn_grid) c->knn_grid = once.keep<KnnGrid>(1);
    PF_HIP(once.err);
    c->knn_nref = n_ref;
    c->knn_nqry = n_qry;
    c->knn_d = d;
    return PF_OK;
}

struct CoordMap {
    int32_t col[16];
    double scale[16];
};
__global__ __launch_bounds__(PF_BLOCK) void k_coords_from_final(const double* __restrict__ fin, int64_t n, int32_t fc, int32_t d,
                                                                CoordMap m, double* __restrict__ out) {
    const int64_t e = (int64_t)blockIdx.x * PF_BLOCK + threadIdx.x;
    if (e >= n * d) return;
    const int64_t i = e / d;
    const int32_t c = (int32_t)(e - i * d);
    out[e] = fin[i * fc + m.col[c]] * m.scale[c];
}

static int knn_upload_k(pf_ctx* c, const double* ref, int64_t n_ref, const double* qry, int64_t n_qry, int32_t d, int32_t k) {
    PF_CHECK(c && ref && qry, PF_E_ARG, "pf_knn_upload: NULL argument");
    PF_TRY(knn_prepare(c, n_ref, n_qry, d, k));
    hipStream_t st = c->stream;
    PF_HIP(hipMemcpyAsync(c->knn_ref.p, ref, sizeof(double) * n_ref * d, hipMemcpyHostToDevice, st));
    PF_HIP(hipMemcpyAsync(c->knn_qry.p, qry, sizeof(double) * n_qry * d, hipMemcpyHostToDevice, st));
    PF_HIP(hipStreamSynchronize(st));
    c->knn_ready = true;
    return PF_OK;
}

int pf_knn_upload(pf_ctx* c, const double* ref, int64_t n_ref, const double* qry, int64_t n_qry, int32_t d) {
    return knn_upload_k(c, ref, n_ref, qry, n_qry, d, 1);
}

static int knn_search(pf_ctx* c) {
    hipStream_t st = c->stream;
    const int d = c->knn_d;
    const char* bad_d = "pf_knn_run: no search for d = %d";
    if (c->knn_k == 1 && c->knn_mode == 0 && d <= 8 && c->knn_nref <= PF_KNN_SMALL && c->knn_nqry <= PF_KNN_SMALL)
        return pf_dispatch_d<1, 8>(d, [&](auto D) { return launch_knn_small<D()>(c); }, bad_d);
    PF_TRY(pf_knn_extent(st, c->knn_ref.p, c->knn_nref, d, c->knn_ext));
    if (c->knn_k == 1 && (c->knn_mode == 2 || (c->knn_mode == 0 && d >= PF_KNN_TREE_MIN_D))) {
        if (c->knn_nqry >= 32768) PF_TRY(pf_downloads_release(c));
        return pf_knn_tree_run(c);
    }
    const int res = c->knn_res;
    const int64_t n_cells = d == 1 ? res : (int64_t)res * res;
    int cell_bits = 1;
    while (((int64_t)1 << cell_bits) < n_cells) ++cell_bits;
    k_make_grid<<<1, 1, 0, st>>>(c->knn_ext, d, res, (KnnGrid*)c->knn_grid);
    PF_HIP(hipGetLastError());
    PF_TRY(sort_points(c, c->knn_ref.p, c->knn_nref, d, 0, cell_bits, c->knn_ref_key.p, c->knn_ref_orig.p, c->knn_ref_s.p));
    k_cell_start<<<pf_blocks(n_cells + 1), PF_BLOCK, 0, st>>>(c->knn_ref_key.p, c->knn_nref, n_cells, c->knn_cell_start.p);
    PF_HIP(hipGetLastError());
    if (c->knn_k == 1) {
        k_gather_rows_soa<<<pf_blocks(c->knn_nref), PF_BLOCK, 0, st>>>(c->knn_ref.p, c->knn_ref_orig.p, c->knn_nref, d, c->knn_ref_ld, c->knn_ref_soa.p);
        PF_HIP(hipGetLastError());
    }
    PF_TRY(sort_points(c, c->knn_qry.p, c->knn_nqry, d, 1, 32, c->knn_qry_key.p, c->knn_qry_orig.p, c->knn_qry_s.p));
    if (c->knn_nqry >= 32768) PF_TRY(pf_downloads_release(c));
    return pf_dispatch_d<1, 16>(d, [&](auto D) { return launch_knn<D()>(c); }, bad_d);
}

int pf_knn_run(pf_ctx* c) {
    PF_CHECK(c != nullptr, PF_E_ARG, "pf_knn_run: ctx is NULL");
    PF_CHECK(c->knn_ready, PF_E_STATE, "pf_knn_run: no uploaded problem");
    PF_HIP(hipSetDevice(c->device));
    PF_HIP(hipEventRecord(c->ev0, c->stream));
    PF_TRY(knn_search(c));
    PF_HIP(hipEventRecord(c->ev1, c->stream));
    PF_HIP(hipEventSynchronize(c->ev1));
    float ms = 0.f;
    PF_HIP(hipEventElapsedTime(&ms, c->ev0, c->ev1));
    c->knn_ms = ms;
    c->knn_done = true;
    return PF_OK;
}

int pf_knn_count(pf_ctx* c, int32_t enable_counting, int64_t* pairs) {
    PF_CHECK(c != nullptr, PF_E_ARG, "pf_knn_count: ctx is NULL");
    unsigned long long h = 0ull;
    if (c->knn_visited.p) {
        PF_HIP(hipMemcpyAsync(&h, c->knn_visited.p, sizeof(h), hipMemcpyDeviceToHost, c->stream));
        PF_HIP(hipStreamSynchronize(c->stream));
    }
    if (pairs) *pairs = (int64_t)h;
    c->knn_count_on = enable_counting != 0;
    return PF_OK;
}

int pf_knn_wave_stats(pf_ctx* c, double* sum_us, double* max_us, int64_t* waves, int64_t* max_candidates, double* detail ) {
    PF_CHECK(c != nullptr, PF_E_ARG, "pf_knn_wave_stats: ctx is NULL");
    const int64_t nw = c->knn_visited.p ? c->knn_visited_waves : 0;
    std::vector<unsigned long long> h((size_t)(8 * nw), 0ull);
    if (nw > 0) {
        PF_HIP(hipMemcpyAsync(h.data(), c->knn_visited.p + 8, sizeof(unsigned long long) * h.size(), hipMemcpyDeviceToHost, c->stream));
        PF_HIP(hipStreamSynchronize(c->stream));
    }
    unsigned long long sum = 0, mx = 0, mc = 0, ch = 0, sc = 0, ts = 0, tb = 0, np = 0;
    for (int64_t w = 0; w < nw; ++w) {
        const unsigned long long* r = h.data() + 8 * w;
        sum += r[0];
        if (r[0] > mx) mx = r[0], mc = r[1];
        ch += r[2], sc += r[3], ts += r[4], tb += r[5], np += r[6];
    }
    if (sum_us) *sum_us = 0.01 * (double)sum;
    if (max_us) *max_us = 0.01 * (double)mx;
    if (waves) *waves = nw;
    if (max_candidates) *max_candidates = (int64_t)mc;
    if (detail) detail[0] = (double)ch, detail[1] = (double)sc, detail[2] = 0.01 * (double)ts, detail[3] = 0.01 * (double)tb, detail[4] = (double)np;
    return PF_OK;
}

int pf_knn_mode(pf_ctx* c, int32_t mode) {
    PF_CHECK(c != nullptr && mode >= 0 && mode <= 2, PF_E_ARG, "pf_knn_mode: bad argument");
    c->knn_mode = mode;
    return PF_OK;
}

int pf_knn_download(pf_ctx* c, int64_t* idx_out, double* d2_out) {
    PF_CHECK(c != nullptr && idx_out != nullptr, PF_E_ARG, "pf_knn_download: NULL argument");
    PF_CHECK(c->knn_done, PF_E_STATE, "pf_knn_download: pf_knn_run has not completed");
    PF_HIP(hipSetDevice(c->device));
    const size_t count = (size_t)c->knn_nqry * c->knn_k;
    const size_t bytes = sizeof(int64_t) * count;
    if (bytes * (d2_out ? 2 : 1) <= ((size_t)8 << 20)) {
        unsigned char* pin = nullptr;
        PF_TRY(pf_pinned_scratch(c, bytes * (d2_out ? 2 : 1), reinterpret_cast<void**>(&pin), 2));
        PF_TRY(pf_copy_by_kernel(c->stream, c->knn_idx.p, pin, bytes));
        if (d2_out) PF_TRY(pf_copy_by_kernel(c->stream, c->knn_d2.p, pin + bytes, bytes));
        PF_HIP(hipStreamSynchronize(c->stream));
        memcpy(idx_out, pin, bytes);
        if (d2_out) memcpy(d2_out, pin + bytes, bytes);
        return PF_OK;
    }
    PF_HIP(hipMemcpyAsync(idx_out, c->knn_idx.p, bytes, hipMemcpyDeviceToHost, c->stream));
    if (d2_out) PF_HIP(hipMemcpyAsync(d2_out, c->knn_d2.p, sizeof(double) * count, hipMemcpyDeviceToHost, c->stream));
    PF_HIP(hipStreamSynchronize(c->stream));
    return PF_OK;
}

int pf_knn(pf_ctx* c, const double* ref, int64_t n_ref, const double* qry, int64_t n_qry, int32_t d, int32_t k,
           int64_t* idx_out, double* d2_out) {
    PF_TRY(knn_upload_k(c, ref, n_ref, qry, n_qry, d, k));
    PF_TRY(pf_knn_run(c));
    return pf_knn_download(c, idx_out, d2_out);
}

int pf_knn1(pf_ctx* c, const double* ref, int64_t n_ref, const double* qry, int64_t n_qry, int32_t d, int64_t* idx_out,
            double* d2_out) {
    PF_TRY(pf_knn_upload(c, ref, n_ref, qry, n_qry, d));
    PF_TRY(pf_knn_run(c));
    return pf_knn_download(c, idx_out, d2_out);
}

static int knn1_blocks_run(pf_ctx* c, const double* ref_block, int64_t n_ref, int32_t ref_stride, const double* qry_block, int64_t n_qry,
                           int32_t qry_stride, int32_t d, const int32_t* col_ref, const double* scale_ref, const int32_t* col_qry,
                           const double* scale_qry) {
    PF_TRY(knn_prepare(c, n_ref, n_qry, d, 1));
    hipStream_t st = c->stream;
    CoordMap mr{}, mq{};
    for (int32_t k = 0; k < d; ++k) {
        mr.col[k] = col_ref[k], mr.scale[k] = scale_ref[k];
        mq.col[k] = col_qry[k], mq.scale[k] = scale_qry[k];
    }
    k_coords_from_final<<<pf_blocks(n_ref * d), PF_BLOCK, 0, st>>>(ref_block, n_ref, ref_stride, d, mr, c->knn_ref.p);
    k_coords_from_final<<<pf_blocks(n_qry * d), PF_BLOCK, 0, st>>>(qry_block, n_qry, qry_stride, d, mq, c->knn_qry.p);
    PF_HIP(hipGetLastError());
    c->knn_ready = true;
    return pf_knn_run(c);
}

int pf_knn1_blocks(pf_ctx* c, const double* ref_block, int64_t n_ref, int32_t ref_stride, const double* qry_block, int64_t n_qry,
                   int32_t qry_stride, int32_t d, const int32_t* col_ref, const double* scale_ref, const int32_t* col_qry,
                   const double* scale_qry, int64_t* idx_out, double* d2_out) {
    PF_CHECK(c && ref_block && qry_block && col_ref && scale_ref && col_qry && scale_qry && idx_out, PF_E_ARG,
             "pf_knn1_blocks: NULL argument");
    PF_CHECK(d >= 1 && d <= 16 && ref_stride >= 1 && qry_stride >= 1, PF_E_ARG, "pf_knn1_blocks: d = %d / strides out of range", d);
    for (int32_t k = 0; k < d; ++k)
        PF_CHECK(col_ref[k] >= 0 && col_ref[k] < ref_stride && col_qry[k] >= 0 && col_qry[k] < qry_stride, PF_E_ARG,
                 "pf_knn1_blocks: column %d out of range", k);
    PF_TRY(knn1_blocks_run(c, ref_block, n_ref, ref_stride, qry_block, n_qry, qry_stride, d, col_ref, scale_ref, col_qry, scale_qry));
    return pf_knn_download(c, idx_out, d2_out);
}

int pf_knn1_graphs(pf_graph* ref_g, pf_graph* qry_g, int32_t d, const int32_t* col_ref, const double* scale_ref,
                   const int32_t* col_qry, const double* scale_qry, int64_t* idx_out, double* d2_out) {
    PF_CHECK(ref_g && qry_g, PF_E_ARG, "pf_knn1_graphs: NULL argument");
    PF_CHECK(ref_g->ctx == qry_g->ctx, PF_E_ARG, "pf_knn1_graphs: the two graphs must share one ctx");
    PF_CHECK(ref_g->final_vecs && qry_g->final_vecs, PF_E_STATE, "pf_knn1_graphs: no pf_finalize_vectors result is resident");
    return pf_knn1_blocks(ref_g->ctx, ref_g->final_vecs, ref_g->n, ref_g->final_count, qry_g->final_vecs, qry_g->n, qry_g->final_count, d,
                          col_ref, scale_ref, col_qry, scale_qry, idx_out, d2_out);
}

int pf_final_device(pf_graph* g, double** block, int64_t* n_rows, int32_t* n_cols) {
    PF_CHECK(g && block && n_rows && n_cols, PF_E_ARG, "pf_final_device: NULL argument");
    PF_CHECK(g->final_vecs != nullptr, PF_E_STATE, "pf_final_device: no pf_finalize_vectors result is resident");
    *block = g->final_vecs;
    *n_rows = g->n;
    *n_cols = g->final_count;
    return PF_OK;
}

}

int pf_knn_extent(hipStream_t st, const double* pts, int64_t n, int32_t d, unsigned long long* ext) {
    PF_HIP(hipMemsetAsync(ext, 0xff, 16 * sizeof(unsigned long long), st));
    PF_HIP(hipMemsetAsync(ext + 16, 0x00, 16 * sizeof(unsigned long long), st));
    k_extent<<<256, PF_BLOCK, 0, st>>>(pts, n, d, ext);
    return PF_OK;
}

int pf_knn1_device(pf_ctx* c, const double* ref_block, int64_t n_ref, int32_t ref_stride, const double* qry_block, int64_t n_qry,
                   int32_t qry_stride, int32_t d) {
    PF_CHECK(c && ref_block && qry_block && d >= 1 && d <= 16 && d <= ref_stride && d <= qry_stride, PF_E_ARG, "pf_knn1_device: bad argument");
    int32_t col[16];
    double one[16];
    for (int32_t k = 0; k < 16; ++k) col[k] = k, one[k] = 1.0;
    return knn1_blocks_run(c, ref_block, n_ref, ref_stride, qry_block, n_qry, qry_stride, d, col, one, col, one);
}
```

pyfocusr_amd/csrc/pf_scan.hip:

```cpp
#include "pf_internal.h"
#include "pf_launch.h"

namespace {

constexpr int SCAN_ITEMS = 8;
constexpr int SCAN_TILE = PF_BLOCK * SCAN_ITEMS;

template <typename T>
__device__ __forceinline__ T wave_inclusive_scan(T v, int lane) {
#pragma unroll
    for (int off = 1; off < PF_WAVE; off <<= 1) {
        T up = __shfl_up(v, off, PF_WAVE);
        if (lane >= off) v += up;
    }
    return v;
}

template <typename T>
__device__ __forceinline__ T block_exclusive_scan(T v, T* total) {
    __shared__ T wave_sum[PF_BLOCK / PF_WAVE];
    const int lane = threadIdx.x & (PF_WAVE - 1);
    const int wid = threadIdx.x / PF_WAVE;
    T inc = wave_inclusive_scan(v, lane);
    if (lane == PF_WAVE - 1) wave_sum[wid] = inc;
    __syncthreads();
    T offset = 0, all = 0;
#pragma unroll
    for (int wv = 0; wv < PF_BLOCK / PF_WAVE; ++wv) {
        T s = wave_sum[wv];
        if (wv < wid) offset += s;
        all += s;
    }
    __syncthreads();
    *total = all;
    return offset + inc - v;
}

template <typename T>
struct scan_block_totals {
    static constexpr int BOUNDS = PF_BLOCK;
    static __device__ __forceinline__ void run(const T* __restrict__ in, T* __restrict__ totals, int64_t n) {
    const int64_t base = (int64_t)blockIdx.x * SCAN_TILE + (int64_t)threadIdx.x * SCAN_ITEMS;
    T s = 0;
#pragma unroll
    for (int k = 0; k < SCAN_ITEMS; ++k) {
        int64_t i = base + k;
        if (i < n) s += in[i];
    }
    T total;
    (void)block_exclusive_scan(s, &total);
    if (threadIdx.x == 0) totals[blockIdx.x] = total;
}
};

template <typename T>
struct scan_block_apply {
    static constexpr int BOUNDS = PF_BLOCK;
    static __device__ __forceinline__ void run(const T* __restrict__ in, T* __restrict__ out,
                                                             const T* __restrict__ block_offset, int64_t n) {
    const int64_t base = (int64_t)blockIdx.x * SCAN_TILE + (int64_t)threadIdx.x * SCAN_ITEMS;
    T v[SCAN_ITEMS];
    T s = 0;
#pragma unroll
    for (int k = 0; k < SCAN_ITEMS; ++k) {
        int64_t i = base + k;
        v[k] = (i < n) ? in[i] : T(0);
        s += v[k];
    }
    T total;
    T run = block_exclusive_scan(s, &total) + (block_offset ? block_offset[blockIdx.x] : T(0));
#pragma unroll
    for (int k = 0; k < SCAN_ITEMS; ++k) {
        int64_t i = base + k;
        if (i < n) out[i] = run;
        run += v[k];
    }
}
};

constexpr int64_t SCAN_DIRECT_BLOCKS = 4096;
template <typename T>
struct scan_block_apply_direct {
    static constexpr int BOUNDS = PF_BLOCK;
    static __device__ __forceinline__ void run(const T* __restrict__ in, T* __restrict__ out,
                                                                    const T* __restrict__ totals, int64_t n) {
    __shared__ T s_off;
    T mine = 0;
    for (int64_t b = threadIdx.x; b < blockIdx.x; b += PF_BLOCK) mine += totals[b];
    T before;
    (void)block_exclusive_scan(mine, &before);
    if (threadIdx.x == 0) s_off = before;
    __syncthreads();
    const int64_t base = (int64_t)blockIdx.x * SCAN_TILE + (int64_t)threadIdx.x * SCAN_ITEMS;
    T v[SCAN_ITEMS];
    T s = 0;
#pragma unroll
    for (int k = 0; k < SCAN_ITEMS; ++k) {
        int64_t i = base + k;
        v[k] = (i < n) ? in[i] : T(0);
        s += v[k];
    }
    T total;
    T run = block_exclusive_scan(s, &total) + s_off;
#pragma unroll
    for (int k = 0; k < SCAN_ITEMS; ++k) {
        int64_t i = base + k;
        if (i < n) out[i] = run;
        run += v[k];
    }
}
};

template <typename T>
int exclusive_scan(hipStream_t st, const T* in, T* out, int64_t n) {
    if (n <= 0) return PF_OK;
    const int64_t blocks = (n + SCAN_TILE - 1) / SCAN_TILE;
    if (blocks == 1) {
        pfl::launch<scan_block_apply<T>>(dim3(1), dim3(PF_BLOCK), 0, st, in, out, nullptr, n);
        PF_HIP(hipGetLastError());
        return PF_OK;
    }
    T* totals = nullptr;
    PF_HIP(pf_malloc(st, (void**)&totals, sizeof(T) * blocks));
    pfl::launch<scan_block_totals<T>>(dim3((unsigned)blocks), dim3(PF_BLOCK), 0, st, in, totals, n);
    PF_HIP(hipGetLastError());
    int r = PF_OK;
    if (blocks <= SCAN_DIRECT_BLOCKS) {
        pfl::launch<scan_block_apply_direct<T>>(dim3((unsigned)blocks), dim3(PF_BLOCK), 0, st, in, out, totals, n);
        if (hipGetLastError() != hipSuccess) r = PF_E_HIP;
    } else {
        r = exclusive_scan<T>(st, totals, totals, blocks);
        if (r == PF_OK) {
            pfl::launch<scan_block_apply<T>>(dim3((unsigned)blocks), dim3(PF_BLOCK), 0, st, in, out, totals, n);
            if (hipGetLastError() != hipSuccess) r = PF_E_HIP;
        }
    }
    pf_free(st, totals);
    return r;
}

}

int pf_exclusive_scan_i32(hipStream_t st, const int32_t* in, int32_t* out, int64_t n) {
    return exclusive_scan<int32_t>(st, in, out, n);
}
int pf_exclusive_scan_i64(hipStream_t st, const int64_t* in, int64_t* out, int64_t n) {
    return exclusive_scan<int64_t>(st, in, out, n);
}
```

Before: 1018.

## Fork eigsort histogram and KNN query sort onto a second stream

Result: faster. 1030, median of 6 (+1.2%).

```diff
diff --git a/include/pyfocusr_hip.h b/include/pyfocusr_hip.h
--- a/include/pyfocusr_hip.h
+++ b/include/pyfocusr_hip.h
@@ -96,6 +96,7 @@
 int pf_persist_enable(int on);
 int pf_persist_two_step(int level);
 int pf_persist_pair_halves(int on);
+int pf_back_fork(int on);
 int pf_persist_clock(pf_ctx* ctx, double* kernel_ms, int64_t* launches, int reset);
 typedef struct pf_persist_info {
     int32_t enabled;
diff --git a/pyfocusr_amd/_hip.py b/pyfocusr_amd/_hip.py
--- a/pyfocusr_amd/_hip.py
+++ b/pyfocusr_amd/_hip.py
@@ -100,6 +100,7 @@
     "pf_persist_enable": (C.c_int, [C.c_int]),
     "pf_persist_two_step": (C.c_int, [C.c_int]),
     "pf_persist_pair_halves": (C.c_int, [C.c_int]),
+    "pf_back_fork": (C.c_int, [C.c_int]),
     "pf_persist_clock": (C.c_int, [C.c_void_p, C.POINTER(C.c_double), C.POINTER(C.c_int64), C.c_int]),
     "pf_persist_state": (C.c_int, [C.c_void_p, C.c_void_p]),
     "pf_graph_window_info": (C.c_int, [C.c_void_p, C.c_int32] + [C.POINTER(C.c_int32)] * 4 + [_i32p, _i32p, _i32p]),
@@ -360,6 +361,10 @@
     _check(load_library().pf_persist_pair_halves(int(bool(on))))
 
 
+def back_fork(on=True):
+    _check(load_library().pf_back_fork(int(bool(on))))
+
+
 def persist_clock(ctx, reset=False):
     ms, n = C.c_double(0.0), C.c_int64(0)
     _check(load_library().pf_persist_clock(ctx._h, C.byref(ms), C.byref(n), int(bool(reset))))
diff --git a/pyfocusr_amd/csrc/pf_eigsort.hip b/pyfocusr_amd/csrc/pf_eigsort.hip
--- a/pyfocusr_amd/csrc/pf_eigsort.hip
+++ b/pyfocusr_amd/csrc/pf_eigsort.hip
@@ -4,10 +4,6 @@
 #include <vector>
 
 #include "pf_internal.h"
-
-extern "C" int pf_knn1_blocks(pf_ctx* c, const double* ref_block, int64_t n_ref, int32_t ref_stride, const double* qry_block, int64_t n_qry,
-                              int32_t qry_stride, int32_t d, const int32_t* col_ref, const double* scale_ref, const int32_t* col_qry,
-                              const double* scale_qry, int64_t* idx_out, double* d2_out);
 
 namespace {
 
@@ -15,19 +11,35 @@
 constexpr int ES_MAX_SAMPLES = 16384;
 constexpr int ES_RED_THREADS = 256;
 
-__global__ __launch_bounds__(PF_BLOCK) void k_es_gather(const double* __restrict__ fin, int32_t fc, const double* __restrict__ pts,
-                                                        const int64_t* __restrict__ rows, int64_t m, int32_t k,
-                                                        const int32_t* __restrict__ col, const double* __restrict__ sign,
-                                                        double* __restrict__ vals, double* __restrict__ raw) {
+struct EsSide {
+    const double* fin;
+    int32_t fc;
+    const double* pts;
+    const int64_t* rows;
+    int64_t m;
+    const int32_t* col;
+    const double* sign;
+    double* vals;
+    double* raw;
+    double* lohi;
+    double* norm;
+};
+
+__global__ __launch_bounds__(PF_BLOCK) void k_es_gather(EsSide t, EsSide s, int32_t k) {
+    const EsSide g = blockIdx.y ? s : t;
+    const int64_t m = g.m;
     const int64_t e = (int64_t)blockIdx.x * PF_BLOCK + threadIdx.x;
     if (e >= m * (k + 3)) return;
     const int64_t c = e / m, r = e - c * m;
-    if (c < k) vals[c * m + r] = fin[rows[r] * fc + col[c]] * sign[c];
-    else raw[r * 3 + (c - k)] = pts[rows[r] * 3 + (c - k)];
-}
-
-__global__ __launch_bounds__(ES_RED_THREADS) void k_es_minmax(const double* __restrict__ raw, int64_t m, double* __restrict__ lohi) {
+    if (c < k) g.vals[c * m + r] = g.fin[g.rows[r] * g.fc + g.col[c]] * g.sign[c];
+    else g.raw[r * 3 + (c - k)] = g.pts[g.rows[r] * 3 + (c - k)];
+}
+
+__global__ __launch_bounds__(ES_RED_THREADS) void k_es_minmax(EsSide t, EsSide s) {
     __shared__ double slo[ES_RED_THREADS], shi[ES_RED_THREADS];
+    const EsSide g = blockIdx.y ? s : t;
+    const double* __restrict__ raw = g.raw;
+    const int64_t m = g.m;
     const int c = blockIdx.x;
     double lo = INFINITY, hi = -INFINITY;
     for (int64_t r = threadIdx.x; r < m; r += ES_RED_THREADS) {
@@ -38,25 +50,25 @@
     slo[threadIdx.x] = lo;
     shi[threadIdx.x] = hi;
     __syncthreads();
-    for (int s = ES_RED_THREADS / 2; s > 0; s >>= 1) {
-        if (threadIdx.x < s) {
-            slo[threadIdx.x] = slo[threadIdx.x + s] < slo[threadIdx.x] ? slo[threadIdx.x + s] : slo[threadIdx.x];
-            shi[threadIdx.x] = shi[threadIdx.x + s] > shi[threadIdx.x] ? shi[threadIdx.x + s] : shi[threadIdx.x];
+    for (int s2 = ES_RED_THREADS / 2; s2 > 0; s2 >>= 1) {
+        if (threadIdx.x < s2) {
+            slo[threadIdx.x] = slo[threadIdx.x + s2] < slo[threadIdx.x] ? slo[threadIdx.x + s2] : slo[threadIdx.x];
+            shi[threadIdx.x] = shi[threadIdx.x + s2] > shi[threadIdx.x] ? shi[threadIdx.x + s2] : shi[threadIdx.x];
         }
         __syncthreads();
     }
     if (threadIdx.x == 0) {
-        lohi[c] = slo[0];
-        lohi[3 + c] = shi[0];
-    }
-}
-
-__global__ __launch_bounds__(PF_BLOCK) void k_es_normalize(const double* __restrict__ raw, const double* __restrict__ lohi, int64_t m,
-                                                           double* __restrict__ out) {
+        g.lohi[c] = slo[0];
+        g.lohi[3 + c] = shi[0];
+    }
+}
+
+__global__ __launch_bounds__(PF_BLOCK) void k_es_normalize(EsSide t, EsSide s) {
+    const EsSide g = blockIdx.y ? s : t;
     const int64_t e = (int64_t)blockIdx.x * PF_BLOCK + threadIdx.x;
-    if (e >= m * 3) return;
+    if (e >= g.m * 3) return;
     const int c = (int)(e % 3);
-    out[e] = (raw[e] - lohi[c]) / (lohi[3 + c] - lohi[c]);
+    g.norm[e] = (g.raw[e] - g.lohi[c]) / (g.lohi[3 + c] - g.lohi[c]);
 }
 
 __global__ __launch_bounds__(ES_SORT_THREADS) void k_es_sort_log(const double* __restrict__ vals_t, const double* __restrict__ vals_s,
@@ -198,11 +210,14 @@
     const size_t doubles = 2 * kt + 3 * ks + 6 * (size_t)(mt + ms) + 12 + 4 * (size_t)k * k;
     unsigned char* d = nullptr;
     const size_t up_bytes = (host.size() + 7) & ~(size_t)7, out_bytes = sizeof(double) * 4 * (size_t)k * k;
+    const size_t idx_bytes = sizeof(int64_t) * (size_t)mt;
     unsigned char* pin = nullptr;
-    PF_TRY(pf_pinned_scratch(c, up_bytes + out_bytes, reinterpret_cast<void**>(&pin)));
+    PF_TRY(pf_pinned_scratch(c, up_bytes + out_bytes + idx_bytes, reinterpret_cast<void**>(&pin)));
     memcpy(pin, host.data(), host.size());
+    hipStream_t sb = pf_back_fork_stream(c);
     PF_HIP(pf_malloc(st, (void**)&d, up_bytes + sizeof(double) * doubles));
     int rc = PF_OK;
+    bool forked = false;
     do {
         auto fail = [&](hipError_t e) {
             if (e == hipSuccess) return false;
@@ -227,28 +242,42 @@
         double* ls = lt + kt;
         double* lsf = ls + ks;
         double* d_out = lsf + ks;
-        k_es_gather<<<pf_blocks(mt * (k + 3)), PF_BLOCK, 0, st>>>(gt->final_vecs, gt->final_count, gt->pts, d_rows_t, mt, k, d_col, d_sign,
-                                                                  vals_t, raw_t);
-        k_es_gather<<<pf_blocks(ms * (k + 3)), PF_BLOCK, 0, st>>>(gs->final_vecs, gs->final_count, gs->pts, d_rows_s, ms, k, d_col + k,
-                                                                  d_sign + k, vals_s, raw_s);
-        k_es_minmax<<<3, ES_RED_THREADS, 0, st>>>(raw_t, mt, lohi);
-        k_es_minmax<<<3, ES_RED_THREADS, 0, st>>>(raw_s, ms, lohi + 6);
-        k_es_normalize<<<pf_blocks(3 * mt), PF_BLOCK, 0, st>>>(raw_t, lohi, mt, norm_t);
-        k_es_normalize<<<pf_blocks(3 * ms), PF_BLOCK, 0, st>>>(raw_s, lohi + 6, ms, norm_s);
-        k_es_sort_log<<<(unsigned)(2 * k), ES_SORT_THREADS, sort_lds, st>>>(vals_t, vals_s, mt, ms, k, lt, ls, lsf);
-        k_es_w1<<<(unsigned)(k * k), ES_RED_THREADS, 0, st>>>(lt, ls, lsf, mt, ms, k, d_out);
-        if (fail(hipGetLastError())) break;
+        const EsSide side_t{gt->final_vecs, gt->final_count, gt->pts, d_rows_t, mt, d_col, d_sign, vals_t, raw_t, lohi, norm_t};
+        const EsSide side_s{gs->final_vecs, gs->final_count, gs->pts, d_rows_s, ms, d_col + k, d_sign + k, vals_s, raw_s, lohi + 6, norm_s};
+        const int64_t m_max = mt > ms ? mt : ms;
+        k_es_gather<<<dim3(pf_blocks(m_max * (k + 3)), 2), PF_BLOCK, 0, st>>>(side_t, side_s, k);
+        if (fail(hipGetLastError())) break;
+        if (sb && fail(hipEventRecord(c->fork_ev, st))) break;
+        k_es_minmax<<<dim3(3, 2), ES_RED_THREADS, 0, st>>>(side_t, side_s);
+        k_es_normalize<<<dim3(pf_blocks(3 * m_max), 2), PF_BLOCK, 0, st>>>(side_t, side_s);
+        if (fail(hipGetLastError())) break;
+        hipStream_t st_hist = st;
+        if (sb) {
+            if (fail(hipStreamWaitEvent(sb, c->fork_ev, 0))) break;
+            st_hist = sb;
+            forked = true;
+        }
+        k_es_sort_log<<<(unsigned)(2 * k), ES_SORT_THREADS, sort_lds, st_hist>>>(vals_t, vals_s, mt, ms, k, lt, ls, lsf);
+        k_es_w1<<<(unsigned)(k * k), ES_RED_THREADS, 0, st_hist>>>(lt, ls, lsf, mt, ms, k, d_out);
+        if (fail(hipGetLastError())) break;
+        if (sb && fail(hipEventRecord(c->join_ev, sb))) break;
         const int32_t cols3[3] = {0, 1, 2};
         const double ones3[3] = {1.0, 1.0, 1.0};
-        rc = pf_knn1_blocks(c, norm_s, ms, 3, norm_t, mt, 3, 3, cols3, ones3, cols3, ones3, idx_out, nullptr);
+        rc = pf_knn1_blocks_queue(c, norm_s, ms, 3, norm_t, mt, 3, 3, cols3, ones3, cols3, ones3);
         if (rc != PF_OK) break;
         k_es_spatial<<<(unsigned)(k * k), ES_RED_THREADS, 0, st>>>(vals_t, vals_s, c->knn_idx.p, mt, ms, k, d_out);
         if (fail(hipGetLastError())) break;
+        if ((rc = pf_copy_by_kernel(st, c->knn_idx.p, pin + up_bytes + out_bytes, idx_bytes)) != PF_OK) break;
+        if (sb && fail(hipStreamWaitEvent(st, c->join_ev, 0))) break;
         if ((rc = pf_copy_by_kernel(st, d_out, pin + up_bytes, out_bytes)) != PF_OK) break;
         if (fail(hipStreamSynchronize(st))) break;
         memcpy(out, pin + up_bytes, out_bytes);
+        memcpy(idx_out, pin + up_bytes + out_bytes, idx_bytes);
     } while (0);
-    if (rc != PF_OK) (void)hipStreamSynchronize(st);
+    if (rc != PF_OK) {
+        if (forked) (void)hipStreamSynchronize(sb);
+        (void)hipStreamSynchronize(st);
+    }
     pf_free(st, d);
     return rc;
 }
diff --git a/pyfocusr_amd/csrc/pf_internal.h b/pyfocusr_amd/csrc/pf_internal.h
--- a/pyfocusr_amd/csrc/pf_internal.h
+++ b/pyfocusr_amd/csrc/pf_internal.h
@@ -346,7 +346,10 @@
     pf_sort_pairs(sc, k_in, k_out, (const int32_t*)v_in, (int32_t*)v_out, n, end_bit);
 }
 
-int pf_exclusive_scan_i32(hipStream_t st, const int32_t* in, int32_t* out, int64_t n);
+int pf_exclusive_scan_i32(hipStream_t st, const int32_t* in, int32_t* out, int64_t n, int32_t* totals = nullptr);
+constexpr int64_t PF_SCAN_TILE = 2048;
+constexpr int64_t PF_SCAN_OWN_TOTALS_MAX = 4096 * PF_SCAN_TILE;
+inline int64_t pf_scan_blocks(int64_t n) { return (n + PF_SCAN_TILE - 1) / PF_SCAN_TILE; }
 int pf_exclusive_scan_i64(hipStream_t st, const int64_t* in, int64_t* out, int64_t n);
 
 int pf_check_slots(pf_graph* g, int32_t first, int32_t count, const char* who);
@@ -381,6 +384,10 @@
 
 int pf_knn1_device(pf_ctx* c, const double* ref_block, int64_t n_ref, int32_t ref_stride, const double* qry_block, int64_t n_qry,
                    int32_t qry_stride, int32_t d);
+int pf_knn1_blocks_queue(pf_ctx* c, const double* ref_block, int64_t n_ref, int32_t ref_stride, const double* qry_block, int64_t n_qry,
+                         int32_t qry_stride, int32_t d, const int32_t* col_ref, const double* scale_ref, const int32_t* col_qry,
+                         const double* scale_qry);
+hipStream_t pf_back_fork_stream(pf_ctx* c);
 
 int pf_knn_extent(hipStream_t st, const double* pts, int64_t n, int32_t d, unsigned long long* ext);
 
diff --git a/pyfocusr_amd/csrc/pf_knn.hip b/pyfocusr_amd/csrc/pf_knn.hip
--- a/pyfocusr_amd/csrc/pf_knn.hip
+++ b/pyfocusr_amd/csrc/pf_knn.hip
@@ -3,8 +3,10 @@
 #include <string.h>
 
 #include <algorithm>
+#include <atomic>
 
 #include "pf_internal.h"
+#include "pf_launch.h"
 #include "pf_wave.h"
 
 namespace {
@@ -57,6 +59,10 @@
         else
             atomicMin(&ext[a], v);
     }
+}
+
+__global__ void k_extent_reset(unsigned long long* ext ) {
+    if (threadIdx.x < 32) ext[threadIdx.x] = threadIdx.x < 16 ? ~0ull : 0ull;
 }
 
 __global__ void k_make_grid(const unsigned long long* __restrict__ ext, int d, int res, KnnGrid* g) {
@@ -653,34 +659,36 @@
     for (int c = 0; c < d; ++c) rows_out[pos * d + c] = pts[i * d + c];
 }
 
-int sort_points(pf_ctx* c, const double* pts, int64_t n, int d, int morton, int key_bits, unsigned* key_out, int32_t* orig_out,
-                double* rows_out) {
-    Scratch s(c->stream);
-    unsigned* k0 = s.get<unsigned>(n);
-    int64_t n_buckets = 1;
-    {
-        const int res = c->knn_res;
-        if (morton) {
-            int bits = 0;
-            while ((1 << bits) < res) ++bits;
-            n_buckets = (int64_t)1 << (2 * bits);
-        } else {
-            n_buckets = d == 1 ? res : (int64_t)res * res;
-        }
-    }
-    int64_t bucket_max = (int64_t)1 << 22;
-    if (const char* ev = getenv("PF_KNN_BUCKET_MAX")) bucket_max = atoll(ev);
-    if (n_buckets <= bucket_max) {
-        int32_t* hist = s.get<int32_t>(3 * n_buckets + 2);
-        s.zero(hist, sizeof(int32_t) * (size_t)(3 * n_buckets + 2));
+int64_t sort_buckets(const pf_ctx* c, int d, int morton) {
+    const int res = c->knn_res;
+    if (!morton) return d == 1 ? res : (int64_t)res * res;
+    int bits = 0;
+    while ((1 << bits) < res) ++bits;
+    return (int64_t)1 << (2 * bits);
+}
+int64_t sort_hist_words(int64_t n_buckets) { return (3 * n_buckets + 2 + 3) & ~(int64_t)3; }
+int64_t sort_bucket_max() {
+    if (const char* ev = getenv("PF_KNN_BUCKET_MAX")) return atoll(ev);
+    return (int64_t)1 << 22;
+}
+
+int sort_points(pf_ctx* c, Scratch& s, hipStream_t st, const double* pts, int64_t n, int d, int morton, int key_bits, unsigned* k0,
+                unsigned* key_out, int32_t* orig_out, double* rows_out, int32_t* hist, int32_t* totals) {
+    const int64_t n_buckets = sort_buckets(c, d, morton);
+    if (n_buckets <= sort_bucket_max()) {
+        if (!hist) {
+            hist = s.get<int32_t>(3 * n_buckets + 2);
+            s.zero(hist, sizeof(int32_t) * (size_t)(3 * n_buckets + 2));
+            totals = nullptr;
+        }
         if (s.ok()) {
             int32_t* start = hist + n_buckets + 1;
             int32_t* cursor = start + n_buckets + 1;
-            k_cell_keys<<<pf_blocks(n), PF_BLOCK, 0, s.st>>>(pts, n, d, (const KnnGrid*)c->knn_grid, morton, k0, nullptr, hist);
+            k_cell_keys<<<pf_blocks(n), PF_BLOCK, 0, st>>>(pts, n, d, (const KnnGrid*)c->knn_grid, morton, k0, nullptr, hist);
             s.launched();
-            if (s.ok() && pf_exclusive_scan_i32(s.st, hist, start, n_buckets + 1) != PF_OK) s.note(hipErrorUnknown);
+            if (s.ok() && pf_exclusive_scan_i32(st, hist, start, n_buckets + 1, totals) != PF_OK) s.note(hipErrorUnknown);
             if (s.ok()) {
-                k_bucket_scatter<<<pf_blocks(n), PF_BLOCK, 0, s.st>>>(k0, n, start, cursor, key_out, orig_out, pts, d, rows_out);
+                k_bucket_scatter<<<pf_blocks(n), PF_BLOCK, 0, st>>>(k0, n, start, cursor, key_out, orig_out, pts, d, rows_out);
                 s.launched();
             }
         }
@@ -700,6 +708,18 @@
     return PF_OK;
 }
 
+}
+
+static std::atomic<int> g_back_fork{-1};
+hipStream_t pf_back_fork_stream(pf_ctx* c) {
+    int v = g_back_fork.load();
+    if (v < 0) {
+        const char* e = getenv("PF_BACK_FORK");
+        v = (e && e[0] == '0') ? 0 : 1;
+        g_back_fork.store(v);
+    }
+    if (!v) return nullptr;
+    return pf_stream_b(c) && c->fork_ev && c->join_ev ? c->stream_b : nullptr;
 }
 
 extern "C" {
@@ -768,14 +788,28 @@
     return knn_upload_k(c, ref, n_ref, qry, n_qry, d, 1);
 }
 
-static int knn_search(pf_ctx* c) {
+static int knn_path(const pf_ctx* c) {
+    const int d = c->knn_d;
+    if (c->knn_k == 1 && c->knn_mode == 0 && d <= 8 && c->knn_nref <= PF_KNN_SMALL && c->knn_nqry <= PF_KNN_SMALL) return 0;
+    if (c->knn_k == 1 && (c->knn_mode == 2 || (c->knn_mode == 0 && d >= PF_KNN_TREE_MIN_D))) return 1;
+    return 2;
+}
+
+static bool knn_counting(const pf_ctx* c) {
+    const int64_t nb_ref = sort_buckets(c, c->knn_d, 0), nb_qry = sort_buckets(c, c->knn_d, 1), most = sort_bucket_max();
+    return nb_ref <= most && nb_qry <= most && nb_ref < PF_SCAN_OWN_TOTALS_MAX && nb_qry < PF_SCAN_OWN_TOTALS_MAX;
+}
+
+static hipStream_t knn_side_stream(pf_ctx* c) { return knn_path(c) == 2 && knn_counting(c) ? pf_back_fork_stream(c) : nullptr; }
+
+static int knn_search(pf_ctx* c, hipStream_t sb) {
     hipStream_t st = c->stream;
     const int d = c->knn_d;
     const char* bad_d = "pf_knn_run: no search for d = %d";
-    if (c->knn_k == 1 && c->knn_mode == 0 && d <= 8 && c->knn_nref <= PF_KNN_SMALL && c->knn_nqry <= PF_KNN_SMALL)
-        return pf_dispatch_d<1, 8>(d, [&](auto D) { return launch_knn_small<D()>(c); }, bad_d);
+    const int path = knn_path(c);
+    if (path == 0) return pf_dispatch_d<1, 8>(d, [&](auto D) { return launch_knn_small<D()>(c); }, bad_d);
     PF_TRY(pf_knn_extent(st, c->knn_ref.p, c->knn_nref, d, c->knn_ext));
-    if (c->knn_k == 1 && (c->knn_mode == 2 || (c->knn_mode == 0 && d >= PF_KNN_TREE_MIN_D))) {
+    if (path == 1) {
         if (c->knn_nqry >= 32768) PF_TRY(pf_downloads_release(c));
         return pf_knn_tree_run(c);
     }
@@ -783,26 +817,61 @@
     const int64_t n_cells = d == 1 ? res : (int64_t)res * res;
     int cell_bits = 1;
     while (((int64_t)1 << cell_bits) < n_cells) ++cell_bits;
+    Scratch s(st);
+    int32_t *hist_r = nullptr, *hist_q = nullptr, *tot_r = nullptr, *tot_q = nullptr;
+    if (knn_counting(c)) {
+        const int64_t nb_ref = sort_buckets(c, d, 0), nb_qry = sort_buckets(c, d, 1);
+        const int64_t wr = sort_hist_words(nb_ref), wq = sort_hist_words(nb_qry), tr = pf_scan_blocks(nb_ref + 1);
+        int32_t* z = s.get<int32_t>(wr + wq + tr + pf_scan_blocks(nb_qry + 1));
+        PF_CHECK(s.ok(), PF_E_HIP, "pf_knn: %s", hipGetErrorString(s.err));
+        hist_r = z, hist_q = z + wr, tot_r = z + wr + wq, tot_q = tot_r + tr;
+        pfl::launch<pfl::k_fill_words>(dim3((unsigned)((wr + wq + 1023) / 1024)), dim3(256), 0, st, reinterpret_cast<uint32_t*>(z),
+                                        wr + wq, 0u);
+    }
     k_make_grid<<<1, 1, 0, st>>>(c->knn_ext, d, res, (KnnGrid*)c->knn_grid);
     PF_HIP(hipGetLastError());
-    PF_TRY(sort_points(c, c->knn_ref.p, c->knn_nref, d, 0, cell_bits, c->knn_ref_key.p, c->knn_ref_orig.p, c->knn_ref_s.p));
-    k_cell_start<<<pf_blocks(n_cells + 1), PF_BLOCK, 0, st>>>(c->knn_ref_key.p, c->knn_nref, n_cells, c->knn_cell_start.p);
-    PF_HIP(hipGetLastError());
-    if (c->knn_k == 1) {
-        k_gather_rows_soa<<<pf_blocks(c->knn_nref), PF_BLOCK, 0, st>>>(c->knn_ref.p, c->knn_ref_orig.p, c->knn_nref, d, c->knn_ref_ld, c->knn_ref_soa.p);
+    unsigned* k0_r = s.get<unsigned>(c->knn_nref);
+    unsigned* k0_q = s.get<unsigned>(c->knn_nqry);
+    PF_CHECK(s.ok(), PF_E_HIP, "pf_knn: %s", hipGetErrorString(s.err));
+    auto queries = [&](hipStream_t on) {
+        return sort_points(c, s, on, c->knn_qry.p, c->knn_nqry, d, 1, 32, k0_q, c->knn_qry_key.p, c->knn_qry_orig.p, c->knn_qry_s.p, hist_q,
+                           tot_q);
+    };
+    auto chains = [&]() -> int {
+        if (sb) PF_HIP(hipEventRecord(c->fork_ev, st));
+        PF_TRY(sort_points(c, s, st, c->knn_ref.p, c->knn_nref, d, 0, cell_bits, k0_r, c->knn_ref_key.p, c->knn_ref_orig.p, c->knn_ref_s.p,
+                           hist_r, tot_r));
+        k_cell_start<<<pf_blocks(n_cells + 1), PF_BLOCK, 0, st>>>(c->knn_ref_key.p, c->knn_nref, n_cells, c->knn_cell_start.p);
         PF_HIP(hipGetLastError());
-    }
-    PF_TRY(sort_points(c, c->knn_qry.p, c->knn_nqry, d, 1, 32, c->knn_qry_key.p, c->knn_qry_orig.p, c->knn_qry_s.p));
+        if (c->knn_k == 1) {
+            k_gather_rows_soa<<<pf_blocks(c->knn_nref), PF_BLOCK, 0, st>>>(c->knn_ref.p, c->knn_ref_orig.p, c->knn_nref, d, c->knn_ref_ld,
+                                                                           c->knn_ref_soa.p);
+            PF_HIP(hipGetLastError());
+        }
+        if (!sb) return queries(st);
+        PF_HIP(hipStreamWaitEvent(sb, c->fork_ev, 0));
+        PF_TRY(queries(sb));
+        PF_HIP(hipEventRecord(c->join_ev, sb));
+        PF_HIP(hipStreamWaitEvent(st, c->join_ev, 0));
+        return PF_OK;
+    };
+    const int rc = chains();
+    if (rc != PF_OK) {
+        if (sb) (void)hipStreamSynchronize(sb);
+        (void)hipStreamSynchronize(st);
+        return rc;
+    }
     if (c->knn_nqry >= 32768) PF_TRY(pf_downloads_release(c));
     return pf_dispatch_d<1, 16>(d, [&](auto D) { return launch_knn<D()>(c); }, bad_d);
 }
 
-int pf_knn_run(pf_ctx* c) {
-    PF_CHECK(c != nullptr, PF_E_ARG, "pf_knn_run: ctx is NULL");
-    PF_CHECK(c->knn_ready, PF_E_STATE, "pf_knn_run: no uploaded problem");
-    PF_HIP(hipSetDevice(c->device));
+static int knn_run_on(pf_ctx* c, hipStream_t sb) {
     PF_HIP(hipEventRecord(c->ev0, c->stream));
-    PF_TRY(knn_search(c));
+    const int rc = knn_search(c, sb);
+    if (rc != PF_OK) {
+        if (sb) (void)hipStreamSynchronize(sb);
+        return rc;
+    }
     PF_HIP(hipEventRecord(c->ev1, c->stream));
     PF_HIP(hipEventSynchronize(c->ev1));
     float ms = 0.f;
@@ -810,6 +879,13 @@
     c->knn_ms = ms;
     c->knn_done = true;
     return PF_OK;
+}
+
+int pf_knn_run(pf_ctx* c) {
+    PF_CHECK(c != nullptr, PF_E_ARG, "pf_knn_run: ctx is NULL");
+    PF_CHECK(c->knn_ready, PF_E_STATE, "pf_knn_run: no uploaded problem");
+    PF_HIP(hipSetDevice(c->device));
+    return knn_run_on(c, knn_side_stream(c));
 }
 
 int pf_knn_count(pf_ctx* c, int32_t enable_counting, int64_t* pairs) {
@@ -891,7 +967,7 @@
 
 static int knn1_blocks_run(pf_ctx* c, const double* ref_block, int64_t n_ref, int32_t ref_stride, const double* qry_block, int64_t n_qry,
                            int32_t qry_stride, int32_t d, const int32_t* col_ref, const double* scale_ref, const int32_t* col_qry,
-                           const double* scale_qry) {
+                           const double* scale_qry, bool queue_only = false) {
     PF_TRY(knn_prepare(c, n_ref, n_qry, d, 1));
     hipStream_t st = c->stream;
     CoordMap mr{}, mq{};
@@ -899,11 +975,27 @@
         mr.col[k] = col_ref[k], mr.scale[k] = scale_ref[k];
         mq.col[k] = col_qry[k], mq.scale[k] = scale_qry[k];
     }
+    hipStream_t sb = knn_side_stream(c);
+    if (sb) {
+        PF_HIP(hipEventRecord(c->fork_ev, st));
+        PF_HIP(hipStreamWaitEvent(sb, c->fork_ev, 0));
+    }
+    k_coords_from_final<<<pf_blocks(n_qry * d), PF_BLOCK, 0, sb ? sb : st>>>(qry_block, n_qry, qry_stride, d, mq, c->knn_qry.p);
     k_coords_from_final<<<pf_blocks(n_ref * d), PF_BLOCK, 0, st>>>(ref_block, n_ref, ref_stride, d, mr, c->knn_ref.p);
-    k_coords_from_final<<<pf_blocks(n_qry * d), PF_BLOCK, 0, st>>>(qry_block, n_qry, qry_stride, d, mq, c->knn_qry.p);
-    PF_HIP(hipGetLastError());
+    if (const hipError_t e = hipGetLastError(); e != hipSuccess) {
+        if (sb) (void)hipStreamSynchronize(sb);
+        return pf_hip_failed("pf_knn1_blocks", e);
+    }
     c->knn_ready = true;
-    return pf_knn_run(c);
+    if (!queue_only) return knn_run_on(c, sb);
+    const int rc = knn_search(c, sb);
+    if (rc != PF_OK && sb) (void)hipStreamSynchronize(sb);
+    return rc;
+}
+
+int pf_back_fork(int on) {
+    g_back_fork.store(on ? 1 : 0);
+    return PF_OK;
 }
 
 int pf_knn1_blocks(pf_ctx* c, const double* ref_block, int64_t n_ref, int32_t ref_stride, const double* qry_block, int64_t n_qry,
@@ -940,10 +1032,16 @@
 }
 
 int pf_knn_extent(hipStream_t st, const double* pts, int64_t n, int32_t d, unsigned long long* ext) {
-    PF_HIP(hipMemsetAsync(ext, 0xff, 16 * sizeof(unsigned long long), st));
-    PF_HIP(hipMemsetAsync(ext + 16, 0x00, 16 * sizeof(unsigned long long), st));
+    k_extent_reset<<<1, 32, 0, st>>>(ext);
     k_extent<<<256, PF_BLOCK, 0, st>>>(pts, n, d, ext);
-    return PF_OK;
+    PF_HIP(hipGetLastError());
+    return PF_OK;
+}
+
+int pf_knn1_blocks_queue(pf_ctx* c, const double* ref_block, int64_t n_ref, int32_t ref_stride, const double* qry_block, int64_t n_qry,
+                         int32_t qry_stride, int32_t d, const int32_t* col_ref, const double* scale_ref, const int32_t* col_qry,
+                         const double* scale_qry) {
+    return knn1_blocks_run(c, ref_block, n_ref, ref_stride, qry_block, n_qry, qry_stride, d, col_ref, scale_ref, col_qry, scale_qry, true);
 }
 
 int pf_knn1_device(pf_ctx* c, const double* ref_block, int64_t n_ref, int32_t ref_stride, const double* qry_block, int64_t n_qry,
diff --git a/pyfocusr_amd/csrc/pf_scan.hip b/pyfocusr_amd/csrc/pf_scan.hip
--- a/pyfocusr_amd/csrc/pf_scan.hip
+++ b/pyfocusr_amd/csrc/pf_scan.hip
@@ -5,6 +5,7 @@
 
 constexpr int SCAN_ITEMS = 8;
 constexpr int SCAN_TILE = PF_BLOCK * SCAN_ITEMS;
+static_assert(SCAN_TILE == PF_SCAN_TILE, "pf_scan_blocks counts these tiles");
 
 template <typename T>
 __device__ __forceinline__ T wave_inclusive_scan(T v, int lane) {
@@ -79,6 +80,7 @@
 };
 
 constexpr int64_t SCAN_DIRECT_BLOCKS = 4096;
+static_assert(SCAN_DIRECT_BLOCKS * SCAN_TILE == PF_SCAN_OWN_TOTALS_MAX, "the limit pf_internal.h names for a caller's totals");
 template <typename T>
 struct scan_block_apply_direct {
     static constexpr int BOUNDS = PF_BLOCK;
@@ -112,11 +114,17 @@
 };
 
 template <typename T>
-int exclusive_scan(hipStream_t st, const T* in, T* out, int64_t n) {
+int exclusive_scan(hipStream_t st, const T* in, T* out, int64_t n, T* own_totals = nullptr) {
     if (n <= 0) return PF_OK;
     const int64_t blocks = (n + SCAN_TILE - 1) / SCAN_TILE;
     if (blocks == 1) {
         pfl::launch<scan_block_apply<T>>(dim3(1), dim3(PF_BLOCK), 0, st, in, out, nullptr, n);
+        PF_HIP(hipGetLastError());
+        return PF_OK;
+    }
+    if (own_totals && blocks <= SCAN_DIRECT_BLOCKS) {
+        pfl::launch<scan_block_totals<T>>(dim3((unsigned)blocks), dim3(PF_BLOCK), 0, st, in, own_totals, n);
+        pfl::launch<scan_block_apply_direct<T>>(dim3((unsigned)blocks), dim3(PF_BLOCK), 0, st, in, out, own_totals, n);
         PF_HIP(hipGetLastError());
         return PF_OK;
     }
@@ -141,8 +149,8 @@
 
 }
 
-int pf_exclusive_scan_i32(hipStream_t st, const int32_t* in, int32_t* out, int64_t n) {
-    return exclusive_scan<int32_t>(st, in, out, n);
+int pf_exclusive_scan_i32(hipStream_t st, const int32_t* in, int32_t* out, int64_t n, int32_t* totals) {
+    return exclusive_scan<int32_t>(st, in, out, n, totals);
 }
 int pf_exclusive_scan_i64(hipStream_t st, const int64_t* in, int64_t* out, int64_t n) {
     return exclusive_scan<int64_t>(st, in, out, n);
```
